# nwicakson/diffpose-nw

Hardware: AMD Instinct MI355X
Metric: poses/sec (B=1024, 17j, K=50 DDIM) at 1/2/4/8 MI355X; MPJPE Δ vs ref (higher is better)
Workload: dtype fp32

## Files before the change

diffpose-nw_amd/csrc/dpk_kernels.hip:

```cpp
#include <hip/hip_runtime.h>

#include <math.h>
#include <stdint.h>
#include <stdio.h>
#include <stdlib.h>
#include <string.h>

#include <algorithm>
#include <atomic>
#include <string>
#include <type_traits>
#include <unordered_map>
#include <vector>

#include "diffpose_kernels.h"

#ifndef DPK_ABLATE
#define DPK_ABLATE 0
#endif
#define DPK_RUN(bit) ((DPK_ABLATE & (bit)) == 0)
#ifndef DPK_TRACE
#define DPK_TRACE 0
#endif
#if DPK_TRACE
namespace dpk {
__shared__ unsigned long long* tr_row[8];
__shared__ int tr_ix[8];
__device__ __forceinline__ void tr_stamp() {
    const int w = threadIdx.x >> 6;
    if (tr_row[w] && (threadIdx.x & 63) == 0 && tr_ix[w] < 256) tr_row[w][tr_ix[w]] = __builtin_amdgcn_s_memtime();
    if ((threadIdx.x & 63) == 0 && tr_row[w]) tr_ix[w] += 1;
}
}
#ifndef DPK_GEMM_HOOK
#define DPK_GEMM_HOOK(tag)                       \
    do {                                         \
        if ((tag) != 0) {                        \
            __builtin_amdgcn_sched_barrier(0);   \
            dpk::tr_stamp();                     \
            __builtin_amdgcn_sched_barrier(0);   \
        }                                        \
    } while (0)
#endif
#endif
#ifndef DPK_GEMM_HOOK
#define DPK_GEMM_HOOK(tag)
#endif


namespace dpk_shared {
struct SampleArgs {
    const float* arena;
    const float* coef;
    const float* tproj;
    const float* x_in;
    float* x_out;
    float* xs;
    float* x0s;
    float* uvxyz;
    int N;
    int K;
    int H;
    int root_mode;
    unsigned mask;
    const unsigned* pmask;
    float eta;
    unsigned long long seed;
    int pose_off;
    int num_layers;
    int split_n;
    int split_k;
    int split_full;
    unsigned* flags;
    unsigned token;
    const float* noise;
    int* split_stats;
    int split_dbg;
#if DPK_TRACE
    unsigned long long* trace;
    int trace_step;
#endif
};
}

#include "dpk_stage.inc"
#include "dpk_scratch.inc"

#define DPK_P 4
namespace dpk {
#include "dpk_sampler.inc"
#include "dpk_genfused.inc"
}
#undef DPK_P
#define DPK_P 2
namespace dpk2 {
#include "dpk_sampler.inc"
#include "dpk_genfused.inc"
}
#undef DPK_P
#define DPK_P 2
#undef DPK_D
#undef DPK_NH
#define DPK_D 128
#define DPK_NH 8
namespace dpkw {
#include "dpk_sampler.inc"
#include "dpk_genfused.inc"
}
#undef DPK_NH
#undef DPK_D
#undef DPK_P
#define DPK_P 2
#define DPK_D 128
#define DPK_NH 4
namespace dpkw4 {
#include "dpk_sampler.inc"
#include "dpk_genfused.inc"
}
#undef DPK_NH
#undef DPK_D
#undef DPK_P
#define DPK_P 4
#define DPK_D 64
#define DPK_NH 2
namespace dpkn {
#include "dpk_sampler.inc"
#include "dpk_genfused.inc"
}
#undef DPK_NH
#define DPK_NH 4
namespace dpkn4 {
#include "dpk_sampler.inc"
#include "dpk_genfused.inc"
}
#undef DPK_NH
#undef DPK_D
#undef DPK_P

namespace dpk {

__global__ void __launch_bounds__(256) ddim_kernel(const float* __restrict__ xt, const float* __restrict__ et,
                                                   float* __restrict__ xn, float* __restrict__ x0o, long long n,
                                                   const float* __restrict__ cf, int step, float eta,
                                                   unsigned long long seed, const float* __restrict__ noise) {
    const long long i = (long long)blockIdx.x * 256 + threadIdx.x;
    if (i >= n) return;
    const float z = noise ? noise[i] : (eta != 0.f ? normal_noise(seed, step, i) : 0.f);
    float x0, x1;
    ddim_elem(cf, xt[i], et[i], z, x0, x1);
    xn[i] = x1;
    if (x0o) x0o[i] = x0;
}

}

using namespace dpk;

struct Sched {
    uint64_t serial = 0;
    float* buf = nullptr;
    float* coef = nullptr;
    float* tps = nullptr;
    int K = 0;
    float eta = 0.f;
    std::vector<float> h_coef;
    uint64_t tps_gen = 0;
    int pins = 0;
    std::vector<std::pair<hipStream_t, hipEvent_t>> uses;
};

struct CapRes {
    unsigned long long id = 0;
    std::atomic<int> refs{1};
    std::atomic<bool> released{false};
    bool tracked = false;
    std::vector<Sched*> scheds;
    std::vector<ScratchBuf> bufs;
    std::vector<std::pair<hipStream_t, int>> slots;
};
static void cap_release_cb(void* p) {
    CapRes* c = static_cast<CapRes*>(p);
    c->released.store(true);
    if (c->refs.fetch_sub(1) == 1) delete c;
}

struct GenModel;
struct dpk_handle {
    int device = 0;
    GenModel* gen = nullptr;
    int n_pts = J;
    int kind = 0;
    int num_layers = NL;
    int n_cu = 256;
    int tail_plan = 2;
    unsigned* flags = nullptr;
    std::vector<int> slot_free;
    std::vector<std::pair<int, hipEvent_t>> slot_busy;
    std::vector<hipEvent_t> slot_ev;
    int split_dbg = 0;
    unsigned token = 0;
    std::vector<CapRes*> caps;
    std::string err;
    float* arena = nullptr;
    float* temb = nullptr;
    float* tproj_zero = nullptr;
    hipStream_t aux = nullptr;
    uint64_t weights_gen = 0;
    Sched* sched = nullptr;
    std::vector<Sched*> retired;
    ScratchPool pool;
    Stage stage;
    Packed pk;
    char* arena16 = nullptr;
    char* arenabf = nullptr;
    int gemm_mode = 0;
    bool have_graph = false, have_weights = false;
    unsigned mask = (1u << J) - 1u;
    const unsigned* pmask = nullptr;
    int pmask_n = 0;
    bool profiling = false;
    std::vector<std::pair<hipEvent_t, hipEvent_t>> ev_used, ev_free;
#if DPK_TRACE
    unsigned long long* trace = nullptr;
    size_t trace_len = 0;
    int trace_step = -1;
#endif
};

static int fail(dpk_handle* h, int code, const std::string& msg) {
    if (h) h->err = msg;
    return code;
}

template <class F>
static int profiled(dpk_handle* h, hipStream_t st, bool cap, const char* who, F launch) {
    if (!h->profiling || cap) return launch();
    if (h->ev_free.empty()) {
        hipEvent_t a, b;
        if (hipEventCreate(&a) != hipSuccess || hipEventCreate(&b) != hipSuccess)
            return fail(h, DPK_E_HIP, std::string(who) + ": event record");
        h->ev_free.push_back({a, b});
    }
    const std::pair<hipEvent_t, hipEvent_t> ev = h->ev_free.back();
    h->ev_free.pop_back();
    if (hipEventRecord(ev.first, st) != hipSuccess) return fail(h, DPK_E_HIP, std::string(who) + ": event record");
    const int rc = launch();
    if (rc) return rc;
    if (hipEventRecord(ev.second, st) != hipSuccess) return fail(h, DPK_E_HIP, std::string(who) + ": event record");
    h->ev_used.push_back(ev);
    return DPK_OK;
}

#define HIPCHK(h, expr)                                                                        \
    do {                                                                                       \
        hipError_t e_ = (expr);                                                                \
        if (e_ != hipSuccess)                                                                  \
            return fail((h), DPK_E_HIP, std::string(#expr) + ": " + hipGetErrorString(e_));    \
    } while (0)

static int capturing(dpk_handle* h, hipStream_t st, bool* cap) {
    hipStreamCaptureStatus cs = hipStreamCaptureStatusNone;
    HIPCHK(h, hipStreamIsCapturing(st, &cs));
    *cap = cs != hipStreamCaptureStatusNone;
    return DPK_OK;
}

static void sched_free(Sched* s) {
    if (s->buf) (void)hipFree(s->buf);
    for (auto& u : s->uses) (void)hipEventDestroy(u.second);
    delete s;
}

static void sched_sweep(dpk_handle* h) {
    std::vector<Sched*> keep;
    for (Sched* s : h->retired) {
        bool done = s->pins == 0;
        for (auto& u : s->uses) done = done && hipEventQuery(u.second) == hipSuccess;
        if (done) sched_free(s);
        else keep.push_back(s);
    }
    h->retired.swap(keep);
}

static int cap_get(dpk_handle* h, hipStream_t st, CapRes** out) {
    hipStreamCaptureStatus cs = hipStreamCaptureStatusNone;
    unsigned long long id = 0;
    hipGraph_t graph = nullptr;
    HIPCHK(h, hipStreamGetCaptureInfo_v2(st, &cs, &id, &graph, nullptr, nullptr));
    for (CapRes* c : h->caps)
        if (c->id == id) {
            *out = c;
            return DPK_OK;
        }
    CapRes* c = new CapRes();
    c->id = id;
    const char* env = getenv("DPK_CAPTURE_RELEASE");
    if (graph && !(env && atoi(env) == 0)) {
        c->refs.fetch_add(1);
        hipUserObject_t obj = nullptr;
        if (hipUserObjectCreate(&obj, c, cap_release_cb, 1, hipUserObjectNoDestructorSync) != hipSuccess) {
            c->refs.fetch_sub(1);
            (void)hipGetLastError();
        } else if (hipGraphRetainUserObject(graph, obj, 1, hipGraphUserObjectMove) != hipSuccess) {
            (void)hipGetLastError();
            (void)hipUserObjectRelease(obj, 1);
        } else {
            c->tracked = true;
        }
    }
    h->caps.push_back(c);
    *out = c;
    return DPK_OK;
}

static void slot_put(dpk_handle* h, int slot) { h->slot_free.push_back(slot); }

static bool drain_relaxed() {
    hipStreamCaptureMode mode = hipStreamCaptureModeRelaxed;
    const bool exch = hipThreadExchangeStreamCaptureMode(&mode) == hipSuccess;
    const hipError_t se = hipDeviceSynchronize();
    if (exch) (void)hipThreadExchangeStreamCaptureMode(&mode);
    if (se != hipSuccess) (void)hipGetLastError();
    return se == hipSuccess;
}

static void cap_sweep(dpk_handle* h) {
    bool any = false;
    for (CapRes* c : h->caps) any = any || (c->tracked && c->released.load());
    if (!any) return;
    std::vector<CapRes*> keep;
    for (CapRes* c : h->caps) {
        if (!(c->tracked && c->released.load())) {
            keep.push_back(c);
            continue;
        }
        for (Sched* s : c->scheds) --s->pins;
        scratch_release(h->pool, c->bufs);
        for (auto& s : c->slots) slot_put(h, s.second);
        if (c->refs.fetch_sub(1) == 1) delete c;
    }
    h->caps.swap(keep);
    sched_sweep(h);
}

static int sched_note_use(dpk_handle* h, Sched* s, hipStream_t st, bool cap) {
    if (cap) {
        CapRes* c = nullptr;
        const int rc = cap_get(h, st, &c);
        if (rc) return rc;
        if (std::find(c->scheds.begin(), c->scheds.end(), s) == c->scheds.end()) {
            c->scheds.push_back(s);
            ++s->pins;
        }
        return DPK_OK;
    }
    hipEvent_t ev = nullptr;
    for (auto& u : s->uses)
        if (u.first == st) ev = u.second;
    if (!ev) {
        HIPCHK(h, hipEventCreateWithFlags(&ev, hipEventDisableTiming));
        s->uses.push_back({st, ev});
    }
    HIPCHK(h, hipEventRecord(ev, st));
    return DPK_OK;
}

static int sched_compute_tps(dpk_handle* h, Sched* s) {
    hipLaunchKernelGGL(temb_kernel, dim3(s->K), dim3(256), 0, h->aux, h->temb, s->coef + 5, 6, s->tps);
    HIPCHK(h, hipGetLastError());
    HIPCHK(h, hipStreamSynchronize(h->aux));
    s->tps_gen = h->weights_gen;
    return DPK_OK;
}

static int upload(dpk_handle* h) {
    HIPCHK(h, hipSetDevice(h->device));
    HIPCHK(h, hipDeviceSynchronize());
    sched_sweep(h);
    if (!h->arena) HIPCHK(h, hipMalloc(&h->arena, (size_t)ARENA_FLOATS * 4));
    if (!h->arena16) HIPCHK(h, hipMalloc(&h->arena16, (size_t)ARENA16_BYTES));
    HIPCHK(h, hipMemcpy(h->arena16, h->pk.a16.data(), (size_t)ARENA16_BYTES, hipMemcpyHostToDevice));
    if (!h->arenabf) HIPCHK(h, hipMalloc(&h->arenabf, (size_t)ARENAB_BYTES));
    HIPCHK(h, hipMemcpy(h->arenabf, h->pk.abf.data(), (size_t)ARENAB_BYTES, hipMemcpyHostToDevice));
    if (!h->temb) HIPCHK(h, hipMalloc(&h->temb, (size_t)TEMB_FLOATS * 4));
    HIPCHK(h, hipMemcpy(h->arena, h->pk.arena.data(), (size_t)ARENA_FLOATS * 4, hipMemcpyHostToDevice));
    HIPCHK(h, hipMemcpy(h->temb, h->pk.temb.data(), (size_t)TEMB_FLOATS * 4, hipMemcpyHostToDevice));
    ++h->weights_gen;
    if (!h->have_weights || h->kind != 0) return DPK_OK;
    if (h->sched) {
        const int rc = sched_compute_tps(h, h->sched);
        if (rc) return rc;
    }
    for (Sched* s : h->retired) {
        const int rc = sched_compute_tps(h, s);
        if (rc) return rc;
    }
    return DPK_OK;
}

constexpr int FLAG_SLOTS = 64;
static int split_slot(dpk_handle* h, hipStream_t st, bool cap) {
    if (!h->flags) return -1;
    if (cap) {
        CapRes* c = nullptr;
        if (cap_get(h, st, &c)) return -1;
        for (auto& s : c->slots)
            if (s.first == st) return s.second;
        if (h->slot_free.empty()) return -1;
        const int slot = h->slot_free.back();
        h->slot_free.pop_back();
        c->slots.push_back({st, slot});
        return slot;
    }
    std::vector<std::pair<int, hipEvent_t>> busy;
    for (auto& b : h->slot_busy) {
        if (hipEventQuery(b.second) == hipSuccess) {
            h->slot_free.push_back(b.first);
            h->slot_ev.push_back(b.second);
        } else {
            busy.push_back(b);
        }
    }
    (void)hipGetLastError();
    h->slot_busy.swap(busy);
    if (h->slot_free.empty()) return -1;
    const int slot = h->slot_free.back();
    h->slot_free.pop_back();
    return slot;
}
static int split_slot_hold(dpk_handle* h, int slot, hipStream_t st) {
    hipEvent_t ev = nullptr;
    if (!h->slot_ev.empty()) {
        ev = h->slot_ev.back();
        h->slot_ev.pop_back();
    } else if (hipEventCreateWithFlags(&ev, hipEventDisableTiming) != hipSuccess) {
        h->slot_free.push_back(slot);
        HIPCHK(h, hipStreamSynchronize(st));
        return DPK_OK;
    }
    h->slot_busy.push_back({slot, ev});
    HIPCHK(h, hipEventRecord(ev, st));
    return DPK_OK;
}

template <int MODE, int PT>
static void launch_tiles(dpk_handle* h, int blocks, size_t shmem, hipStream_t st, const SampleArgs& a) {
    const char* a16 = h->gemm_mode == 2 ? h->arenabf : h->arena16;
    if constexpr (PT == 4) dpk::launch_sample<MODE>(h->pk.sparse, h->gemm_mode, blocks, shmem, st, a, h->arena, a16);
    else dpk2::launch_sample<MODE>(h->pk.sparse, h->gemm_mode, blocks, shmem, st, a, h->arena, a16);
}

template <int MODE>
static int launch_sampler(dpk_handle* h, hipStream_t st, SampleArgs a, bool cap) {
    const int N = a.N;
    const int round4 = P * h->n_cu;
    if constexpr (MODE == M_SAMPLE) {
        const int tiles = (N + P - 1) / P, q = tiles / h->n_cu, r = tiles % h->n_cu;
        if (h->tail_plan == 2 && a.K >= 2 && q >= 1 && r > 0 && 2 * r <= h->n_cu) {
            const int slot = split_slot(h, st, cap);
            if (slot >= 0) {
                a.pose_off = 0;
                a.split_n = r;
                a.split_k = a.K / 2;
                a.split_full = q * h->n_cu;
                a.flags = h->flags + (size_t)slot * h->n_cu;
                a.split_stats = reinterpret_cast<int*>(h->flags + (size_t)FLAG_SLOTS * h->n_cu);
                a.split_dbg = h->split_dbg;
                h->token = (h->token + 1) & 0x3fffffffu;
                if (h->token == 0) h->token = 1;
                a.token = h->token;
                launch_tiles<MODE, P>(h, q * h->n_cu + 2 * r, 0, st, a);
                HIPCHK(h, hipGetLastError());
                return cap ? DPK_OK : split_slot_hold(h, slot, st);
            }
        }
    }
    int n4 = N;
    const int rem = N % round4;
    if (h->tail_plan >= 1 && rem != 0 && rem <= 2 * h->n_cu) n4 = N - rem;
    if (n4 > 0) {
        a.pose_off = 0;
        launch_tiles<MODE, P>(h, (n4 + P - 1) / P, 0, st, a);
    }
    if (n4 < N) {
        constexpr int P2 = dpk2::P;
        constexpr size_t half = 160 * 1024 / 2, lds2 = (size_t)dpk2::SM_FLOATS * 4;
        constexpr size_t pad = lds2 > half ? 0 : half - lds2 + 256;
        a.pose_off = n4;
        launch_tiles<MODE, P2>(h, (N - n4 + P2 - 1) / P2, pad, st, a);
    }
    HIPCHK(h, hipGetLastError());
    return DPK_OK;
}

static int call_scratch(dpk_handle* h, hipStream_t st, bool cap, size_t n, const char* who, ScratchBuf& got,
                        ScratchStatus& why) {
    why = SCRATCH_OK;
    if (!cap) {
        got = ScratchBuf{st, scratch_get(h->pool, st, n), n};
        if (got.p) return DPK_OK;
        return fail(h, DPK_E_HIP, std::string(who) + ": scratch of " + std::to_string(n) + " floats: " +
                                      hipGetErrorString(hipGetLastError()));
    }
    CapRes* c = nullptr;
    const int rc = cap_get(h, st, &c);
    if (rc) return rc;
    why = scratch_get_captured(h->pool, c->bufs, st, n, got);
    return why == SCRATCH_OK ? DPK_OK : DPK_E_STATE;
}

static SampleArgs eps_args(const dpk_handle* h, const float* arena, const float* tproj, const float* x, float* out,
                           int N) {
    SampleArgs a{};
    a.arena = arena;
    a.tproj = tproj;
    a.x_in = x;
    a.x_out = out;
    a.N = N;
    a.K = 1;
    a.mask = h->mask;
    a.pmask = h->pmask;
    a.num_layers = h->num_layers;
    return a;
}
static SampleArgs sample_args(const dpk_handle* h, const float* arena, const float* tproj, const Sched* sc,
                              const float* x, float* out, float* xs, float* x0s, int N, uint64_t seed,
                              const float* noise) {
    SampleArgs a = eps_args(h, arena, tproj, x, out, N);
    a.coef = sc->coef;
    a.K = sc->K;
    a.eta = sc->eta;
    a.xs = xs;
    a.x0s = x0s;
    a.seed = seed;
    a.noise = noise;
    return a;
}
static SampleArgs pose_args(const dpk_handle* h, const float* arena, const float* zeros, const float* x2d, float* xyz,
                            float* uvxyz, int N, int H, int root_mode) {
    SampleArgs a = eps_args(h, arena, zeros, x2d, xyz, N);
    a.uvxyz = uvxyz;
    a.H = H;
    a.root_mode = root_mode;
    return a;
}

#include "dpk_generic.inc"

static int enter_call(dpk_handle* h, int N, const char* who, hipStream_t st, bool* cap) {
    if (h->pmask && N > h->pmask_n)
        return fail(h, DPK_E_INVALID, std::string(who) + ": " + std::to_string(N) + " poses but dpk_set_pose_masks covers " +
                                          std::to_string(h->pmask_n));
    HIPCHK(h, hipSetDevice(h->device));
    const int rc = capturing(h, st, cap);
    if (rc) return rc;
    if (!*cap) cap_sweep(h);
    return DPK_OK;
}

extern "C" {

int dpk_version(void) { return 100; }

int dpk_kernel_geometry(int* ppw, int* tpw, int* lds) {
    if (ppw) *ppw = P;
    if (tpw) *tpw = NT;
    if (lds) *lds = SM_FLOATS * 4;
    return DPK_OK;
}

int dpk_create(const dpk_config* cfg, dpk_handle** out) {
    if (!cfg || !out) return DPK_E_INVALID;
    *out = nullptr;
    const char* fg = getenv("DPK_FORCE_GENERIC");
    const bool pose_io = cfg->coords_in == CIN_POSE && cfg->coords_out == COUT_POSE;
    const bool compiled = cfg->hid_dim == D && cfg->num_layers >= 1 && cfg->num_layers <= NL && cfg->n_head == NH &&
                          cfg->n_pts == J && (pose_io || (cfg->coords_in == CIN && cfg->coords_out == COUT)) &&
                          !(fg && atoi(fg) != 0);
    if (cfg->hid_dim < 2 || cfg->n_head < 1 || cfg->hid_dim % cfg->n_head != 0 || cfg->num_layers < 1 ||
        cfg->n_pts < 2 || cfg->n_pts > dpkg::GJ_MAX || cfg->coords_in < 1 || cfg->coords_out < 1)
        return DPK_E_UNSUPPORTED;
    int kind;
    if (pose_io) kind = 1;
    else if (cfg->coords_in == cfg->coords_out) kind = 0;
    else return DPK_E_UNSUPPORTED;
    int ndev = 0;
    if (hipGetDeviceCount(&ndev) != hipSuccess || cfg->device < 0 || cfg->device >= ndev) return DPK_E_HIP;
    dpk_handle* h = new dpk_handle();
    h->device = cfg->device;
    h->kind = kind;
    h->num_layers = cfg->num_layers;
    h->n_pts = cfg->n_pts;
    h->mask = cfg->n_pts >= 32 ? ~0u : (1u << cfg->n_pts) - 1u;
    if (compiled) stage_init(h->stage, D, NH, J, cfg->num_layers, cfg->coords_in, cfg->coords_out, kind);
    else {
        h->gen = gen_new(cfg->hid_dim, cfg->n_head, cfg->n_pts, cfg->num_layers, cfg->coords_in, cfg->coords_out, kind);
        h->pool.replaced = gen_scratch_replaced;
        h->pool.ctx = h->gen;
    }
    if (hipSetDevice(h->device) != hipSuccess ||
        hipStreamCreateWithFlags(&h->aux, hipStreamNonBlocking) != hipSuccess ||
        hipDeviceGetAttribute(&h->n_cu, hipDeviceAttributeMultiprocessorCount, h->device) != hipSuccess) {
        if (h->aux) (void)hipStreamDestroy(h->aux);
        gen_free(h->gen);
        delete h;
        return DPK_E_HIP;
    }
    h->n_cu = std::max(h->n_cu, 1);
    if (const char* ts = getenv("DPK_TAIL_SPLIT")) h->tail_plan = std::min(std::max(atoi(ts), 0), 2);
    if (DPK_TRACE) h->tail_plan = 0;
    const size_t flag_bytes = ((size_t)FLAG_SLOTS * h->n_cu + 4) * 4;
    for (int s = FLAG_SLOTS - 1; s >= 0; --s) h->slot_free.push_back(s);
    if (hipMalloc(&h->flags, flag_bytes) != hipSuccess || hipMemset(h->flags, 0, flag_bytes) != hipSuccess) {
        if (h->flags) (void)hipFree(h->flags);
        (void)hipStreamDestroy(h->aux);
        gen_free(h->gen);
        delete h;
        return DPK_E_HIP;
    }
    *out = h;
    return DPK_OK;
}

void dpk_destroy(dpk_handle* h) {
    if (!h) return;
    (void)hipSetDevice(h->device);
    if (h->arena) (void)hipFree(h->arena);
    if (h->arena16) (void)hipFree(h->arena16);
    if (h->arenabf) (void)hipFree(h->arenabf);
    if (h->temb) (void)hipFree(h->temb);
    if (h->tproj_zero) (void)hipFree(h->tproj_zero);
    if (h->flags) (void)hipFree(h->flags);
    gen_free(h->gen);
    if (h->sched) sched_free(h->sched);
    for (Sched* s : h->retired) sched_free(s);
    scratch_free_all(h->pool);
    for (CapRes* c : h->caps) {
        scratch_free(c->bufs);
        if (c->refs.fetch_sub(1) == 1) delete c;
    }
    for (auto& b : h->slot_busy) (void)hipEventDestroy(b.second);
    for (hipEvent_t e : h->slot_ev) (void)hipEventDestroy(e);
    if (h->aux) (void)hipStreamDestroy(h->aux);
    for (auto* v : {&h->ev_used, &h->ev_free})
        for (auto& e : *v) {
            (void)hipEventDestroy(e.first);
            (void)hipEventDestroy(e.second);
        }
    delete h;
}

const char* dpk_last_error(const dpk_handle* h) { return h ? h->err.c_str() : "null handle"; }

static int pack_upload(dpk_handle* h) {
    if (h->gen) return gen_upload(h, h->gen);
    dpk::pack_model(h->stage, h->pk, true);
    return upload(h);
}

int dpk_set_graph(dpk_handle* h, const float* adj) {
    if (!h || !adj) return fail(h, DPK_E_INVALID, "dpk_set_graph: null argument");
    stage_set_graph(h->gen ? h->gen->s : h->stage, adj);
    h->have_graph = true;
    return h->have_weights ? pack_upload(h) : DPK_OK;
}

int dpk_set_mask(dpk_handle* h, const uint8_t* m) {
    if (!h || !m) return fail(h, DPK_E_INVALID, "dpk_set_mask: null argument");
    unsigned bits = 0;
    for (int j = 0; j < h->n_pts; ++j)
        if (m[j]) bits |= 1u << j;
    h->mask = bits;
    return DPK_OK;
}

int dpk_set_pose_masks(dpk_handle* h, const uint32_t* bits_dev, int n) {
    if (!h) return DPK_E_INVALID;
    if (bits_dev && n <= 0) return fail(h, DPK_E_INVALID, "dpk_set_pose_masks: n must be positive");
    h->pmask = reinterpret_cast<const unsigned*>(bits_dev);
    h->pmask_n = bits_dev ? n : 0;
    return DPK_OK;
}

int dpk_load_weights(dpk_handle* h, const char* const* names, const float* const* ptrs, const int64_t* numels,
                     int n) {
    if (!h || !names || !ptrs || !numels || n <= 0) return fail(h, DPK_E_INVALID, "dpk_load_weights: bad args");
    for (int i = 0; i < n; ++i)
        if (!names[i] || !ptrs[i]) return fail(h, DPK_E_INVALID, "dpk_load_weights: null entry");
    std::string err;
    if (!stage_load(h->gen ? h->gen->s : h->stage, names, ptrs, numels, n, err))
        return fail(h, DPK_E_WEIGHTS, "dpk_load_weights: " + err);
    h->have_weights = true;
    const int rc = pack_upload(h);
    if (rc || h->gen || h->kind == 0) return rc;
    if (!h->tproj_zero) {
        HIPCHK(h, hipMalloc(&h->tproj_zero, (size_t)NL * D * 4));
        HIPCHK(h, hipMemset(h->tproj_zero, 0, (size_t)NL * D * 4));
    }
    return DPK_OK;
}

int dpk_set_schedule(dpk_handle* h, const float* abar, int n_alpha, const int* seq, int K, float eta) {
    if (!h || !abar || !seq || K <= 0 || n_alpha < 2) return fail(h, DPK_E_INVALID, "dpk_set_schedule: bad args");
    if (h->kind != 0) return fail(h, DPK_E_STATE, "GCNpose handle (coords 2->3) has no diffusion schedule");
    std::vector<float> c((size_t)K * 6);
    for (int s = 0; s < K; ++s) {
        const int t = seq[K - 1 - s];
        const int tn = (K - 2 - s) >= 0 ? seq[K - 2 - s] : -1;
        if (t + 1 < 0 || t + 1 >= n_alpha || tn + 1 < 0 || tn + 1 >= n_alpha)
            return fail(h, DPK_E_INVALID, "dpk_set_schedule: timestep outside alpha table (index t+1)");
        const float at = abar[t + 1], an = abar[tn + 1];
        const float one = 1.0f;
        volatile float s1a = sqrtf(one - at);
        volatile float sa = sqrtf(at);
        volatile float san = sqrtf(an);
        volatile float r = at / an;
        volatile float u = one - r;
        volatile float v = one - an;
        volatile float w = u * v;
        volatile float inner = w / (one - at);
        volatile float c1 = eta * sqrtf(inner);
        volatile float c1sq = c1 * c1;
        volatile float c2 = sqrtf((one - an) - c1sq);
        c[s * 6 + 0] = s1a;
        c[s * 6 + 1] = sa;
        c[s * 6 + 2] = san;
        c[s * 6 + 3] = c1;
        c[s * 6 + 4] = c2;
        c[s * 6 + 5] = (float)t;
    }
    HIPCHK(h, hipSetDevice(h->device));
    sched_sweep(h);
    if (h->sched && h->sched->K == K && h->sched->eta == eta && h->sched->h_coef == c) return DPK_OK;
    Sched* s = new Sched();
    static uint64_t sched_serial = 0;
    s->serial = ++sched_serial;
    const size_t tps_off = ((size_t)K * 6 + 3) / 4 * 4;
    hipError_t e = hipMalloc(&s->buf, (tps_off + (size_t)K * NL * D) * 4);
    if (e != hipSuccess) {
        delete s;
        return fail(h, DPK_E_HIP, std::string("dpk_set_schedule: hipMalloc: ") + hipGetErrorString(e) +
                                      " (a schedule cannot be built while a graph is being captured)");
    }
    s->coef = s->buf;
    s->tps = s->buf + tps_off;
    s->K = K;
    s->eta = eta;
    s->h_coef = c;
    e = hipMemcpyAsync(s->coef, c.data(), c.size() * 4, hipMemcpyHostToDevice, h->aux);
    if (e == hipSuccess) e = hipStreamSynchronize(h->aux);
    if (e != hipSuccess) {
        sched_free(s);
        return fail(h, DPK_E_HIP, std::string("dpk_set_schedule: coef upload: ") + hipGetErrorString(e));
    }
    if (h->have_weights && !h->gen) {
        const int rc = sched_compute_tps(h, s);
        if (rc) {
            sched_free(s);
            return rc;
        }
    }
    if (h->sched) h->retired.push_back(h->sched);
    h->sched = s;
    sched_sweep(h);
    return DPK_OK;
}


static int check_ready(dpk_handle* h, int kind = 0) {
    if (h->kind != kind)
        return fail(h, DPK_E_STATE, kind ? "GCNdiff handle: dpk_pose needs a GCNpose handle (coords 2->3)"
                                         : "GCNpose handle (coords 2->3): use dpk_pose");
    if (!h->have_graph) return fail(h, DPK_E_STATE, "graph (adjacency) not set");
    if (!h->have_weights) return fail(h, DPK_E_STATE, "weights not loaded");
    if (h->gen && h->gemm_mode != 0)
        return fail(h, DPK_E_UNSUPPORTED, "generic-shape path (model shape other than hid 96 / 4 heads / 17 joints): "
                                          "fp32 GEMMs only (gemm mode 0)");
    if (h->gemm_mode == 1 && !h->pk.w16_ok)
        return fail(h, DPK_E_UNSUPPORTED, "gemm mode 1 (3x fp16): a GEMM weight has |w| >= 1015, outside the split-fp16 "
                                          "packing range; use gemm mode 0 (fp32)");
    return DPK_OK;
}

int dpk_eps(dpk_handle* h, const float* x, const float* t, float* eps, int N, void* stream) {
    if (!h) return DPK_E_INVALID;
    if (N < 0 || (N > 0 && (!x || !t || !eps))) return fail(h, DPK_E_INVALID, "dpk_eps: bad args");
    int rc = check_ready(h);
    if (rc) return rc;
    if (N == 0) return DPK_OK;
    hipStream_t st = (hipStream_t)stream;
    bool cap = false;
    if ((rc = enter_call(h, N, "dpk_eps", st, &cap))) return rc;
    if (h->gen) return gen_eps(h, x, t, eps, N, st, cap);
    constexpr size_t PP = (size_t)NL * D;
    ScratchBuf buf;
    ScratchStatus why;
    if ((rc = call_scratch(h, st, cap, (size_t)(cap ? N : std::max(N, 64)) * PP, "dpk_eps", buf, why))) {
        if (why == SCRATCH_NO_SPARE)
            return fail(h, rc, "dpk_eps: a captured call needs a projection buffer of " + std::to_string(N) +
                                   " poses, and the spare holds " + std::to_string(buf.cap / PP) +
                                   "; make an uncaptured dpk_eps call of >= N poses before the capture");
        if (why == SCRATCH_SHARED_TOO_SMALL)
            return fail(h, rc, "dpk_eps: the captured calls of one stream share the buffer of the capture's "
                               "first call (" + std::to_string(buf.cap / PP) + " poses); this one has " +
                                   std::to_string(N) + "; warm up with the largest N before capturing");
        return rc;
    }
    hipLaunchKernelGGL(temb_kernel, dim3(N), dim3(256), 0, st, h->temb, t, 1, buf.p);
    HIPCHK(h, hipGetLastError());
    return profiled(h, st, cap, "dpk_eps", [&] {
        return launch_sampler<M_EPS>(h, st, eps_args(h, h->arena, buf.p, x, eps, N), cap);
    });
}

int dpk_sample(dpk_handle* h, const float* x, float* out, float* xs, float* x0s, int N, uint64_t seed,
               void* stream) {
    return dpk_sample_noise(h, x, out, xs, x0s, N, seed, nullptr, stream);
}

int dpk_sample_noise(dpk_handle* h, const float* x, float* out, float* xs, float* x0s, int N, uint64_t seed,
                     const float* noise, void* stream) {
    if (!h) return DPK_E_INVALID;
    if (N < 0 || (N > 0 && (!x || !out))) return fail(h, DPK_E_INVALID, "dpk_sample: bad args");
    int rc = check_ready(h);
    if (rc) return rc;
    Sched* sc = h->sched;
    if (!sc) return fail(h, DPK_E_STATE, "schedule not set");
    if (N == 0) return DPK_OK;
    if (!h->gen && sc->tps_gen != h->weights_gen)
        return fail(h, DPK_E_STATE, "dpk_sample: schedule projections are stale");
    hipStream_t st = (hipStream_t)stream;
    bool cap = false;
    if ((rc = enter_call(h, N, "dpk_sample", st, &cap))) return rc;
    if (!cap) sched_sweep(h);
    if (h->gen) return gen_sample(h, sc, x, out, xs, x0s, N, seed, noise, st, cap);
    if (xs) HIPCHK(h, hipMemcpyAsync(xs, x, (size_t)N * PE * 4, hipMemcpyDeviceToDevice, st));
    SampleArgs a = sample_args(h, h->arena, sc->tps, sc, x, out, xs, x0s, N, seed, noise);
#if DPK_TRACE
    if (h->trace_step >= 0) {
        const size_t len = (size_t)((N + P - 1) / P) * NW * TRACE_SLOTS;
        if (h->trace_len < len) {
            if (h->trace) HIPCHK(h, hipFree(h->trace));
            HIPCHK(h, hipMalloc(&h->trace, len * 8));
            h->trace_len = len;
        }
        HIPCHK(h, hipMemsetAsync(h->trace, 0, len * 8, st));
    }
    a.trace = h->trace_step >= 0 ? h->trace : nullptr;
    a.trace_step = h->trace_step;
#endif
    rc = profiled(h, st, cap, "dpk_sample", [&] { return launch_sampler<M_SAMPLE>(h, st, a, cap); });
    return rc ? rc : sched_note_use(h, sc, st, cap);
}

int dpk_pose(dpk_handle* h, const float* x2d, float* xyz, float* uvxyz, int N, int H, int root_mode,
             void* stream) {
    if (!h) return DPK_E_INVALID;
    if (N < 0 || H < 1 || root_mode < 0 || root_mode > 2 || (N > 0 && (!x2d || (!xyz && !uvxyz))))
        return fail(h, DPK_E_INVALID, "dpk_pose: bad args");
    int rc = check_ready(h, 1);
    if (rc) return rc;
    if (N == 0) return DPK_OK;
    hipStream_t st = (hipStream_t)stream;
    bool cap = false;
    if ((rc = enter_call(h, N, "dpk_pose", st, &cap))) return rc;
    if (h->gen) return gen_pose(h, x2d, xyz, uvxyz, N, H, root_mode, st, cap);
    return profiled(h, st, cap, "dpk_pose", [&] {
        return launch_sampler<M_POSE>(h, st, pose_args(h, h->arena, h->tproj_zero, x2d, xyz, uvxyz, N, H, root_mode), cap);
    });
}

int dpk_set_gemm_mode(dpk_handle* h, int mode) {
    if (!h) return DPK_E_INVALID;
    if (mode < 0 || mode > 2)
        return fail(h, DPK_E_INVALID, "dpk_set_gemm_mode: mode must be 0 (fp32), 1 (3xfp16) or 2 (bf16)");
    h->gemm_mode = mode;
    return DPK_OK;
}

int dpk_set_tail_plan(dpk_handle* h, int plan) {
    if (!h) return DPK_E_INVALID;
    if (plan < 0 || plan > 2) return fail(h, DPK_E_INVALID, "dpk_set_tail_plan: plan must be 0, 1 or 2");
    h->tail_plan = DPK_TRACE ? 0 : plan;
    return DPK_OK;
}

int dpk_profile(dpk_handle* h, int enable) {
    if (!h) return DPK_E_INVALID;
    h->profiling = enable != 0;
    return DPK_OK;
}

int dpk_profile_read(dpk_handle* h, float* ms, int cap, int* count) {
    if (!h || (cap > 0 && !ms)) return fail(h, DPK_E_INVALID, "dpk_profile_read: bad args");
    HIPCHK(h, hipSetDevice(h->device));
    int n = 0;
    for (auto& e : h->ev_used) {
        HIPCHK(h, hipEventSynchronize(e.second));
        float t = 0.f;
        HIPCHK(h, hipEventElapsedTime(&t, e.first, e.second));
        if (n < cap) ms[n] = t;
        ++n;
        h->ev_free.push_back(e);
    }
    h->ev_used.clear();
    if (count) *count = n;
    return DPK_OK;
}

int dpk_ddim_update(dpk_handle* h, const float* xt, const float* et, float* xn, float* x0, int64_t n, int step,
                    uint64_t seed, void* stream) {
    return dpk_ddim_update_noise(h, xt, et, xn, x0, n, step, seed, nullptr, stream);
}

int dpk_ddim_update_noise(dpk_handle* h, const float* xt, const float* et, float* xn, float* x0, int64_t n,
                          int step, uint64_t seed, const float* noise, void* stream) {
    if (!h) return DPK_E_INVALID;
    if (n < 0 || (n > 0 && (!xt || !et || !xn))) return fail(h, DPK_E_INVALID, "dpk_ddim_update: bad args");
    Sched* sc = h->sched;
    if (!sc) return fail(h, DPK_E_STATE, "schedule not set");
    if (step < 0 || step >= sc->K) return fail(h, DPK_E_INVALID, "dpk_ddim_update: step out of range");
    if (n == 0) return DPK_OK;
    HIPCHK(h, hipSetDevice(h->device));
    hipStream_t st = (hipStream_t)stream;
    bool cap = false;
    int rc = capturing(h, st, &cap);
    if (rc) return rc;
    if (!cap) cap_sweep(h);
    const long long nb = (n + 255) / 256;
    hipLaunchKernelGGL(ddim_kernel, dim3((unsigned)nb), dim3(256), 0, st, xt, et, xn, x0, (long long)n,
                       sc->coef + step * 6, step, sc->eta, (unsigned long long)seed, noise);
    HIPCHK(h, hipGetLastError());
    return sched_note_use(h, sc, st, cap);
}

int dpk_debug_split(dpk_handle* h, int mode, int* fallbacks) {
    if (!h) return DPK_E_INVALID;
    if (mode < 0 || mode > 2) return fail(h, DPK_E_INVALID, "dpk_debug_split: mode must be 0, 1 or 2");
    h->split_dbg = mode;
    if (fallbacks) {
        HIPCHK(h, hipSetDevice(h->device));
        HIPCHK(h, hipDeviceSynchronize());
        int* ctr = reinterpret_cast<int*>(h->flags + (size_t)FLAG_SLOTS * h->n_cu);
        HIPCHK(h, hipMemcpy(fallbacks, ctr, 4, hipMemcpyDeviceToHost));
        HIPCHK(h, hipMemset(ctr, 0, 4));
    }
    return DPK_OK;
}

int dpk_debug_resources(dpk_handle* h, int* out, int n) {
    if (!h || (n > 0 && !out)) return DPK_E_INVALID;
    int released = 0, tracked = 0, retired = (int)h->retired.size();
    for (CapRes* c : h->caps) {
        tracked += c->tracked ? 1 : 0;
        released += (c->tracked && c->released.load()) ? 1 : 0;
    }
    const size_t spare = h->pool.spare.cap;
    const int v[8] = {(int)h->caps.size(), tracked, released, (int)h->slot_free.size(), retired,
                      h->gen ? 0 : (int)(spare / ((size_t)NL * D)), gen_graph_count(h->gen),
                      h->gen ? (int)((spare * 4) >> 10) : 0};
    for (int i = 0; i < n && i < 8; ++i) out[i] = v[i];
    return DPK_OK;
}

#if DPK_TRACE
int dpk_debug_trace(dpk_handle* h, int step, unsigned long long* out, long long cap) {
    if (!h) return DPK_E_INVALID;
    h->trace_step = step;
    if (!out || !h->trace) return DPK_OK;
    HIPCHK(h, hipDeviceSynchronize());
    HIPCHK(h, hipMemcpy(out, h->trace, std::min((size_t)cap, h->trace_len) * 8, hipMemcpyDeviceToHost));
    return (int)std::min((size_t)cap, h->trace_len);
}
#endif

}
```

diffpose-nw_amd/csrc/dpk_layout.inc:

```

#ifndef DPK_D
#define DPK_D 96
#endif
#ifndef DPK_NH
#define DPK_NH 4
#endif
constexpr int J = 17;
constexpr int D = DPK_D;
constexpr int D2 = 2 * D;
constexpr int D3 = 3 * D;
constexpr int E = 4 * D;
constexpr int NL = 5;
constexpr int NH = DPK_NH;
constexpr int DK = D / NH;
static_assert(D % 32 == 0 && D <= 128 && (DK == 24 || DK == 16 || DK == 32), "widths: multiples of 32 up to 128, d_k 16, 24 or 32");
constexpr int NCD = D / 16;
constexpr int CIN = 5;
constexpr int COUT = 5;
constexpr int PE = J * CIN;

constexpr bool HALF_MODES = D == 96 && NH == 4;

constexpr int P = DPK_P;
constexpr int R = P * J;
static_assert(P == 4 || P == 2, "4 or 2 poses per workgroup");
constexpr int NW = 4;
constexpr int NT = 64 * NW;
constexpr int stride40(int n) { return n + (104 - n % 64) % 64; }
constexpr int LDX = stride40(D);
constexpr int LD2 = stride40(D3);
static_assert(LDX % 64 == 40 && LD2 % 64 == 40 && LDX >= D && LD2 >= D3, "row strides");

constexpr int SM_XS = 0;
constexpr int SM_B1 = SM_XS + R * LDX;
constexpr int SM_B2 = SM_B1 + R * LDX;
constexpr int SM_XST = SM_B2 + R * LD2;
constexpr int SM_LNP = SM_XST + ((R * CIN + 3) / 4) * 4;
constexpr int SM_TC = SM_LNP + NL * 4 * D;
constexpr int SM_TS = SM_TC + 2 * J * J;
constexpr int SM_FLOATS = SM_TS + J * (5 + 9) * 2;
static_assert(SM_FLOATS * 4 <= 160 * 1024, "LDS budget");

constexpr int BLK = 256;
constexpr int KB_D = D / 16, KB_D2 = D2 / 16, KB_D3 = D3 / 16;
constexpr int OFF_QKV = 0;
constexpr int OFF_O = OFF_QKV + 3 * NCD * KB_D * BLK;
constexpr int OFF_FC1 = OFF_O + NCD * KB_D * BLK;
constexpr int OFF_FC2 = OFF_FC1 + 2 * NCD * KB_D * BLK;
constexpr int OFF_C1 = OFF_FC2 + NCD * KB_D2 * BLK;
constexpr int OFF_C2 = OFF_C1 + NCD * KB_D3 * BLK;
constexpr int OFF_BQKV = OFF_C2 + NCD * KB_D3 * BLK;
constexpr int OFF_BO = OFF_BQKV + D3;
constexpr int OFF_BFC1 = OFF_BO + D;
constexpr int OFF_BFC2 = OFF_BFC1 + D2;
constexpr int OFF_BC1 = OFF_BFC2 + D;
constexpr int OFF_BC2 = OFF_BC1 + D;
constexpr int OFF_LN0A = OFF_BC2 + D;
constexpr int OFF_LN0B = OFF_LN0A + D;
constexpr int OFF_LN1A = OFF_LN0B + D;
constexpr int OFF_LN1B = OFF_LN1A + D;
constexpr int OFF_LG = OFF_LN1B + D;
constexpr int OFF_LGF = ((OFF_LG + J * J + 63) / 64) * 64;
constexpr int OFF_CQKV = OFF_LGF + 2 * 5 * 64;
constexpr int LAYER_FLOATS = ((OFF_CQKV + D3 + 63) / 64) * 64;
constexpr int OFF_WIN = NL * LAYER_FLOATS;
constexpr int OFF_WOUT = OFF_WIN + NCD * 1 * BLK;
constexpr int OFF_BIN = OFF_WOUT + 1 * KB_D3 * BLK;
constexpr int OFF_BOUT = OFF_BIN + D;
constexpr int OFF_CHEB = OFF_BOUT + 16;
constexpr int OFF_CHEBS = OFF_CHEB + 2 * J * J;
constexpr int SPT1 = 5, SPT2 = 9;
constexpr int OFF_CHEBT = OFF_CHEBS + 136;
constexpr int CHEBT_FLOATS = J * (SPT1 + SPT2) * 2;
constexpr int ARENA_FLOATS = ((OFF_CHEBT + CHEBT_FLOATS + 63) / 64) * 64;

constexpr float W16_SCALE = 64.0f;
constexpr int BLK16 = 2048;
constexpr int KB32_D = D / 32, KB32_D2 = D2 / 32, KB32_D3 = D3 / 32;
constexpr int O16_QKV = 0;
constexpr int O16_O = O16_QKV + 3 * NCD * KB32_D * BLK16;
constexpr int O16_FC1 = O16_O + NCD * KB32_D * BLK16;
constexpr int O16_FC2 = O16_FC1 + 2 * NCD * KB32_D * BLK16;
constexpr int O16_C1 = O16_FC2 + NCD * KB32_D2 * BLK16;
constexpr int O16_C2 = O16_C1 + NCD * KB32_D3 * BLK16;
constexpr int LAYER16_BYTES = O16_C2 + NCD * KB32_D3 * BLK16;
constexpr int ARENA16_BYTES = NL * LAYER16_BYTES;

constexpr int TOFF_W0 = 0;
constexpr int TOFF_B0 = TOFF_W0 + D * E;
constexpr int TOFF_W1 = TOFF_B0 + E;
constexpr int TOFF_B1 = TOFF_W1 + E * E;
constexpr int TOFF_WP = TOFF_B1 + E;
constexpr int TOFF_BP = TOFF_WP + NL * E * D;
constexpr int TEMB_FLOATS = TOFF_BP + NL * D;

constexpr float SQRT_DK = DK == 24 ? 4.898979485566356f : DK == 32 ? 5.656854249492381f : 4.0f;
constexpr float LN_EPS = 1e-6f;
constexpr int H36M_EDGES[16][2] = {{0, 1}, {1, 2}, {2, 3}, {0, 4}, {4, 5}, {5, 6}, {0, 7}, {7, 8},
                                   {8, 9}, {9, 10}, {8, 11}, {11, 12}, {12, 13}, {8, 14}, {14, 15}, {15, 16}};
struct SparsePattern {
    int n1[J], c1[J][J], o1[J];
    int n2[J], c2[J][J], o2[J];
    int nnz1, nnz2;
};
constexpr SparsePattern make_pattern() {
    SparsePattern sp{};
    bool a[J][J] = {};
    for (int i = 0; i < J; ++i) a[i][i] = true;
    for (int e = 0; e < 16; ++e) {
        a[H36M_EDGES[e][0]][H36M_EDGES[e][1]] = true;
        a[H36M_EDGES[e][1]][H36M_EDGES[e][0]] = true;
    }
    int t1 = 0, t2 = 0;
    for (int i = 0; i < J; ++i) {
        sp.n1[i] = 0;
        sp.n2[i] = 0;
        sp.o1[i] = t1;
        sp.o2[i] = t2;
        for (int j = 0; j < J; ++j) {
            bool two = false;
            for (int k = 0; k < J; ++k) two = two || (a[i][k] && a[k][j]);
            if (a[i][j]) sp.c1[i][sp.n1[i]++] = j;
            if (two) sp.c2[i][sp.n2[i]++] = j;
        }
        t1 += sp.n1[i];
        t2 += sp.n2[i];
    }
    sp.nnz1 = t1;
    sp.nnz2 = t2;
    return sp;
}
constexpr SparsePattern SPAT = make_pattern();
static_assert(SPAT.nnz1 == 49 && SPAT.nnz2 == 87, "H36M Chebyshev sparsity");
```

diffpose-nw_amd/csrc/dpk_sampler.inc:

```

#include "dpk_layout.inc"

struct NoHook {
    __device__ __forceinline__ void operator()() const {}
};
#ifndef DPK_PRE_MID
#define DPK_PRE_MID 14
#endif
#define DPK_MID(bit) ((DPK_PRE_MID & (bit)) != 0)

typedef float f32x4 __attribute__((ext_vector_type(4)));
typedef float f32x2 __attribute__((ext_vector_type(2)));

__device__ __forceinline__ f32x2 pfma(f32x2 a, f32x2 b, f32x2 c) { return __builtin_elementwise_fma(a, b, c); }
__device__ __forceinline__ f32x2 splat2(float x) { return f32x2{x, x}; }
__device__ __forceinline__ f32x2 vpair(float x) {
    f32x2 p = {x, x};
    asm volatile("" : "+v"(p));
    return p;
}
__device__ __forceinline__ f32x4 padd4(f32x4 x, f32x2 ns) {
    const f32x2 lo = f32x2{x[0], x[1]} + ns, hi = f32x2{x[2], x[3]} + ns;
    return f32x4{lo[0], lo[1], hi[0], hi[1]};
}
__device__ __forceinline__ f32x4 pmul4(f32x4 x, f32x2 r) {
    const f32x2 lo = f32x2{x[0], x[1]} * r, hi = f32x2{x[2], x[3]} * r;
    return f32x4{lo[0], lo[1], hi[0], hi[1]};
}

typedef _Float16 f16x8 __attribute__((ext_vector_type(8)));
typedef _Float16 f16x4 __attribute__((ext_vector_type(4)));
typedef _Float16 f16x2 __attribute__((ext_vector_type(2)));
typedef __bf16 bf16x8 __attribute__((ext_vector_type(8)));
typedef __bf16 bf16x2 __attribute__((ext_vector_type(2)));
typedef short s16x4 __attribute__((ext_vector_type(4)));

enum { M_SAMPLE = 0, M_EPS = 1, M_POSE = 2 };
constexpr int CIN_POSE = 2, COUT_POSE = 3;

using SampleArgs = ::dpk_shared::SampleArgs;
constexpr int TRACE_SLOTS = 256;

__device__ __forceinline__ void philox(uint32_t c[4], uint32_t k0, uint32_t k1) {
#pragma unroll
    for (int r = 0; r < 10; ++r) {
        const uint64_t p0 = (uint64_t)0xD2511F53u * c[0];
        const uint64_t p1 = (uint64_t)0xCD9E8D57u * c[2];
        const uint32_t n0 = (uint32_t)(p1 >> 32) ^ c[1] ^ k0;
        const uint32_t n2 = (uint32_t)(p0 >> 32) ^ c[3] ^ k1;
        c[1] = (uint32_t)p1;
        c[3] = (uint32_t)p0;
        c[0] = n0;
        c[2] = n2;
        k0 += 0x9E3779B9u;
        k1 += 0xBB67AE85u;
    }
}

__device__ __forceinline__ float normal_noise(unsigned long long seed, int step, long long idx) {
    uint32_t c[4] = {(uint32_t)idx, (uint32_t)((unsigned long long)idx >> 32), (uint32_t)step, 0x5EEDu};
    philox(c, (uint32_t)seed, (uint32_t)(seed >> 32));
    const float u1 = ((float)(c[0] >> 8) + 1.0f) * (1.0f / 16777216.0f);
    const float u2 = (float)(c[1] >> 8) * (1.0f / 16777216.0f);
    return sqrtf(-2.0f * logf(u1)) * cosf(6.283185307179586f * u2);
}

__device__ __forceinline__ void ddim_elem(const float* cf, float xt, float et, float z, float& x0, float& xn) {
    x0 = (xt - et * cf[0]) / cf[1];
    xn = (cf[2] * x0 + cf[3] * z) + cf[4] * et;
}

template <int J>
__device__ __forceinline__ float row_ror(float x) {
    return __builtin_bit_cast(float, __builtin_amdgcn_update_dpp(__builtin_bit_cast(int, x), __builtin_bit_cast(int, x),
                                                                 0x120 + J, 0xf, 0xf, false));
}

__device__ __forceinline__ float sum4rows(float v) {
    float a = v, b = v;
    asm("s_nop 1\n\tv_permlane32_swap_b32 %0, %1" : "+v"(a), "+v"(b));
    const float s1 = a + b;
    float c = s1, d = s1;
    asm("s_nop 1\n\tv_permlane16_swap_b32 %0, %1" : "+v"(c), "+v"(d));
    return c + d;
}

__device__ __forceinline__ void sum4rows2(float& x, float& y) {
    asm("s_nop 1\n\tv_permlane32_swap_b32 %0, %1" : "+v"(x), "+v"(y));
    float c = x + y, d = c;
    asm("s_nop 1\n\tv_permlane16_swap_b32 %0, %1" : "+v"(c), "+v"(d));
    x = c + d;
    y = x;
    asm("s_nop 1\n\tv_permlane32_swap_b32 %0, %1" : "+v"(x), "+v"(y));
}
__device__ __forceinline__ void max4rows2(float& x, float& y) {
    asm("s_nop 1\n\tv_permlane32_swap_b32 %0, %1" : "+v"(x), "+v"(y));
    float c = fmaxf(x, y), d = c;
    asm("s_nop 1\n\tv_permlane16_swap_b32 %0, %1" : "+v"(c), "+v"(d));
    x = fmaxf(c, d);
    y = x;
    asm("s_nop 1\n\tv_permlane32_swap_b32 %0, %1" : "+v"(x), "+v"(y));
}

__device__ __forceinline__ float rs4rows(float v0, float v1, float v2, float v3) {
    asm("s_nop 1\n\tv_permlane32_swap_b32 %0, %1" : "+v"(v0), "+v"(v2));
    asm("s_nop 1\n\tv_permlane32_swap_b32 %0, %1" : "+v"(v1), "+v"(v3));
    float a = v0 + v2, b = v1 + v3;
    asm("s_nop 1\n\tv_permlane16_swap_b32 %0, %1" : "+v"(a), "+v"(b));
    return a + b;
}

constexpr int PAD_MFMA4 = 5;
constexpr int PAD_MFMA16 = 11;
template <int N, int K>
__device__ __forceinline__ void mfma_pad(f32x4 (&v)[K]) {
    static_assert(K >= 1 && K <= 8, "mfma_pad: 1..8 accumulators");
    if constexpr (K == 1) asm volatile("s_nop %1" : "+v"(v[0]) : "i"(N));
    else if constexpr (K == 2) asm volatile("s_nop %2" : "+v"(v[0]), "+v"(v[1]) : "i"(N));
    else if constexpr (K == 3) asm volatile("s_nop %3" : "+v"(v[0]), "+v"(v[1]), "+v"(v[2]) : "i"(N));
    else if constexpr (K == 4) asm volatile("s_nop %4" : "+v"(v[0]), "+v"(v[1]), "+v"(v[2]), "+v"(v[3]) : "i"(N));
    else if constexpr (K == 5)
        asm volatile("s_nop %5" : "+v"(v[0]), "+v"(v[1]), "+v"(v[2]), "+v"(v[3]), "+v"(v[4]) : "i"(N));
    else if constexpr (K == 6)
        asm volatile("s_nop %6" : "+v"(v[0]), "+v"(v[1]), "+v"(v[2]), "+v"(v[3]), "+v"(v[4]), "+v"(v[5]) : "i"(N));
    else if constexpr (K == 7)
        asm volatile("s_nop %7"
                     : "+v"(v[0]), "+v"(v[1]), "+v"(v[2]), "+v"(v[3]), "+v"(v[4]), "+v"(v[5]), "+v"(v[6])
                     : "i"(N));
    else
        asm volatile("s_nop %8"
                     : "+v"(v[0]), "+v"(v[1]), "+v"(v[2]), "+v"(v[3]), "+v"(v[4]), "+v"(v[5]), "+v"(v[6]), "+v"(v[7])
                     : "i"(N));
}

__device__ __forceinline__ int opaque(int x) {
    asm volatile("" : "+v"(x));
    return x;
}
__device__ __forceinline__ int opaque_s(int x) {
    asm volatile("" : "+s"(x));
    return x;
}

struct BSrc {
    __amdgpu_buffer_rsrc_t rsrc;
    int voff;
    int sbase;
    __device__ __forceinline__ f32x4 load(int blk) const {
        return __builtin_bit_cast(f32x4, __builtin_amdgcn_raw_buffer_load_b128(rsrc, voff, sbase + blk * 1024, 0));
    }
};

__device__ __forceinline__ f32x4 bload(const BSrc& s, int toff, int kb) {
    return __builtin_bit_cast(f32x4, __builtin_amdgcn_raw_buffer_load_b128(s.rsrc, toff, kb * 1024, 0));
}

template <int NC, int KB>
__device__ __forceinline__ BSrc bsrc(const float* Bp, int ct0, int lane) {
    BSrc s;
    s.rsrc = __builtin_amdgcn_make_buffer_rsrc((void*)Bp, (short)0, 0x7fffffff, 0x00020000);
    s.voff = lane * 16;
    s.sbase = ct0 * KB * 1024;
    return s;
}

enum { TM_NONE = 0, TM_VALU = 1, TM_MFMA4 = 2 };

template <int NR, int NCW, int TM, int TR, int KB, bool TRANS = true>
struct GemmTile {
    static constexpr int TA = TM == TM_VALU ? TR : 1;
    static constexpr int NQ = TM == TM_MFMA4 ? (NCW + 1) / 2 : 1;
    f32x4 acc[NR][NCW];
    float tl[NCW][TA];
    f32x4 tacc[NQ];
    int aoff[NR], toff[TA];

    __device__ __forceinline__ void loadA(f32x4 (&a)[NR], f32x4 (&t)[TA], const float* A, int kb) const {
#pragma unroll
        for (int i = 0; i < NR; ++i) a[i] = *reinterpret_cast<const f32x4*>(A + aoff[i] + kb * 16);
        if constexpr (TM != TM_NONE) {
#pragma unroll
            for (int i = 0; i < TA; ++i) t[i] = *reinterpret_cast<const f32x4*>(A + toff[i] + kb * 16);
        }
    }
    __device__ __forceinline__ static void loadB(f32x4 (&b)[NCW], const BSrc& s, const int (&soff)[NCW], int kb) {
#pragma unroll
        for (int c = 0; c < NCW; ++c) b[c] = bload(s, soff[c], kb);
    }
    template <bool FIRST = false>
    __device__ __forceinline__ void mma(const f32x4 (&a)[NR], const f32x4 (&t)[TA], const f32x4 (&b)[NCW]) {
        const f32x4 z = {0.f, 0.f, 0.f, 0.f};
#pragma unroll
        for (int j = 0; j < 4; ++j) {
#pragma unroll
            for (int i = 0; i < NR; ++i)
#pragma unroll
                for (int c = 0; c < NCW; ++c) {
                    const f32x4 cin = (FIRST && j == 0) ? z : acc[i][c];
                    acc[i][c] = TRANS ? __builtin_amdgcn_mfma_f32_16x16x4f32(b[c][j], a[i][j], cin, 0, 0, 0)
                                      : __builtin_amdgcn_mfma_f32_16x16x4f32(a[i][j], b[c][j], cin, 0, 0, 0);
                }
            if constexpr (TM == TM_VALU) {
#pragma unroll
                for (int c = 0; c < NCW; ++c)
#pragma unroll
                    for (int r = 0; r < TR; ++r) tl[c][r] = fmaf(t[r][j], b[c][j], tl[c][r]);
            } else if constexpr (TM == TM_MFMA4) {
#pragma unroll
                for (int q = 0; q < NQ; ++q)
                    tacc[q] = __builtin_amdgcn_mfma_f32_4x4x1f32(b[q][j], t[0][j], (FIRST && j == 0) ? z : tacc[q], 0, 0, 0);
            }
        }
    }
    __device__ __forceinline__ static void schedule_half() { __builtin_amdgcn_sched_barrier(0); }
};

template <int NCW>
struct BPre {
    f32x4 b0[NCW], b1[NCW];
};

__device__ __forceinline__ int gemm_ch(int wave) { return R == 68 ? (wave & 1) : (wave >> 1); }
__device__ __forceinline__ int gemm_pr(int wave) { return R == 68 ? (wave >> 1) : (wave & 1); }

template <int NCW>
__device__ __forceinline__ int col_rot(int wave) { return gemm_pr(wave) ? (NCW + 1) / 2 : 0; }

template <int NCW, int KB>
__device__ __forceinline__ void tile_offsets(int (&soff)[NCW], const BSrc& s, int rot) {
#pragma unroll
    for (int c = 0; c < NCW; ++c) {
        const int cc = c + rot;
        soff[c] = s.voff + s.sbase + (cc >= NCW ? cc - NCW : cc) * KB * 1024;
    }
}

template <int NC, int KB, int NPRE = 2>
__device__ __forceinline__ BPre<NC / 2> gemm_prefetch(const float* Bp, int wave, int lane) {
    constexpr int NCW = NC / 2;
    const BSrc s = bsrc<NC, KB>(Bp, gemm_ch(wave) * NCW, lane);
    int soff[NCW];
    tile_offsets<NCW, KB>(soff, s, col_rot<NCW>(wave));
    BPre<NCW> pre;
#pragma unroll
    for (int c = 0; c < NCW; ++c) {
        pre.b0[c] = bload(s, soff[c], 0);
        pre.b1[c] = (KB > 1 && NPRE > 1) ? bload(s, soff[c], 1) : f32x4{0.f, 0.f, 0.f, 0.f};
    }
    return pre;
}

#ifndef DPK_PRE_LATE
#define DPK_PRE_LATE 5
#endif
#define DPK_LATE(bit) ((DPK_PRE_LATE & (bit)) != 0)
#ifndef DPK_FC1_NPRE
#define DPK_FC1_NPRE 2
#endif
#ifndef DPK_QKV_NPRE
#define DPK_QKV_NPRE 1
#endif
enum { E_STORE = 0, E_STORE_RELU, E_RESID, E_RESID_RELU, E_CHEB1, E_STORE_NB };

struct EpiArgs {
    float* dst;
    int ldd;
    const float* bias;
    const float* tproj;
    int tproj_pose_stride;
    int pose0;
    int pose_max;
};

__device__ __forceinline__ float rcp_nr(float d) {
    const float r = __builtin_amdgcn_rcpf(d);
    return fmaf(r, fmaf(-d, r, 1.0f), r);
}

template <int MODE>
__device__ __forceinline__ float epi_value(float acc, float bias, float tp, float old) {
    const float v = acc + bias;
    if constexpr (MODE == E_STORE_NB) return acc;
    else if constexpr (MODE == E_STORE) return v;
    else if constexpr (MODE == E_STORE_RELU) return fmaxf(v, 0.f);
    else if constexpr (MODE == E_RESID) return old + v;
    else if constexpr (MODE == E_RESID_RELU) return old + fmaxf(v, 0.f);
    else return fmaxf(v, 0.f) + tp;
}

template <int MODE, bool NB = false>
__device__ __forceinline__ f32x4 epi_value4(f32x4 acc, f32x4 bias, f32x4 tp, f32x4 old) {
    if constexpr (MODE == E_STORE_NB) return acc;
    f32x4 v = acc;
    if constexpr (!NB) v = acc + bias;
    const f32x4 z = {0.f, 0.f, 0.f, 0.f};
    if constexpr (MODE == E_STORE) return v;
    else if constexpr (MODE == E_STORE_RELU) return __builtin_elementwise_max(v, z);
    else if constexpr (MODE == E_RESID) return old + v;
    else if constexpr (MODE == E_RESID_RELU) return old + __builtin_elementwise_max(v, z);
    else return __builtin_elementwise_max(v, z) + tp;
}

__device__ __forceinline__ float tproj_at(const EpiArgs& e, int row, int col, float tcol) {
    if (e.tproj_pose_stride == 0) return tcol;
    const int pose = min(e.pose0 + row / J, e.pose_max);
    return e.tproj[(size_t)pose * e.tproj_pose_stride + col];
}


template <int NR, int NCW, int TM, int TR, int NC, int KB, int MODE, bool XS2 = false, int NPRE = 2>
__device__ __forceinline__ void gemm_wave(const float* A, int lda, const float* Bp, int rt0, int ct0, int rot,
                                          int trow0, bool tail_dup, int lane, const EpiArgs& e,
                                          const BPre<NCW>& pre, const float* AX = nullptr, int ldx = 0) {
    using T = GemmTile<NR, NCW, TM, TR, KB>;
    constexpr int TA = T::TA, NQ = T::NQ;
    static_assert(KB == 1 || KB % 2 == 0, "k-blocks in pairs");
    lane = opaque(lane);
    T g;
#pragma unroll
    for (int c = 0; c < NCW; ++c)
#pragma unroll
        for (int r = 0; r < TA; ++r) g.tl[c][r] = 0.f;
    const int rl = lane & 15, kq = (lane >> 4) * 4;
#pragma unroll
    for (int i = 0; i < NR; ++i) g.aoff[i] = ((rt0 + i) * 16 + rl) * lda + kq;
    if constexpr (TM == TM_MFMA4) {
        g.toff[0] = (trow0 + (lane & 3)) * lda + kq;
    } else {
#pragma unroll
        for (int i = 0; i < TA; ++i) g.toff[i] = (trow0 + i) * lda + kq;
    }
    int xoff[NR], xtoff = 0;
    if constexpr (XS2) {
        static_assert(TM == TM_MFMA4, "XS2: 4x4x1 tail rows");
#pragma unroll
        for (int i = 0; i < NR; ++i) xoff[i] = ((rt0 + i) * 16 + rl) * ldx + kq;
        xtoff = (trow0 + (lane & 3)) * ldx + kq;
    }
    int gcol[NCW];
#pragma unroll
    for (int c = 0; c < NCW; ++c) {
        const int cc = c + rot;
        gcol[c] = ct0 + (cc >= NCW ? cc - NCW : cc);
    }
    const BSrc src = bsrc<NC, KB>(Bp, ct0, lane);
    int soff[NCW];
    tile_offsets<NCW, KB>(soff, src, rot);
    const int tcol = 4 * ((lane >> 2) & 3) + (lane >> 4);
    f32x4 bias4[NCW], tp4[NCW];
    float tbias[NQ], ttp[NQ];
    auto load_epi_consts = [&]() {
        const unsigned kqu = (unsigned)kq, tcu = (unsigned)tcol;
        const int boff = (int)(e.bias - Bp) * 4;
#pragma unroll
        for (int c = 0; c < NCW; ++c) {
            const float* pt = e.tproj + gcol[c] * 16;
            if constexpr (MODE == E_STORE_NB) bias4[c] = f32x4{0.f, 0.f, 0.f, 0.f};
            else bias4[c] = __builtin_bit_cast(f32x4, __builtin_amdgcn_raw_buffer_load_b128(src.rsrc, kq * 4, boff + gcol[c] * 64, 0));
            tp4[c] = (MODE == E_CHEB1 && e.tproj_pose_stride == 0) ? *reinterpret_cast<const f32x4*>(pt + kqu)
                                                                   : f32x4{0.f, 0.f, 0.f, 0.f};
        }
#pragma unroll
        for (int q = 0; q < NQ; ++q) {
            tbias[q] = 0.f;
            ttp[q] = 0.f;
            if constexpr (TM == TM_MFMA4) {
                if constexpr (MODE != E_STORE_NB)
                    tbias[q] = __builtin_bit_cast(float, __builtin_amdgcn_raw_buffer_load_b32(src.rsrc, tcol * 4, boff + gcol[q] * 64, 0));
                if (MODE == E_CHEB1 && e.tproj_pose_stride == 0) ttp[q] = (e.tproj + gcol[q] * 16)[tcu];
            }
        }
    };
    constexpr int KBX = D / 16;
    constexpr int S = (KB == 1) ? 1
                      : (XS2 && (KBX == 8 || KBX == 4)) ? 4
                      : (NCW <= 6 && KB % 3 == 0) ? 3 : 2;
    static_assert(KB == 1 || KB % S == 0, "ring slots divide the k-blocks");
    static_assert(!XS2 || (KB > 2 * S && (KBX == S || KBX == 2 * S)), "XS2: the x block is one or two ring passes");
    f32x4 as[S][NR], ts[S][TA], bs[S][NCW];
    auto loadA = [&](int st, int kb) {
        if (XS2 && kb < KBX) {
#pragma unroll
            for (int i = 0; i < NR; ++i) as[st][i] = *reinterpret_cast<const f32x4*>(AX + xoff[i] + kb * 16);
            ts[st][0] = *reinterpret_cast<const f32x4*>(AX + xtoff + kb * 16);
        } else {
            g.loadA(as[st], ts[st], A, kb);
        }
    };
    constexpr bool RES = MODE == E_RESID || MODE == E_RESID_RELU;
    const int trow = trow0 + (lane & 3);
    constexpr int R0 = (NCW + 1) / 2;
    auto tile_ptr = [&](int i, int c) -> float* {
        const int row = (rt0 + i) * 16 + rl;
        float* rb = e.dst + row * e.ldd + kq + ct0 * 16;
        return (c < NCW - R0 ? rb + rot * 16 : rb - (rot ? (NCW - R0) * 16 : 0)) + c * 16;
    };
    f32x4 old[NR][NCW];
    float oldt[NQ];
    auto load_old = [&]() {
        if constexpr (RES) {
#pragma unroll
            for (int i = 0; i < NR; ++i)
#pragma unroll
                for (int c = 0; c < NCW; ++c)
                    old[i][c] = *reinterpret_cast<const f32x4*>(tile_ptr(i, c));
            if constexpr (TM == TM_MFMA4) {
#pragma unroll
                for (int q = 0; q < NQ; ++q) oldt[q] = e.dst[min(trow, R - 1) * e.ldd + gcol[q] * 16 + tcol];
            }
        }
    };
    constexpr int NP = S > 1 ? NPRE : 1;
#pragma unroll
    for (int c = 0; c < NCW; ++c) {
        bs[0][c] = pre.b0[c];
        if constexpr (NP > 1) bs[1][c] = pre.b1[c];
    }
    DPK_GEMM_HOOK(0);
#pragma unroll
    for (int st = NP; st < S; ++st) T::loadB(bs[st], src, soff, st);
#pragma unroll
    for (int st = 0; st < S; ++st) loadA(st, st);
    if constexpr (KB > S) {
#pragma unroll
        for (int st = 0; st < S; ++st) {
            if (st == 0) g.template mma<true>(as[0], ts[0], bs[0]);
            else g.mma(as[st], ts[st], bs[st]);
            T::loadB(bs[st], src, soff, st + S);
            loadA(st, st + S);
            T::schedule_half();
        }
#pragma unroll 1
        for (int kb = S; kb < KB - S; kb += S) {
#pragma unroll
            for (int st = 0; st < S; ++st) {
                g.mma(as[st], ts[st], bs[st]);
                T::loadB(bs[st], src, soff, kb + st + S);
                g.loadA(as[st], ts[st], A, kb + st + S);
                T::schedule_half();
            }
        }
        load_old();
        load_epi_consts();
#pragma unroll
        for (int st = 0; st < S; ++st) g.mma(as[st], ts[st], bs[st]);
    } else {
        __builtin_amdgcn_sched_barrier(0);
        load_epi_consts();
        load_old();
#pragma unroll
        for (int st = 0; st < S; ++st) {
            if (st == 0) g.template mma<true>(as[st], ts[st], bs[st]);
            else g.mma(as[st], ts[st], bs[st]);
        }
    }
    DPK_GEMM_HOOK(1);
    __builtin_amdgcn_sched_barrier(0);
    auto tproj4 = [&](int row, int col4, const f32x4& uniform4) -> f32x4 {
        if constexpr (MODE != E_CHEB1) return f32x4{0.f, 0.f, 0.f, 0.f};
        if (e.tproj_pose_stride == 0) return uniform4;
        const int pose = min(e.pose0 + row / J, e.pose_max);
        return *reinterpret_cast<const f32x4*>(e.tproj + (size_t)pose * e.tproj_pose_stride + col4);
    };
#pragma unroll
    for (int i = 0; i < NR; ++i) {
        const int row = (rt0 + i) * 16 + rl;
#pragma unroll
        for (int c = 0; c < NCW; ++c) {
            const int col4 = gcol[c] * 16 + kq;
            const f32x4 tp = tproj4(row, col4, tp4[c]);
            *reinterpret_cast<f32x4*>(tile_ptr(i, c)) =
                epi_value4<MODE>(g.acc[i][c], bias4[c], tp, RES ? old[i][c] : f32x4{0.f, 0.f, 0.f, 0.f});
        }
    }
    if constexpr (TM == TM_VALU) {
        static_assert(TM != TM_VALU, "gemm_wave computes transposed tiles; VALU tails are gemm_out's");
    } else if constexpr (TM == TM_MFMA4) {
        const int row = trow;
        mfma_pad<PAD_MFMA4>(g.tacc);
#pragma unroll
        for (int q = 0; q < NQ; ++q) {
            const float v = rs4rows(g.tacc[q][0], g.tacc[q][1], g.tacc[q][2], g.tacc[q][3]);
            const bool skip = (q == NQ - 1 && tail_dup) || row >= R;
            const int col = gcol[q] * 16 + tcol;
            const float tp = MODE == E_CHEB1 ? tproj_at(e, min(row, R - 1), col, ttp[q]) : 0.f;
            float val = epi_value<MODE>(v, tbias[q], tp, RES ? oldt[q] : 0.f);
            asm volatile("" : "+v"(val));
            if (!skip) e.dst[row * e.ldd + col] = val;
        }
    }
    DPK_GEMM_HOOK(2);
}

template <int NC, int KB, int MODE, bool XS2 = false, int NPRE = 2>
__device__ __forceinline__ void gemm_wg(const float* A, int lda, const float* Bp, int wave, int lane,
                                        const EpiArgs& e, const BPre<NC / 2>& pre,
                                        const float* AX = nullptr, int ldx = 0) {
    static_assert(NC % 2 == 0 && (R == 68 || R == 34), "row tiles x 2 column halves + tail rows");
    constexpr int NCW = NC / 2;
    constexpr int NRW = R == 68 ? 2 : 1;
    const int pr = gemm_pr(wave);
    const bool dup = (NCW & 1) && pr == 1;
    gemm_wave<NRW, NCW, TM_MFMA4, 0, NC, KB, MODE, XS2, NPRE>(A, lda, Bp, NRW * pr, gemm_ch(wave) * NCW,
                                                             col_rot<NCW>(wave), R - R % 16, dup, lane, e, pre, AX, ldx);
}

template <int PW>
__device__ __forceinline__ int pass_col(int ctp, int c, int rot) {
    const int cc = c + rot;
    return ctp + (cc >= PW ? cc - PW : cc);
}

#ifndef DPK_HS_BF
#define DPK_HS_BF 3
#endif
#ifndef DPK_PWQ16
#define DPK_PWQ16 3
#endif
#ifndef DPK_PWF16
#define DPK_PWF16 3
#endif
constexpr int BLKB = 1024;
template <int G>
constexpr int blkh() { return G == 1 ? BLK16 : BLKB; }
template <int G>
constexpr int offh(int l, int o16) { return G == 1 ? l * LAYER16_BYTES + o16 : (l * LAYER16_BYTES + o16) / 2; }
constexpr int ARENAB_BYTES = ARENA16_BYTES / 2;

template <int G>
struct AFr {
    f16x8 h, l;
};

__device__ __forceinline__ f16x8 cat2x4(f16x2 a, f16x2 b, f16x2 c, f16x2 d) {
    const f16x4 ab = __builtin_shufflevector(a, b, 0, 1, 2, 3), cd = __builtin_shufflevector(c, d, 0, 1, 2, 3);
    return __builtin_shufflevector(ab, cd, 0, 1, 2, 3, 4, 5, 6, 7);
}
template <int G>
__device__ __forceinline__ void acvt(const f32x4& lo4, const f32x4& hi4, AFr<G>& o) {
    const f32x2 v[4] = {f32x2{lo4[0], lo4[1]}, f32x2{lo4[2], lo4[3]}, f32x2{hi4[0], hi4[1]}, f32x2{hi4[2], hi4[3]}};
    f16x2 h[4], l[4];
#pragma unroll
    for (int p = 0; p < 4; ++p) {
        if constexpr (G == 2) {
            h[p] = __builtin_bit_cast(f16x2, __builtin_convertvector(v[p], bf16x2));
        } else {
            h[p] = __builtin_convertvector(v[p], f16x2);
            l[p] = __builtin_convertvector(v[p] - __builtin_convertvector(h[p], f32x2), f16x2);
        }
    }
    o.h = cat2x4(h[0], h[1], h[2], h[3]);
    if constexpr (G == 1) o.l = cat2x4(l[0], l[1], l[2], l[3]);
}

struct BSrcH {
    __amdgpu_buffer_rsrc_t rsrc;
    __device__ __forceinline__ f16x8 load(int voff, int soff) const {
        return __builtin_bit_cast(f16x8, __builtin_amdgcn_raw_buffer_load_b128(rsrc, voff, soff, 0));
    }
};
template <int G, int NC, int KB32>
__device__ __forceinline__ BSrcH bsrch(const char* Bp) {
    BSrcH s;
    s.rsrc = __builtin_amdgcn_make_buffer_rsrc((void*)Bp, (short)0, NC * KB32 * blkh<G>(), 0x00020000);
    return s;
}

template <int G, int PW>
struct BPreH {
    f16x8 h[2][PW], l[2][G == 1 ? PW : 1];
};
template <int PW>
__device__ __forceinline__ int passh_rot(int wave) { return gemm_pr(wave) ? (PW + 1) / 2 : 0; }
template <int G, int NC, int KB32, int PW>
__device__ __forceinline__ BPreH<G, PW> gemmh_prefetch(const char* Bp, int wave, int lane, int ps = 0) {
    constexpr int BK = blkh<G>();
    const BSrcH s = bsrch<G, NC, KB32>(Bp);
    const int ctp = gemm_ch(wave) * (NC / 2) + ps * PW, rot = passh_rot<PW>(wave);
    BPreH<G, PW> pre;
#pragma unroll
    for (int c = 0; c < PW; ++c) {
        const int voff = lane * 16 + pass_col<PW>(ctp, c, rot) * KB32 * BK;
#pragma unroll
        for (int k = 0; k < 2; ++k) {
            pre.h[k][c] = s.load(voff, k * BK);
            if constexpr (G == 1) pre.l[k][c] = s.load(voff, k * BK + 1024);
        }
    }
    return pre;
}

template <int G, int NR, int PW, int NC, int KB32, int MODE, bool XS2, int S, int AR>
__device__ __forceinline__ void gemmh_pass(const float* A, int lda, const float* AX, int ldx, const BSrcH& src,
                                           int rt0, int ctp, int rot, int trow0, bool tail_dup, int lane,
                                           const EpiArgs& e, const BPreH<G, PW>& pre, AFr<G> (*ar)[NR + 1]) {
    constexpr int BK = blkh<G>();
    constexpr int NQ = (PW + 1) / 2;
    constexpr int NA = NR + 1;
    static_assert(S >= 2 && S <= KB32, "ring slots");
    lane = opaque(lane);
    const int rl = lane & 15, g = lane >> 4, kq = g * 4;
    int gcol[PW], voff[PW];
#pragma unroll
    for (int c = 0; c < PW; ++c) {
        gcol[c] = pass_col<PW>(ctp, c, rot);
        voff[c] = lane * 16 + gcol[c] * KB32 * BK;
    }
    int aoff[NA], xoff[NA];
#pragma unroll
    for (int i = 0; i < NR; ++i) {
        aoff[i] = (int)__umul24((unsigned)((rt0 + i) * 16 + rl), (unsigned)lda) + kq;
        xoff[i] = (int)__umul24((unsigned)((rt0 + i) * 16 + rl), (unsigned)ldx) + kq;
    }
    const int trow_a = min(trow0 + rl, R - 1);
    aoff[NR] = (int)__umul24((unsigned)trow_a, (unsigned)lda) + kq;
    xoff[NR] = (int)__umul24((unsigned)trow_a, (unsigned)ldx) + kq;
    f32x4 raw[NA][2];
    auto loadA = [&](int kb) {
        if constexpr (AR != 2) {
#pragma unroll
            for (int i = 0; i < NA; ++i) {
                const float* p = (XS2 && kb * 32 < D) ? AX + xoff[i] + kb * 32 : A + aoff[i] + kb * 32;
                raw[i][0] = *reinterpret_cast<const f32x4*>(p);
                raw[i][1] = *reinterpret_cast<const f32x4*>(p + 16);
            }
        }
    };
    f16x8 bh[S][PW], bl[S][G == 1 ? PW : 1];
    auto loadB = [&](int st, int kb) {
#pragma unroll
        for (int c = 0; c < PW; ++c) {
            bh[st][c] = src.load(voff[c], kb * BK);
            if constexpr (G == 1) bl[st][c] = src.load(voff[c], kb * BK + 1024);
        }
    };
    f32x4 bias4[PW], tp4[PW];
    auto load_epi = [&]() {
        const __amdgpu_buffer_rsrc_t br = __builtin_amdgcn_make_buffer_rsrc((void*)e.bias, (short)0, 0x7fffffff, 0x00020000);
#pragma unroll
        for (int c = 0; c < PW; ++c) {
            bias4[c] = MODE == E_STORE_NB ? f32x4{0.f, 0.f, 0.f, 0.f}
                                          : __builtin_bit_cast(f32x4, __builtin_amdgcn_raw_buffer_load_b128(br, kq * 4, gcol[c] * 64, 0));
            tp4[c] = (MODE == E_CHEB1 && e.tproj_pose_stride == 0)
                         ? *reinterpret_cast<const f32x4*>(e.tproj + gcol[c] * 16 + kq)
                         : f32x4{0.f, 0.f, 0.f, 0.f};
        }
    };
#pragma unroll
    for (int c = 0; c < PW; ++c) {
        bh[0][c] = pre.h[0][c];
        bh[1][c] = pre.h[1][c];
        if constexpr (G == 1) {
            bl[0][c] = pre.l[0][c];
            bl[1][c] = pre.l[1][c];
        }
    }
#pragma unroll
    for (int st = 2; st < S; ++st) loadB(st, st);
    loadA(0);
    DPK_GEMM_HOOK(0);
    f32x4 acc[NR][PW], tacc[NQ];
    const f32x4 z = {0.f, 0.f, 0.f, 0.f};
    AFr<G> af[NA];
    auto cvt = [&](int kb) {
#pragma unroll
        for (int i = 0; i < NA; ++i) {
            if constexpr (AR == 2) af[i] = ar[kb][i];
            else acvt<G>(raw[i][0], raw[i][1], af[i]);
            if constexpr (AR == 1) ar[kb][i] = af[i];
        }
    };
    constexpr bool RES = MODE == E_RESID || MODE == E_RESID_RELU;
    f32x4 oldv[NR][PW], oldt[NQ];
    auto load_old = [&]() {
#pragma unroll
        for (int i = 0; i < NR; ++i) {
            const float* rp = e.dst + __umul24((unsigned)((rt0 + i) * 16 + rl), (unsigned)e.ldd) + kq;
#pragma unroll
            for (int c = 0; c < PW; ++c) oldv[i][c] = *reinterpret_cast<const f32x4*>(rp + gcol[c] * 16);
        }
#pragma unroll
        for (int q = 0; q < NQ; ++q)
            oldt[q] = *reinterpret_cast<const f32x4*>(e.dst + __umul24((unsigned)trow_a, (unsigned)e.ldd) + gcol[q] * 16 + kq);
    };
    constexpr int LAG = 2;
    constexpr int KEPI = KB32 - 2;
    constexpr float INV = 1.0f / W16_SCALE;
    const f32x2 inv2 = {INV, INV};
    auto epi_tile = [&](int i, int c) {
        const int row = (rt0 + i) * 16 + rl;
        float* p = e.dst + __umul24((unsigned)row, (unsigned)e.ldd) + kq + gcol[c] * 16;
        const f32x4 old = RES ? oldv[i][c] : z;
        f32x4 tp = tp4[c];
        if (MODE == E_CHEB1 && e.tproj_pose_stride != 0) {
            const int pose = min(e.pose0 + row / J, e.pose_max);
            tp = *reinterpret_cast<const f32x4*>(e.tproj + (size_t)pose * e.tproj_pose_stride + gcol[c] * 16 + kq);
        }
        const f32x4 a = acc[i][c];
        const f32x2 lo = __builtin_elementwise_fma(f32x2{a[0], a[1]}, inv2, f32x2{bias4[c][0], bias4[c][1]});
        const f32x2 hi = __builtin_elementwise_fma(f32x2{a[2], a[3]}, inv2, f32x2{bias4[c][2], bias4[c][3]});
        const f32x4 v = f32x4{lo[0], lo[1], hi[0], hi[1]};
        *reinterpret_cast<f32x4*>(p) = epi_value4<MODE, true>(v, z, tp, old);
    };
    auto tail_mfmas = [&](int st, int kb) {
#pragma unroll
        for (int q = 0; q < NQ; ++q) {
            f32x4 t = kb == 0 ? z : tacc[q];
            const f16x8 th = af[NR].h;
            if constexpr (G == 2) {
                t = __builtin_amdgcn_mfma_f32_16x16x32_bf16(__builtin_bit_cast(bf16x8, bh[st][q]), __builtin_bit_cast(bf16x8, th), t, 0, 0, 0);
            } else {
                t = __builtin_amdgcn_mfma_f32_16x16x32_f16(bl[st][q], th, t, 0, 0, 0);
                t = __builtin_amdgcn_mfma_f32_16x16x32_f16(bh[st][q], af[NR].l, t, 0, 0, 0);
                t = __builtin_amdgcn_mfma_f32_16x16x32_f16(bh[st][q], th, t, 0, 0, 0);
            }
            tacc[q] = t;
        }
    };
    auto epi_tail = [&](int q) {
        const int row = trow0 + rl;
        f32x4 tp = tp4[q];
        if (MODE == E_CHEB1 && e.tproj_pose_stride != 0) {
            const int pose = min(e.pose0 + min(row, R - 1) / J, e.pose_max);
            tp = *reinterpret_cast<const f32x4*>(e.tproj + (size_t)pose * e.tproj_pose_stride + gcol[q] * 16 + kq);
        }
        const f32x4 a = tacc[q];
        const f32x2 lo = __builtin_elementwise_fma(f32x2{a[0], a[1]}, inv2, f32x2{bias4[q][0], bias4[q][1]});
        const f32x2 hi = __builtin_elementwise_fma(f32x2{a[2], a[3]}, inv2, f32x2{bias4[q][2], bias4[q][3]});
        f32x4 o = epi_value4<MODE, true>(f32x4{lo[0], lo[1], hi[0], hi[1]}, z, tp, RES ? oldt[q] : z);
        asm volatile("" : "+v"(o));
        const bool skip = (q == NQ - 1 && tail_dup) || row >= R;
        if (!skip) *reinterpret_cast<f32x4*>(e.dst + __umul24((unsigned)row, (unsigned)e.ldd) + gcol[q] * 16 + kq) = o;
    };
#pragma unroll
    for (int kb = 0; kb < KB32; ++kb) {
        const int st = kb % S;
        cvt(kb);
        if (kb + 1 < KB32) loadA(kb + 1);
        if (kb == KEPI) {
            load_epi();
            if constexpr (RES) load_old();
        }
        const bool weave_kb = kb + 1 == KB32;
#pragma unroll
        for (int tt = 0; tt < NR * PW; ++tt) {
            const int i = tt / PW, c = tt % PW;
            const f32x4 cin = kb == 0 ? z : acc[i][c];
            if constexpr (G == 2) {
                acc[i][c] = __builtin_amdgcn_mfma_f32_16x16x32_bf16(__builtin_bit_cast(bf16x8, bh[st][c]),
                                                                    __builtin_bit_cast(bf16x8, af[i].h), cin, 0, 0, 0);
            } else {
                f32x4 t = __builtin_amdgcn_mfma_f32_16x16x32_f16(bl[st][c], af[i].h, cin, 0, 0, 0);
                t = __builtin_amdgcn_mfma_f32_16x16x32_f16(bh[st][c], af[i].l, t, 0, 0, 0);
                acc[i][c] = __builtin_amdgcn_mfma_f32_16x16x32_f16(bh[st][c], af[i].h, t, 0, 0, 0);
            }
            if (weave_kb && tt >= LAG) {
                epi_tile((tt - LAG) / PW, (tt - LAG) % PW);
                __builtin_amdgcn_sched_barrier(0);
            }
        }
        tail_mfmas(st, kb);
        if (kb + S < KB32) loadB(st, kb + S);
        __builtin_amdgcn_sched_barrier(0);
    }
    DPK_GEMM_HOOK(1);
#pragma unroll
    for (int tt = NR * PW > LAG ? NR * PW - LAG : 0; tt < NR * PW; ++tt) epi_tile(tt / PW, tt % PW);
#pragma unroll
    for (int q = 0; q < NQ; ++q) epi_tail(q);
    DPK_GEMM_HOOK(2);
}

template <int G, int NC, int KB32, int PW, int MODE, bool XS2 = false>
__device__ __forceinline__ void gemmh_wg(const float* A, int lda, const char* Bp, int wave, int lane, const EpiArgs& e,
                                         const BPreH<G, PW>& pre, const float* AX = nullptr, int ldx = 0) {
    static_assert(NC % 2 == 0 && (NC / 2) % PW == 0 && (R == 68 || R == 34), "passes of PW column tiles");
    constexpr int NCW = NC / 2, NRW = R == 68 ? 2 : 1, NPASS = NCW / PW;
    constexpr int S = PW >= 6 ? ((G == 2 && KB32 == 3) ? 3 : 2)
                              : (KB32 <= 3 ? KB32 : (G == 2 ? (DPK_HS_BF < KB32 ? DPK_HS_BF : KB32) : 3));
    const int pr = gemm_pr(wave);
    const int rot = passh_rot<PW>(wave);
    const bool dup = (PW & 1) && pr == 1;
    const BSrcH src = bsrch<G, NC, KB32>(Bp);
    const int ct0 = gemm_ch(wave) * NCW;
    if constexpr (NPASS == 1) {
        gemmh_pass<G, NRW, PW, NC, KB32, MODE, XS2, S, 0>(A, lda, AX, ldx, src, NRW * pr, ct0, rot, R - R % 16, dup,
                                                          lane, e, pre, nullptr);
    } else {
        AFr<G> ar[KB32][NRW + 1];
        gemmh_pass<G, NRW, PW, NC, KB32, MODE, XS2, S, 1>(A, lda, AX, ldx, src, NRW * pr, ct0, rot, R - R % 16, dup,
                                                          lane, e, pre, ar);
#pragma unroll
        for (int ps = 1; ps < NPASS; ++ps) {
            const BPreH<G, PW> p2 = gemmh_prefetch<G, NC, KB32, PW>(Bp, wave, lane, ps);
            gemmh_pass<G, NRW, PW, NC, KB32, MODE, XS2, S, 2>(A, lda, AX, ldx, src, NRW * pr, ct0 + ps * PW, rot,
                                                              R - R % 16, dup, lane, e, p2, ar);
        }
    }
}

template <int G, int NC, int KB32, int PW>
struct HGemm {
    using Pre = BPreH<G, PW>;
    __device__ __forceinline__ static Pre prefetch(const char* Bp, int wave, int lane) {
        return gemmh_prefetch<G, NC, KB32, PW>(Bp, wave, lane);
    }
    template <int MODE, bool XS2 = false>
    __device__ __forceinline__ static void run(const float* A, int lda, const char* Bp, int wave, int lane,
                                               const EpiArgs& e, const Pre& pre, const float* AX = nullptr, int ldx = 0) {
        gemmh_wg<G, NC, KB32, PW, MODE, XS2>(A, lda, Bp, wave, lane, e, pre, AX, ldx);
    }
};

template <int KB>
__device__ __forceinline__ BPre<1> out_prefetch(const float* Bp, int lane) {
    const BSrc s = bsrc<1, KB>(Bp, 0, lane);
    BPre<1> pre;
    pre.b0[0] = s.load(0);
    pre.b1[0] = s.load(1);
    return pre;
}

template <int KB, int NCOL, class Epi>
__device__ __forceinline__ void gemm_out(const float* A, int lda, const float* Bp, int wave, int lane, Epi epi,
                                         const BPre<1>& pre) {
    using T = GemmTile<1, 1, TM_VALU, 1, KB, false>;
    static_assert(KB % 2 == 0, "k-blocks in pairs");
    lane = opaque(lane);
    T g;
    g.acc[0][0] = f32x4{0.f, 0.f, 0.f, 0.f};
    g.tl[0][0] = 0.f;
    const int rl = lane & 15, kq = (lane >> 4) * 4;
    g.aoff[0] = (wave * 16 + rl) * lda + kq;
    g.toff[0] = (R - R % 16 + wave) * lda + kq;
    const BSrc src = bsrc<1, KB>(Bp, 0, lane);
    const int soff[1] = {src.voff};
    f32x4 a0[1], t0[1], b0[1] = {pre.b0[0]}, a1[1], t1[1], b1[1] = {pre.b1[0]};
    g.loadA(a0, t0, A, 0);
    g.loadA(a1, t1, A, 1);
#pragma unroll 1
    for (int kb = 0; kb < KB - 2; kb += 2) {
        g.mma(a0, t0, b0);
        T::loadB(b0, src, soff, kb + 2);
        g.loadA(a0, t0, A, kb + 2);
        g.mma(a1, t1, b1);
        T::loadB(b1, src, soff, kb + 3);
        g.loadA(a1, t1, A, kb + 3);
    }
    g.mma(a0, t0, b0);
    g.mma(a1, t1, b1);
    const float tv = sum4rows(g.tl[0][0]);
    if (rl < NCOL) {
#pragma unroll
        for (int r = 0; r < 4; ++r) epi(wave * 16 + kq + r, rl, g.acc[0][0][r]);
        if (kq == 0) epi(R - R % 16 + wave, rl, tv);
    }
}
__device__ __forceinline__ float row_sum(float v) {
    v += row_ror<8>(v);
    v += row_ror<4>(v);
    v += row_ror<2>(v);
    return v + row_ror<1>(v);
}

__device__ __forceinline__ float quad_sum(float v) {
    v += __builtin_bit_cast(float, __builtin_amdgcn_update_dpp(__builtin_bit_cast(int, v), __builtin_bit_cast(int, v),
                                                               0xB1, 0xf, 0xf, false));
    return v + __builtin_bit_cast(float, __builtin_amdgcn_update_dpp(__builtin_bit_cast(int, v), __builtin_bit_cast(int, v),
                                                                     0x4E, 0xf, 0xf, false));
}
template <bool POSEMAP = false, bool AFFINE = true>
__device__ __forceinline__ void layer_norm(const float* src, float* dst, const float* gain, const float* shift,
                                           int tid) {
    tid = opaque(tid);
    const int w = tid >> 6, lane = tid & 63;
    constexpr int LNC = D / 16, LNT = D / 32;
    static_assert(!POSEMAP || R == 68, "pose-mapped LayerNorm: 4-pose tiles");
    constexpr float RD = 1.0f / (float)D, RD1 = 1.0f / (float)(D - 1);
    constexpr int RM = R - R % 16, RT = R % 16;
    static_assert((RM == 64 && RT == 4) || (RM == 32 && RT == 2), "row tiles + one tail row per wave");
    if constexpr (RM != 64)
        if (w >= RT) return;
    const int row = (POSEMAP ? w * J : w * 16) + (lane >> 2), part = lane & 3;
    const int trow = POSEMAP ? w * J + 16 : RM + w;
    const float* s = src + row * LDX;
    const int tl = lane & 15;
    const float* st = src + trow * LDX;
    f32x4 v[LNC], gv[LNC], sv[LNC];
    f32x2 u[LNT], tg[LNT], tsh[LNT];
#pragma unroll
    for (int e = 0; e < LNC; ++e) v[e] = *reinterpret_cast<const f32x4*>(s + 4 * (part + 4 * e));
#pragma unroll
    for (int e = 0; e < LNT; ++e) u[e] = *reinterpret_cast<const f32x2*>(st + 2 * tl + 32 * e);
    const float c0 = s[0], tc0 = st[0];
    if constexpr (AFFINE) {
#pragma unroll
        for (int e = 0; e < LNC; ++e) {
            gv[e] = *reinterpret_cast<const f32x4*>(gain + 4 * (part + 4 * e));
            sv[e] = *reinterpret_cast<const f32x4*>(shift + 4 * (part + 4 * e));
        }
#pragma unroll
        for (int e = 0; e < LNT; ++e) {
            tg[e] = *reinterpret_cast<const f32x2*>(gain + 2 * tl + 32 * e);
            tsh[e] = *reinterpret_cast<const f32x2*>(shift + 2 * tl + 32 * e);
        }
    }
    f32x4 d1 = {0.f, 0.f, 0.f, 0.f}, d2 = {0.f, 0.f, 0.f, 0.f};
    const f32x2 nc0 = vpair(-c0);
#pragma unroll
    for (int e = 0; e < LNC; ++e) {
        const f32x4 d = padd4(v[e], nc0);
        d1 += d;
        d2 = __builtin_elementwise_fma(d, d, d2);
    }
    f32x2 e1 = {0.f, 0.f}, e2 = {0.f, 0.f};
    const f32x2 ntc0 = vpair(-tc0);
#pragma unroll
    for (int e = 0; e < LNT; ++e) {
        const f32x2 d = u[e] + ntc0;
        e1 += d;
        e2 = __builtin_elementwise_fma(d, d, e2);
    }
    const float s1 = quad_sum((d1[0] + d1[1]) + (d1[2] + d1[3]));
    const float s2 = quad_sum((d2[0] + d2[1]) + (d2[2] + d2[3]));
    const float t1 = row_sum(e1[0] + e1[1]);
    const float t2 = row_sum(e2[0] + e2[1]);
    const float mean = fmaf(s1, RD, c0), tmean = fmaf(t1, RD, tc0);
    const float var = fmaxf(fmaf(-s1 * RD, s1, s2), 0.f) * RD1;
    const float tvar = fmaxf(fmaf(-t1 * RD, t1, t2), 0.f) * RD1;
    const float den = __builtin_amdgcn_sqrtf(var) + LN_EPS, tden = __builtin_amdgcn_sqrtf(tvar) + LN_EPS;
    const float rcp = rcp_nr(den), trcp = rcp_nr(tden);
    const f32x2 nmean = vpair(-mean), rcpp = vpair(rcp);
    const f32x2 ntmean = vpair(-tmean), trcpp = vpair(trcp);
    float* d = dst + row * LDX;
#pragma unroll
    for (int e = 0; e < LNC; ++e) {
        const int c = 4 * (part + 4 * e);
        f32x4 t;
        if constexpr (!AFFINE) t = pmul4(padd4(v[e], nmean), rcpp);
        else t = __builtin_elementwise_fma(padd4(v[e], nmean), pmul4(gv[e], rcpp), sv[e]);
        *reinterpret_cast<f32x4*>(d + c) = t;
    }
    float* dt = dst + trow * LDX;
#pragma unroll
    for (int e = 0; e < LNT; ++e) {
        const int c = 2 * tl + 32 * e;
        f32x2 t;
        if constexpr (!AFFINE) t = (u[e] + ntmean) * trcpp;
        else t = __builtin_elementwise_fma(u[e] + ntmean, tg[e] * trcpp, tsh[e]);
        if (lane < 16) *reinterpret_cast<f32x2*>(dt + c) = t;
    }
}

__device__ __forceinline__ s16x4 bf4(float a, float b, float c, float d) {
    typedef unsigned u32x2 __attribute__((ext_vector_type(2)));
    const unsigned lo = __builtin_bit_cast(unsigned, __builtin_convertvector(f32x2{a, b}, bf16x2));
    const unsigned hi = __builtin_bit_cast(unsigned, __builtin_convertvector(f32x2{c, d}, bf16x2));
    return __builtin_bit_cast(s16x4, u32x2{lo, hi});
}

template <int GA = 0, class Hook = NoHook>
__device__ __forceinline__ void attention_mma(const float* qkv, float* out, unsigned mask, int wave, int lane,
                                              const Hook& hook = Hook{}) {
    static_assert(GA == 0 || DK == 24, "bf16 attention: d_k 24");
    constexpr bool A16 = GA == 2;
    lane = opaque(lane);
    constexpr int WPP = NW / P, HW = NH / WPP;
    static_assert(WPP * P == NW && HW * WPP == NH, "waves per pose");
    wave = opaque_s(wave);
    const int pose = WPP == 1 ? wave : wave / WPP;
    const int hoff = WPP == 1 ? 0 : (wave % WPP) * HW * DK;
    if (pose >= P) return;
    const int g = lane >> 4, c = lane & 15;
    constexpr float LOG2E = 1.4426950408889634f;
    const float sl = (1.0f / SQRT_DK) * LOG2E;
    const float* prow = qkv + pose * J * LD2 + hoff;
    float* orow = out + pose * J * LDX + hoff;
    const bool kok16 = ((mask >> 16) & 1u) != 0u;
    bool kokr[4];
#pragma unroll
    for (int r = 0; r < 4; ++r) kokr[r] = ((mask >> (4 * g + r)) & 1u) != 0u;
    auto scale = [&](float dot, bool ok) { return fmaf(dot, ok ? sl : 0.f, ok ? 0.f : -1e9f); };
    auto ex = [&](float x) { return __builtin_amdgcn_exp2f(x); };
    f32x4 q4[HW], k4[HW], Q4[HW], K4[HW], V4a[HW], V4b[HW];
    f32x2 q2[HW], k2[HW], Q2[HW], K2[HW];
    f32x4 qh[HW], kh[HW], Qh[HW], Kh[HW];
    float va[HW][4], vb[HW][4];
#pragma unroll
    for (int h = 0; h < HW; ++h) {
        const float* rc = prow + h * DK + c * LD2;
        const float* r16 = prow + h * DK + 16 * LD2;
        q4[h] = *reinterpret_cast<const f32x4*>(rc + 4 * g);
        k4[h] = *reinterpret_cast<const f32x4*>(rc + D + 4 * g);
        Q4[h] = *reinterpret_cast<const f32x4*>(r16 + 4 * g);
        K4[h] = *reinterpret_cast<const f32x4*>(r16 + D + 4 * g);
        if constexpr (GA == 2 || DK == 32) {
            const int o2 = 16 + 4 * (DK == 32 ? g : (g & 1));
            qh[h] = *reinterpret_cast<const f32x4*>(rc + o2);
            kh[h] = *reinterpret_cast<const f32x4*>(rc + D + o2);
            Qh[h] = *reinterpret_cast<const f32x4*>(r16 + o2);
            Kh[h] = *reinterpret_cast<const f32x4*>(r16 + D + o2);
            if constexpr (DK == 24) Kh[h] = g < 2 ? Kh[h] : f32x4{0.f, 0.f, 0.f, 0.f};
        } else if constexpr (DK == 24) {
            q2[h] = *reinterpret_cast<const f32x2*>(rc + 16 + 2 * g);
            k2[h] = *reinterpret_cast<const f32x2*>(rc + D + 16 + 2 * g);
            Q2[h] = *reinterpret_cast<const f32x2*>(r16 + 16 + 2 * g);
            K2[h] = *reinterpret_cast<const f32x2*>(r16 + D + 16 + 2 * g);
        }
    }
    f32x4 st[HW], st16[HW];
    f32x4 sk16[HW], skk[HW];
#pragma unroll
    for (int h = 0; h < HW; ++h) {
        st[h] = f32x4{0.f, 0.f, 0.f, 0.f};
        st16[h] = f32x4{0.f, 0.f, 0.f, 0.f};
    }
    auto load_v = [&]() {
#pragma unroll
        for (int h = 0; h < HW; ++h) {
            const float* vbase = prow + h * DK + 2 * D;
#pragma unroll
            for (int r = 0; r < 4; ++r) {
                va[h][r] = vbase[(4 * g + r) * LD2 + c];
                if constexpr (DK == 32) {
                    vb[h][r] = vbase[(4 * g + r) * LD2 + 16 + c];
                } else if constexpr (DK == 24) {
                    const float v1 = vbase[(4 * g + r) * LD2 + 16 + (c & 7)];
                    vb[h][r] = c < 8 ? v1 : 1.0f;
                } else {
                    vb[h][r] = 1.0f;
                }
            }
            V4a[h] = *reinterpret_cast<const f32x4*>(vbase + 16 * LD2 + 4 * g);
            if constexpr (DK == 24) V4b[h] = *reinterpret_cast<const f32x4*>(vbase + 16 * LD2 + 16 + 4 * (g & 1));
            if constexpr (DK == 32) V4b[h] = *reinterpret_cast<const f32x4*>(vbase + 16 * LD2 + 16 + 4 * g);
        }
    };
    if constexpr (GA == 2) {
#pragma unroll
        for (int h = 0; h < HW; ++h) {
            AFr<2> fk, fq, fQ;
            acvt<2>(k4[h], kh[h], fk);
            acvt<2>(q4[h], qh[h], fq);
            acvt<2>(Q4[h], Qh[h], fQ);
            if constexpr (DK == 24) {
                typedef unsigned u32x4 __attribute__((ext_vector_type(4)));
                u32x4 kw = __builtin_bit_cast(u32x4, fk.h);
                kw[2] = g < 2 ? kw[2] : 0u;
                kw[3] = g < 2 ? kw[3] : 0u;
                fk.h = __builtin_bit_cast(f16x8, kw);
            }
            const bf16x8 kb = __builtin_bit_cast(bf16x8, fk.h);
            st[h] = __builtin_amdgcn_mfma_f32_16x16x32_bf16(kb, __builtin_bit_cast(bf16x8, fq.h), st[h], 0, 0, 0);
            st16[h] = __builtin_amdgcn_mfma_f32_16x16x32_bf16(kb, __builtin_bit_cast(bf16x8, fQ.h), st16[h], 0, 0, 0);
            if constexpr (A16) {
                AFr<2> fK;
                acvt<2>(K4[h], Kh[h], fK);
                const bf16x8 k16 = __builtin_bit_cast(bf16x8, fK.h);
                const f32x4 z4 = {0.f, 0.f, 0.f, 0.f};
                sk16[h] = __builtin_amdgcn_mfma_f32_16x16x32_bf16(k16, __builtin_bit_cast(bf16x8, fq.h), z4, 0, 0, 0);
                skk[h] = __builtin_amdgcn_mfma_f32_16x16x32_bf16(k16, __builtin_bit_cast(bf16x8, fQ.h), z4, 0, 0, 0);
            }
        }
    } else {
#pragma unroll
    for (int m = 0; m < DK / 4; ++m)
#pragma unroll
        for (int h = 0; h < HW; ++h) {
            const float kk = m < 4 ? k4[h][m & 3] : DK == 32 ? kh[h][m & 3] : k2[h][m & 1];
            const float qq = m < 4 ? q4[h][m & 3] : DK == 32 ? qh[h][m & 3] : q2[h][m & 1];
            const float QQ = m < 4 ? Q4[h][m & 3] : DK == 32 ? Qh[h][m & 3] : Q2[h][m & 1];
            st[h] = __builtin_amdgcn_mfma_f32_16x16x4f32(kk, qq, st[h], 0, 0, 0);
            st16[h] = __builtin_amdgcn_mfma_f32_16x16x4f32(kk, QQ, st16[h], 0, 0, 0);
        }
    }
    if constexpr (!__is_same(Hook, NoHook)) {
        __builtin_amdgcn_sched_barrier(0);
        hook();
        __builtin_amdgcn_sched_barrier(0);
    }
    load_v();
    float s_c16[HW], s_1616[HW];
    if constexpr (A16) {
#pragma unroll
        for (int h = 0; h < HW; ++h) {
            s_c16[h] = scale(sk16[h][0], kok16);
            s_1616[h] = scale(skk[h][0], kok16);
        }
    } else {
#pragma unroll
    for (int h = 0; h < HW; ++h) {
        float pa = 0.f, pc = 0.f;
#pragma unroll
        for (int m = 0; m < 4; ++m) {
            pa = fmaf(q4[h][m], K4[h][m], pa);
            pc = fmaf(Q4[h][m], K4[h][m], pc);
        }
        if constexpr (GA == 2 || DK == 32) {
#pragma unroll
            for (int m = 0; m < 4; ++m) {
                pa = fmaf(qh[h][m], Kh[h][m], pa);
                pc = fmaf(Qh[h][m], Kh[h][m], pc);
            }
        } else if constexpr (DK == 24) {
#pragma unroll
            for (int m = 0; m < 2; ++m) {
                pa = fmaf(q2[h][m], K2[h][m], pa);
                pc = fmaf(Q2[h][m], K2[h][m], pc);
            }
        }
        s_c16[h] = pa;
        s_1616[h] = pc;
    }
#pragma unroll
    for (int h = 0; h < HW; ++h) {
        sum4rows2(s_c16[h], s_1616[h]);
        s_c16[h] = scale(s_c16[h], kok16);
        s_1616[h] = scale(s_1616[h], kok16);
    }
    }
    float p[HW][4], p16[HW], u[HW][4], u16[HW], mx[HW], my[HW];
#pragma unroll
    for (int h = 0; h < HW; ++h) {
#pragma unroll
        for (int r = 0; r < 4; ++r) {
            p[h][r] = scale(st[h][r], kokr[r]);
            u[h][r] = scale(st16[h][r], kokr[r]);
        }
    }
    float big = 0.f, big2 = 0.f;
#pragma unroll
    for (int h = 0; h < HW; ++h) {
#pragma unroll
        for (int r = 0; r < 4; ++r) big = fmaxf(big, fmaxf(fabsf(st[h][r]), fabsf(st16[h][r])));
        big2 = fmaxf(big2, fmaxf(fabsf(s_c16[h]), fabsf(s_1616[h])));
    }
    big = fmaxf(big * sl, big2);
    const bool shift = (mask & ((1u << J) - 1u)) == 0u || __builtin_amdgcn_ballot_w64(!(big <= 64.f)) != 0;
    if (!shift) {
#pragma unroll
        for (int h = 0; h < HW; ++h) {
#pragma unroll
            for (int r = 0; r < 4; ++r) {
                p[h][r] = ex(p[h][r]);
                u[h][r] = ex(u[h][r]);
            }
            p16[h] = ex(s_c16[h]);
            u16[h] = ex(s_1616[h]);
        }
    } else {
#pragma unroll
    for (int h = 0; h < HW; ++h) {
        mx[h] = fmaxf(fmaxf(p[h][0], p[h][1]), fmaxf(p[h][2], p[h][3]));
        my[h] = fmaxf(fmaxf(u[h][0], u[h][1]), fmaxf(u[h][2], u[h][3]));
    }
#pragma unroll
    for (int h = 0; h < HW; ++h) {
        max4rows2(mx[h], my[h]);
        mx[h] = fmaxf(mx[h], s_c16[h]);
        my[h] = fmaxf(my[h], s_1616[h]);
    }
#pragma unroll
    for (int h = 0; h < HW; ++h) {
#pragma unroll
        for (int r = 0; r < 4; ++r) {
            p[h][r] = ex(p[h][r] - mx[h]);
            u[h][r] = ex(u[h][r] - my[h]);
        }
        p16[h] = ex(s_c16[h] - mx[h]);
        u16[h] = ex(s_1616[h] - my[h]);
    }
    }
    f32x4 oa[HW], ob[HW];
    f32x4 oa16[HW], ob16[HW];
    float ya[HW], yb[HW];
#pragma unroll
    for (int h = 0; h < HW; ++h) {
        oa[h] = f32x4{0.f, 0.f, 0.f, 0.f};
        ob[h] = f32x4{0.f, 0.f, 0.f, 0.f};
        ya[h] = 0.f;
        yb[h] = 0.f;
    }
    if constexpr (GA == 2) {
#pragma unroll
        for (int h = 0; h < HW; ++h) {
            const s16x4 pb = bf4(p[h][0], p[h][1], p[h][2], p[h][3]);
            const s16x4 vab = bf4(va[h][0], va[h][1], va[h][2], va[h][3]), vbb = bf4(vb[h][0], vb[h][1], vb[h][2], vb[h][3]);
            oa[h] = __builtin_amdgcn_mfma_f32_16x16x16bf16_1k(vab, pb, oa[h], 0, 0, 0);
            ob[h] = __builtin_amdgcn_mfma_f32_16x16x16bf16_1k(vbb, pb, ob[h], 0, 0, 0);
            if constexpr (A16) {
                const s16x4 ub = bf4(u[h][0], u[h][1], u[h][2], u[h][3]);
                const f32x4 z4 = {0.f, 0.f, 0.f, 0.f};
                oa16[h] = __builtin_amdgcn_mfma_f32_16x16x16bf16_1k(vab, ub, z4, 0, 0, 0);
                ob16[h] = __builtin_amdgcn_mfma_f32_16x16x16bf16_1k(vbb, ub, z4, 0, 0, 0);
            }
        }
    } else {
#pragma unroll
    for (int r = 0; r < 4; ++r)
#pragma unroll
        for (int h = 0; h < HW; ++h) {
            oa[h] = __builtin_amdgcn_mfma_f32_16x16x4f32(va[h][r], p[h][r], oa[h], 0, 0, 0);
            ob[h] = __builtin_amdgcn_mfma_f32_16x16x4f32(vb[h][r], p[h][r], ob[h], 0, 0, 0);
        }
    }
    if constexpr (!A16) {
        __builtin_amdgcn_sched_barrier(0);
#pragma unroll
        for (int r = 0; r < 4; ++r)
#pragma unroll
            for (int h = 0; h < HW; ++h) {
                ya[h] = fmaf(u[h][r], va[h][r], ya[h]);
                yb[h] = fmaf(u[h][r], vb[h][r], yb[h]);
            }
#pragma unroll
        for (int h = 0; h < HW; ++h) sum4rows2(ya[h], yb[h]);
    }
    float rs[HW], rs16[HW];
    if constexpr (DK == 24) mfma_pad<PAD_MFMA16>(ob);
    if constexpr (A16) mfma_pad<PAD_MFMA16>(ob16);
#pragma unroll
    for (int h = 0; h < HW; ++h) {
        float den, den16;
        if constexpr (DK == 32) {
            float sp = (p[h][0] + p[h][1]) + (p[h][2] + p[h][3]), su = (u[h][0] + u[h][1]) + (u[h][2] + u[h][3]);
            sum4rows2(sp, su);
            den = sp + p16[h];
            den16 = su + u16[h];
        } else if constexpr (DK == 24) {
            float sa = ob[h][0], sb = ob[h][0];
            asm("s_nop 1\n\tv_permlane32_swap_b32 %0, %1" : "+v"(sa), "+v"(sb));
            den = (g < 2 ? sb : ob[h][0]) + p16[h];
            if constexpr (A16) {
                float ta = ob16[h][0], tb = ob16[h][0];
                asm("s_nop 1\n\tv_permlane32_swap_b32 %0, %1" : "+v"(ta), "+v"(tb));
                den16 = (g < 2 ? tb : ob16[h][0]) + u16[h];
            } else {
                const float yr = row_ror<8>(yb[h]);
                den16 = (c < 8 ? yr : yb[h]) + u16[h];
            }
        } else {
            den = ob[h][0] + p16[h];
            den16 = yb[h] + u16[h];
        }
        rs[h] = __builtin_amdgcn_rcpf(den);
        rs16[h] = __builtin_amdgcn_rcpf(den16);
    }
#pragma unroll
    for (int h = 0; h < HW; ++h) {
        const f32x4 p4 = {p16[h], p16[h], p16[h], p16[h]};
        oa[h] = __builtin_elementwise_fma(p4, V4a[h], oa[h]) * rs[h];
        const float* v16 = prow + h * DK + 16 * LD2 + 2 * D;
        const int col = h * DK;
        *reinterpret_cast<f32x4*>(orow + c * LDX + col + 4 * g) = oa[h];
        if constexpr (A16) {
            const f32x4 u4 = {u16[h], u16[h], u16[h], u16[h]};
            const f32x4 o16a = __builtin_elementwise_fma(u4, V4a[h], oa16[h]) * rs16[h];
            const f32x4 o16b = __builtin_elementwise_fma(u4, V4b[h], ob16[h]) * rs16[h];
            if (c == 0) *reinterpret_cast<f32x4*>(orow + 16 * LDX + col + 4 * g) = o16a;
            if (c == 0 && g < 2) *reinterpret_cast<f32x4*>(orow + 16 * LDX + col + 16 + 4 * g) = o16b;
        } else if (g == 0) {
            orow[16 * LDX + col + c] = fmaf(u16[h], v16[c], ya[h]) * rs16[h];
        }
        if constexpr (DK == 24) {
            ob[h] = __builtin_elementwise_fma(p4, V4b[h], ob[h]) * rs[h];
            if (g < 2) *reinterpret_cast<f32x4*>(orow + c * LDX + col + 16 + 4 * g) = ob[h];
            if (!A16 && g == 1 && c < 8) orow[16 * LDX + col + 16 + c] = fmaf(u16[h], v16[16 + c], yb[h]) * rs16[h];
        } else if constexpr (DK == 32) {
            ob[h] = __builtin_elementwise_fma(p4, V4b[h], ob[h]) * rs[h];
            *reinterpret_cast<f32x4*>(orow + c * LDX + col + 16 + 4 * g) = ob[h];
            if (g == 1) orow[16 * LDX + col + 16 + c] = fmaf(u16[h], v16[16 + c], yb[h]) * rs16[h];
        }
    }
}


template <bool SPARSE, bool XSKIP = false>
__device__ __forceinline__ void cheb_prep(const float* __restrict__ cw, const float* src, float* b2, int wave,
                                          int lane) {
    lane = opaque(lane);
    constexpr int WPP = NW / P, G = 2, ng = D / G / WPP;
    static_assert(ng <= 64 && P <= NW, "one pose per wave, one column pair per lane");
    wave = opaque_s(wave);
    const int p = WPP == 1 ? wave : wave / WPP;
    if (p >= P || lane >= ng) return;
    const int c = lane * G + (WPP == 1 ? 0 : (wave % WPP) * (D / WPP));
    const float* sp = src + opaque(p * J * LDX + c);
    float* dp = b2 + opaque(p * J * LD2 + c);
    f32x2 v[J];
#pragma unroll
    for (int i = 0; i < J; ++i) v[i] = *reinterpret_cast<const f32x2*>(sp + i * LDX);
    auto lx = [&](int j, const f32x2 (&u)[J]) {
        f32x2 acc = {0.f, 0.f};
        if constexpr (SPARSE) {
#pragma unroll
            for (int k = 0; k < SPAT.n1[j]; ++k) acc = pfma(splat2(cw[SPAT.o1[j] + k]), u[SPAT.c1[j][k]], acc);
        } else {
#pragma unroll
            for (int i = 0; i < J; ++i) acc = pfma(splat2(cw[j * J + i]), u[i], acc);
        }
        return acc;
    };
    f32x2 t1[J];
#pragma unroll
    for (int j = 0; j < J; ++j) t1[j] = lx(j, v);
#pragma unroll
    for (int j = 0; j < J; ++j) {
        const f32x2 t2 = pfma(splat2(2.0f), lx(j, t1), -v[j]);
        if constexpr (XSKIP) {
            *reinterpret_cast<f32x2*>(dp + j * LD2 + D) = t1[j];
            *reinterpret_cast<f32x2*>(dp + j * LD2 + 2 * D) = t2;
        } else {
            *reinterpret_cast<f32x2*>(dp + j * LD2) = t1[j];
            *reinterpret_cast<f32x2*>(dp + j * LD2 + D) = t2;
            *reinterpret_cast<f32x2*>(dp + j * LD2 + 2 * D) = v[j];
        }
    }
}

struct GFrag {
    float lb[5], l16[5];
    f32x4 b4[NCD];
    float b1[2];
    bf16x8 lh;
    bf16x8 ll;
    float m16[5];
};
__device__ __forceinline__ GFrag gfrag_load(const float* __restrict__ LF, int lane) {
    GFrag f;
#pragma unroll
    for (int s = 0; s < 5; ++s) {
        f.lb[s] = LF[s * 64 + lane];
        f.l16[s] = LF[(5 + s) * 64 + lane];
    }
    return f;
}
__device__ __forceinline__ GFrag gfrag_load_h(const float* __restrict__ LG, int lane) {
    GFrag f;
    const int g = lane >> 4, cl = lane & 15;
    const float* Lr = LG + cl * J + 4 * g;
    const float* L16 = LG + 16 * J + 4 * g;
    f32x4 lo, hi = {0.f, 0.f, 0.f, 0.f};
#pragma unroll
    for (int e = 0; e < 4; ++e) {
        lo[e] = Lr[e];
        f.m16[e] = L16[e];
    }
    const float l_c16 = LG[cl * J + 16], l_1616 = LG[16 * J + 16];
    hi[0] = g == 0 ? l_c16 : 0.f;
    f.m16[4] = g == 0 ? l_1616 : 0.f;
    AFr<2> fr;
    acvt<2>(lo, hi, fr);
    f.lh = __builtin_bit_cast(bf16x8, fr.h);
    const bf16x8 h = f.lh;
    f32x4 rlo, rhi;
#pragma unroll
    for (int e = 0; e < 4; ++e) {
        rlo[e] = lo[e] - (float)h[e];
        rhi[e] = hi[e] - (float)h[4 + e];
    }
    AFr<2> fl;
    acvt<2>(rlo, rhi, fl);
    f.ll = __builtin_bit_cast(bf16x8, fl.h);
    return f;
}
__device__ __forceinline__ void gbias_load(GFrag& f, const float* __restrict__ bias, int lane, int wave) {
    constexpr int TW = NCD / (NW / P);
    if constexpr (TW < NCD) bias += 16 * TW * (wave & 1);
    const int g = lane >> 4, cl = lane & 15;
#pragma unroll
    for (int t = 0; t < NCD; ++t)
        f.b4[t] = t < TW ? *reinterpret_cast<const f32x4*>(bias + 16 * t + 4 * g) : f32x4{0.f, 0.f, 0.f, 0.f};
    f.b1[0] = TW == 6 ? bias[16 * g + cl] : 0.f;
    f.b1[1] = TW == 6 ? bias[16 * (4 + (g & 1)) + cl] : 0.f;
}

template <bool RESID, int GA = 0, class Hook = NoHook>
__device__ __forceinline__ void graph_mma(const GFrag& f, const float* src, float* dst,
                                          const float* __restrict__ bias, int wave, int lane, const Hook& hook = Hook{}) {
    lane = opaque(lane);
    constexpr int WPP = NW / P, TW = NCD / WPP;
    static_assert(TW == 6 || TW == 4 || TW == 3, "graph_mma: 3, 4 or 6 column tiles per wave");
    static_assert(GA == 0 || GA == 2, "fp32 or bf16 graph product");
    wave = opaque_s(wave);
    const int pose = WPP == 1 ? wave : wave / WPP;
    const int t0 = WPP == 1 ? 0 : (wave % WPP) * TW;
    if (pose >= P) return;
    const int g = lane >> 4, cl = lane & 15;
    const float(&lb)[5] = f.lb;
    const float(&l16)[5] = f.l16;
    const float* xp = src + pose * J * LDX + cl + 16 * t0;
    const int row_j = pose * J + cl, row16 = pose * J + 16;
    const int c16a = 16 * (t0 + (TW == 3 ? min(g, 2) : g)) + cl, c16b = 16 * (4 + (g & 1)) + cl;
    f32x4 old[TW];
    float old16a = 0.f, old16b = 0.f, b16a = 0.f;
    if constexpr (RESID) {
#pragma unroll
        for (int t = 0; t < TW; ++t) old[t] = *reinterpret_cast<const f32x4*>(dst + row_j * LDX + 16 * (t0 + t) + 4 * g);
        old16a = dst[row16 * LDX + c16a];
        if constexpr (TW == 6) old16b = dst[row16 * LDX + c16b];
        else b16a = bias[c16a];
    }
    f32x4 acc[TW];
    float p16[TW];
    const f32x4 z = {0.f, 0.f, 0.f, 0.f};
    if constexpr (GA != 0) {
        f32x4 xa[TW];
        float x16[TW];
#pragma unroll
        for (int t = 0; t < TW; ++t) {
#pragma unroll
            for (int e = 0; e < 4; ++e) xa[t][e] = xp[(4 * g + e) * LDX + 16 * t];
            x16[t] = xp[16 * LDX + 16 * t];
        }
#pragma unroll
        for (int t = 0; t < TW; ++t) {
            AFr<2> fx;
            acvt<2>(xa[t], f32x4{g == 0 ? x16[t] : 0.f, 0.f, 0.f, 0.f}, fx);
            acc[t] = __builtin_amdgcn_mfma_f32_16x16x32_bf16(__builtin_bit_cast(bf16x8, fx.h), f.lh, z, 0, 0, 0);
            acc[t] = __builtin_amdgcn_mfma_f32_16x16x32_bf16(__builtin_bit_cast(bf16x8, fx.h), f.ll, acc[t], 0, 0, 0);
        }
        __builtin_amdgcn_sched_barrier(0);
        hook();
        __builtin_amdgcn_sched_barrier(0);
#pragma unroll
        for (int t = 0; t < TW; ++t) {
            float v = f.m16[4] * x16[t];
#pragma unroll
            for (int e = 0; e < 4; ++e) v = fmaf(f.m16[e], xa[t][e], v);
            p16[t] = v;
        }
    } else {
        float a[TW][5];
#pragma unroll
        for (int s = 0; s < 5; ++s) {
            const int row = min(4 * s + g, J - 1);
#pragma unroll
            for (int t = 0; t < TW; ++t) a[t][s] = xp[row * LDX + 16 * t];
        }
#pragma unroll
        for (int s = 0; s < 5; ++s)
#pragma unroll
            for (int t = 0; t < TW; ++t) acc[t] = __builtin_amdgcn_mfma_f32_16x16x4f32(a[t][s], lb[s], s == 0 ? z : acc[t], 0, 0, 0);
        __builtin_amdgcn_sched_barrier(0);
        hook();
        __builtin_amdgcn_sched_barrier(0);
#pragma unroll
        for (int s = 0; s < 5; ++s)
#pragma unroll
            for (int t = 0; t < TW; ++t) p16[t] = s == 0 ? l16[0] * a[t][0] : fmaf(l16[s], a[t][s], p16[t]);
    }
#pragma unroll
    for (int t = 0; t < TW; ++t) {
        const int c0 = 16 * (t0 + t) + 4 * g;
        if constexpr (RESID) {
            *reinterpret_cast<f32x4*>(dst + row_j * LDX + c0) = old[t] + (acc[t] + f.b4[t]);
        } else {
            *reinterpret_cast<f32x4*>(dst + row_j * LDX + c0) = acc[t];
        }
    }
    if constexpr (TW == 6) {
        const float va = rs4rows(p16[0], p16[1], p16[2], p16[3]);
        const float vb = rs4rows(p16[4], p16[5], p16[4], p16[5]);
        if constexpr (RESID) {
            dst[row16 * LDX + c16a] = old16a + (va + f.b1[0]);
            if (g < 2) dst[row16 * LDX + c16b] = old16b + (vb + f.b1[1]);
        } else {
            dst[row16 * LDX + c16a] = va;
            if (g < 2) dst[row16 * LDX + c16b] = vb;
        }
    } else if constexpr (TW == 4) {
        const float va = rs4rows(p16[0], p16[1], p16[2], p16[3]);
        if constexpr (RESID) dst[row16 * LDX + c16a] = old16a + (va + b16a);
        else dst[row16 * LDX + c16a] = va;
    } else {
        const float va = rs4rows(p16[0], p16[1], p16[2], p16[2]);
        if (g < 3) {
            if constexpr (RESID) dst[row16 * LDX + c16a] = old16a + (va + b16a);
            else dst[row16 * LDX + c16a] = va;
        }
    }
}

template <bool SPARSE>
__device__ __forceinline__ void input_prep(const float* __restrict__ cw, const float* xst, float* b1, int tid) {
    tid = opaque(tid);
    if (tid >= P * CIN) return;
    const int p = tid / CIN, c = tid - p * CIN;
    float v[J];
#pragma unroll
    for (int i = 0; i < J; ++i) v[i] = xst[(p * J + i) * CIN + c];
#pragma unroll
    for (int j = 0; j < J; ++j) {
        float a1 = 0.f, a2 = 0.f;
        if constexpr (SPARSE) {
#pragma unroll
            for (int k = 0; k < SPAT.n1[j]; ++k) a1 = fmaf(cw[SPAT.o1[j] + k], v[SPAT.c1[j][k]], a1);
#pragma unroll
            for (int k = 0; k < SPAT.n2[j]; ++k) a2 = fmaf(cw[SPAT.nnz1 + SPAT.o2[j] + k], v[SPAT.c2[j][k]], a2);
        } else {
#pragma unroll
            for (int i = 0; i < J; ++i) {
                a1 = fmaf(cw[j * J + i], v[i], a1);
                a2 = fmaf(cw[J * J + j * J + i], v[i], a2);
            }
        }
        float* rowp = b1 + (p * J + j) * LDX;
        rowp[c] = v[j];
        rowp[CIN + c] = a1;
        rowp[2 * CIN + c] = a2;
        if (c == 0) rowp[3 * CIN] = 0.f;
    }
}

__device__ __forceinline__ float swishf(float x) { return x * (1.0f / (1.0f + expf(-x))); }

__global__ void __launch_bounds__(256) temb_kernel(const float* __restrict__ tw, const float* __restrict__ tvals,
                                                   int tstride, float* __restrict__ tproj) {
    __shared__ float emb[D];
    __shared__ float h0[E];
    __shared__ float h1[E];
    const int tid = threadIdx.x;
    const float t = tvals[(size_t)blockIdx.x * tstride];
    const float neg_scale = -(float)(9.210340371976184 / (double)(D / 2 - 1));
    if (tid < D) {
        const int k = tid < D / 2 ? tid : tid - D / 2;
        const float f = expf((float)k * neg_scale);
        const float arg = t * f;
        emb[tid] = tid < D / 2 ? sinf(arg) : cosf(arg);
    }
    __syncthreads();
    for (int o = tid; o < E; o += 256) {
        float acc = 0.f;
        for (int k = 0; k < D; ++k) acc = fmaf(emb[k], tw[TOFF_W0 + k * E + o], acc);
        h0[o] = swishf(acc + tw[TOFF_B0 + o]);
    }
    __syncthreads();
    for (int o = tid; o < E; o += 256) {
        float acc = 0.f;
        for (int k = 0; k < E; ++k) acc = fmaf(h0[k], tw[TOFF_W1 + k * E + o], acc);
        h1[o] = swishf(acc + tw[TOFF_B1 + o]);
    }
    __syncthreads();
    for (int o = tid; o < NL * D; o += 256) {
        const int l = o / D, c = o - l * D;
        const float* wp = tw + TOFF_WP + (size_t)l * E * D;
        float acc = 0.f;
        for (int k = 0; k < E; ++k) acc = fmaf(h1[k], wp[k * D + c], acc);
        tproj[(size_t)blockIdx.x * NL * D + o] = acc + tw[TOFF_BP + o];
    }
}

constexpr unsigned SPL_RUN = 1u, SPL_PUB = 2u, SPL_ABANDON = 3u;
constexpr int SPL_IDLE_POLLS = 4096;

__device__ __forceinline__ bool split_claim(const SampleArgs& a, int j, int tid) {
    __shared__ int ok;
    if (tid == 0) {
        if (a.split_dbg == 1)
            for (int it = 0; it < 30000; ++it) __builtin_amdgcn_s_sleep(127);
        const unsigned run = (a.token << 2) | SPL_RUN, ab = (a.token << 2) | SPL_ABANDON;
        int res = -1;
        while (res < 0) {
            unsigned v = __hip_atomic_load(a.flags + j, __ATOMIC_RELAXED, __HIP_MEMORY_SCOPE_AGENT);
            if (v == ab) {
                __hip_atomic_store(a.flags + j, 0u, __ATOMIC_RELAXED, __HIP_MEMORY_SCOPE_AGENT);
                res = 0;
            } else if (__hip_atomic_compare_exchange_strong(a.flags + j, &v, run, __ATOMIC_RELAXED, __ATOMIC_RELAXED,
                                                            __HIP_MEMORY_SCOPE_AGENT)) {
                res = 1;
            }
        }
        ok = res;
    }
    __syncthreads();
    return ok != 0;
}
__device__ __forceinline__ void split_publish(const SampleArgs& a, int j, int tid) {
    __builtin_amdgcn_fence(__ATOMIC_RELEASE, "agent");
    __syncthreads();
    if (tid == 0)
        __hip_atomic_store(a.flags + j, (a.token << 2) | SPL_PUB, __ATOMIC_RELEASE, __HIP_MEMORY_SCOPE_AGENT);
}
__device__ __forceinline__ bool split_wait(const SampleArgs& a, int j, int tid) {
    __shared__ int ok;
    if (tid == 0) {
        const unsigned run = (a.token << 2) | SPL_RUN, pub = (a.token << 2) | SPL_PUB;
        const unsigned ab = (a.token << 2) | SPL_ABANDON;
        int idle = a.split_dbg ? 0 : SPL_IDLE_POLLS;
        int res = -1;
        while (res < 0) {
            unsigned v = __hip_atomic_load(a.flags + j, __ATOMIC_ACQUIRE, __HIP_MEMORY_SCOPE_AGENT);
            if (v == pub) {
                __hip_atomic_store(a.flags + j, 0u, __ATOMIC_RELAXED, __HIP_MEMORY_SCOPE_AGENT);
                res = 1;
            } else if (v == run || idle > 0) {
                if (v != run) --idle;
                __builtin_amdgcn_s_sleep(64);
            } else if (__hip_atomic_compare_exchange_strong(a.flags + j, &v, ab, __ATOMIC_ACQUIRE, __ATOMIC_RELAXED,
                                                            __HIP_MEMORY_SCOPE_AGENT)) {
                if (a.split_stats) __hip_atomic_fetch_add(a.split_stats, 1, __ATOMIC_RELAXED, __HIP_MEMORY_SCOPE_AGENT);
                res = 0;
            }
        }
        ok = res;
    }
    __syncthreads();
    __builtin_amdgcn_fence(__ATOMIC_ACQUIRE, "agent");
    return ok != 0;
}

template <int MODE, bool SPARSE, int G16, int ZM = 0>
__global__ void __launch_bounds__(NT, 1) sample_kernel(SampleArgs a, const float* __restrict__ arena,
                                                               const char* __restrict__ arena16) {
    constexpr bool EPS_MODE = MODE == M_EPS;
    constexpr bool POSE = MODE == M_POSE;
    __shared__ __attribute__((aligned(16))) float sm[SM_FLOATS];
    float* XS = sm + SM_XS;
    float* B1 = sm + SM_B1;
    float* B2 = sm + SM_B2;
    float* XST = sm + SM_XST;
    float* LNP = sm + SM_LNP;

    const int tid = threadIdx.x, lane = tid & 63;
    const int wave = __builtin_amdgcn_readfirstlane(tid >> 6);
    int tile = blockIdx.x, s_beg = 0, s_end = MODE == M_SAMPLE ? a.K : 1, half = 0;
    if constexpr (MODE == M_SAMPLE) {
        if (a.split_n) {
            const int b = blockIdx.x, n = a.split_n;
            if (b < n) {
                tile = a.split_full + b;
                s_end = a.split_k;
                half = 1;
            } else if (b < n + a.split_full) {
                tile = b - n;
            } else {
                tile = a.split_full + (b - n - a.split_full);
                s_beg = a.split_k;
                half = 2;
            }
        }
    }
    const int pose0 = a.pose_off + tile * P;
    const int npose = min(P, a.N - pose0);
    const int nvalid = npose * PE;
    const float* W = arena;
    const float* CW = SPARSE ? W + OFF_CHEBS : sm + SM_TC;
    unsigned kmask = a.mask;
    if (a.pmask) kmask = a.pmask[min(pose0 + wave / (NW / P), a.N - 1)];

    if constexpr (POSE) {
        for (int i = tid; i < R * CIN; i += NT) {
            const int row = i / CIN, c = i - row * CIN;
            XST[i] = (c < CIN_POSE && row < npose * J) ? a.x_in[((size_t)pose0 * J + row) * CIN_POSE + c] : 0.f;
        }
    } else {
        const float* src = a.x_in;
        if constexpr (MODE == M_SAMPLE) {
            if (half == 1 && !split_claim(a, tile - a.split_full, tid)) return;
            if (half == 2) {
                if (split_wait(a, tile - a.split_full, tid)) src = a.x_out;
                else s_beg = 0;
            }
        }
        for (int i = tid; i < R * CIN; i += NT) XST[i] = i < nvalid ? src[(size_t)pose0 * PE + i] : 0.f;
    }
    static_assert(OFF_LN0B == OFF_LN0A + D && OFF_LN1A == OFF_LN0A + 2 * D && OFF_LN1B == OFF_LN0A + 3 * D, "LN block");
    for (int i = tid; i < NL * 4 * D; i += NT) LNP[i] = W[(i / (4 * D)) * LAYER_FLOATS + OFF_LN0A + i % (4 * D)];
    for (int i = tid; i < 2 * J * J; i += NT) sm[SM_TC + i] = W[OFF_CHEB + i];
    if constexpr (SPARSE)
        for (int i = tid; i < CHEBT_FLOATS; i += NT)
            reinterpret_cast<int*>(sm)[SM_TS + i] = reinterpret_cast<const int*>(W)[OFF_CHEBT + i];
    __syncthreads();

#if DPK_TRACE
    if ((tid & 63) == 0) {
        ::dpk::tr_row[wave] = nullptr;
        ::dpk::tr_ix[wave] = 0;
    }
#define DPK_STAMP()                                                                                       \
    do {                                                                                                  \
        if ((tid & 63) == 0)                                                                              \
            ::dpk::tr_row[wave] = (a.trace && s == a.trace_step)                                                 \
                               ? a.trace + ((size_t)blockIdx.x * NW + wave) * TRACE_SLOTS                 \
                               : nullptr;                                                                 \
        ::dpk::tr_stamp();                                                                                       \
    } while (0)
#define BAR()          \
    do {               \
        DPK_STAMP();   \
        __syncthreads(); \
        DPK_STAMP();   \
    } while (0)
#else
#define BAR() __syncthreads()
#endif
#pragma unroll 1
    for (int s = s_beg; s < s_end; ++s) {
        {
            const BPre<NCD / 2> pre = gemm_prefetch<NCD, 1>(W + OFF_WIN, wave, lane);
            input_prep<SPARSE>(CW, XST, B1, tid);
            BAR();
            const EpiArgs e{XS, LDX, W + OFF_BIN, nullptr, 0, pose0, a.N - 1};
            gemm_wg<NCD, 1, E_STORE>(B1, LDX, W + OFF_WIN, wave, lane, e, pre);
        }
        BAR();

#pragma unroll 1
        for (int l = 0; l < a.num_layers; ++l) {
            const float* LW = W + l * LAYER_FLOATS;
            constexpr int GH = G16 ? G16 : 1;
            const char* LH = arena16 + offh<GH>(l, 0);
            constexpr int PWQ = G16 == 2 ? 9 : DPK_PWQ16;
            constexpr int PWF = G16 == 2 ? 6 : DPK_PWF16;
            constexpr int GG = G16 == 2 ? 2 : 0;
            {
                const EpiArgs e{B2, LD2, LW + OFF_CQKV, nullptr, 0, pose0, a.N - 1};
                using HQ = HGemm<GH, 3 * NCD, KB32_D, PWQ>;
                BPre<3 * NCD / 2> pre;
                typename HQ::Pre preh;
                if constexpr (G16 == 0 && !DPK_LATE(1)) pre = gemm_prefetch<3 * NCD, KB_D, DPK_QKV_NPRE>(LW + OFF_QKV, wave, lane);
                if (DPK_RUN(8)) layer_norm<false, false>(XS, B1, LNP + l * 4 * D, LNP + l * 4 * D + D, tid);
                if constexpr (G16) {
                    __builtin_amdgcn_sched_barrier(0);
                    preh = HQ::prefetch(LH + O16_QKV / GH, wave, lane);
                } else if constexpr (DPK_LATE(1)) {
                    __builtin_amdgcn_sched_barrier(0);
                    pre = gemm_prefetch<3 * NCD, KB_D, DPK_QKV_NPRE>(LW + OFF_QKV, wave, lane);
                }
                BAR();
                if (DPK_RUN(16 | 32)) {
                    if constexpr (G16) HQ::template run<E_STORE>(B1, LDX, LH + O16_QKV / GH, wave, lane, e, preh);
                    else gemm_wg<3 * NCD, KB_D, E_STORE, false, DPK_QKV_NPRE>(B1, LDX, LW + OFF_QKV, wave, lane, e, pre);
                }
            }
            BAR();
            {
                const EpiArgs e{XS, LDX, LW + OFF_BO, nullptr, 0, pose0, a.N - 1};
                using HO = HGemm<GH, NCD, KB32_D, 3>;
                BPre<NCD / 2> pre;
                typename HO::Pre preh;
                auto o_pre = [&]() {
                    if constexpr (G16) preh = HO::prefetch(LH + O16_O / GH, wave, lane);
                    else pre = gemm_prefetch<NCD, KB_D>(LW + OFF_O, wave, lane);
                };
                if constexpr (!DPK_LATE(2) && !DPK_MID(2)) o_pre();
                if (DPK_RUN(1)) {
                    if constexpr (DPK_MID(2)) attention_mma<GG>(B2, B1, kmask, wave, lane, o_pre);
                    else attention_mma<GG>(B2, B1, kmask, wave, lane);
                }
                if constexpr (DPK_LATE(2)) {
                    __builtin_amdgcn_sched_barrier(0);
                    o_pre();
                }
                BAR();
                if (DPK_RUN(16 | 64)) {
                    if constexpr (G16) HO::template run<E_RESID>(B1, LDX, LH + O16_O / GH, wave, lane, e, preh);
                    else gemm_wg<NCD, KB_D, E_RESID>(B1, LDX, LW + OFF_O, wave, lane, e, pre);
                }
            }
            BAR();
            GFrag gb;
            gbias_load(gb, LW + OFF_BFC2, lane, wave);
            {
                using HF = HGemm<GH, 2 * NCD, KB32_D, PWF>;
                BPre<NCD> pre;
                typename HF::Pre preh;
                auto f_pre = [&]() {
                    if constexpr (G16) preh = HF::prefetch(LH + O16_FC1 / GH, wave, lane);
                    else pre = gemm_prefetch<2 * NCD, KB_D, DPK_FC1_NPRE>(LW + OFF_FC1, wave, lane);
                };
                constexpr bool FC1_MID = DPK_MID(4) && R == 68;
                if constexpr (!DPK_LATE(4) && !FC1_MID) f_pre();
                const GFrag gf = GG != 0 ? gfrag_load_h(LW + OFF_LG, lane) : gfrag_load(LW + OFF_LGF, lane);
                if constexpr (R == 68) {
                    if (DPK_RUN(8)) layer_norm<true>(XS, B1, LNP + l * 4 * D + 2 * D, LNP + l * 4 * D + 3 * D, tid);
                    asm volatile("" ::: "memory");
                    if constexpr (FC1_MID) {
                        if (DPK_RUN(2)) graph_mma<false, GG>(gf, B1, B1, nullptr, wave, lane, f_pre);
                    } else if (DPK_RUN(2)) graph_mma<false, GG>(gf, B1, B1, nullptr, wave, lane);
                } else {
                    if (DPK_RUN(8)) layer_norm(XS, B1, LNP + l * 4 * D + 2 * D, LNP + l * 4 * D + 3 * D, tid);
                    BAR();
                    if (DPK_RUN(2)) graph_mma<false, GG>(gf, B1, B1, nullptr, wave, lane);
                }
                if constexpr (DPK_LATE(4) && !FC1_MID) {
                    __builtin_amdgcn_sched_barrier(0);
                    f_pre();
                }
                BAR();
                if (DPK_RUN(16 | 128)) {
                    const EpiArgs e{B2, LD2, LW + OFF_BFC1, nullptr, 0, pose0, a.N - 1};
                    if constexpr (G16) HF::template run<E_STORE_RELU>(B1, LDX, LH + O16_FC1 / GH, wave, lane, e, preh);
                    else gemm_wg<2 * NCD, KB_D, E_STORE_RELU, false, DPK_FC1_NPRE>(B1, LDX, LW + OFF_FC1, wave, lane, e, pre);
                }
            }
            GFrag gf2 = GG != 0 ? gfrag_load_h(LW + OFF_LG, lane) : gfrag_load(LW + OFF_LGF, lane);
#pragma unroll
            for (int t = 0; t < NCD; ++t) gf2.b4[t] = gb.b4[t];
            gf2.b1[0] = gb.b1[0];
            gf2.b1[1] = gb.b1[1];
            {
                const EpiArgs e{B1, LDX, nullptr, nullptr, 0, pose0, a.N - 1};
                if constexpr (G16) {
                    using H2 = HGemm<GH, NCD, KB32_D2, 3>;
                    const typename H2::Pre pre = H2::prefetch(LH + O16_FC2 / GH, wave, lane);
                    BAR();
                    if (DPK_RUN(16 | 256)) H2::template run<E_STORE_NB>(B2, LD2, LH + O16_FC2 / GH, wave, lane, e, pre);
                } else {
                    const BPre<NCD / 2> pre = gemm_prefetch<NCD, KB_D2>(LW + OFF_FC2, wave, lane);
                    BAR();
                    if (DPK_RUN(16 | 256)) gemm_wg<NCD, KB_D2, E_STORE_NB>(B2, LD2, LW + OFF_FC2, wave, lane, e, pre);
                }
            }
            {
                const float* tp = a.tproj + (MODE == M_SAMPLE ? (size_t)s * NL * D : 0) + l * D;
                const EpiArgs e{B1, LDX, LW + OFF_BC1, tp, EPS_MODE ? NL * D : 0, pose0, a.N - 1};
                using HC = HGemm<GH, NCD, KB32_D3, 3>;
                BPre<NCD / 2> pre;
                typename HC::Pre preh;
                auto c1_pre = [&]() {
                    if constexpr (G16) preh = HC::prefetch(LH + O16_C1 / GH, wave, lane);
                    else pre = gemm_prefetch<NCD, KB_D3>(LW + OFF_C1, wave, lane);
                };
                if constexpr (!DPK_LATE(8) && !DPK_MID(8)) c1_pre();
                BAR();
                if constexpr (DPK_MID(8)) {
                    if (DPK_RUN(2)) graph_mma<true, GG>(gf2, B1, XS, LW + OFF_BFC2, wave, lane, c1_pre);
                } else if (DPK_RUN(2)) graph_mma<true, GG>(gf2, B1, XS, LW + OFF_BFC2, wave, lane);
                if (DPK_RUN(4)) cheb_prep<SPARSE, true>(CW, XS, B2, wave, lane);
                if constexpr (DPK_LATE(8)) {
                    __builtin_amdgcn_sched_barrier(0);
                    c1_pre();
                }
                BAR();
                if (DPK_RUN(16 | 512)) {
                    if constexpr (G16) HC::template run<E_CHEB1, true>(B2, LD2, LH + O16_C1 / GH, wave, lane, e, preh, XS, LDX);
                    else gemm_wg<NCD, KB_D3, E_CHEB1, true>(B2, LD2, LW + OFF_C1, wave, lane, e, pre, XS, LDX);
                }
            }
            {
                const EpiArgs e{XS, LDX, LW + OFF_BC2, nullptr, 0, pose0, a.N - 1};
                using HC = HGemm<GH, NCD, KB32_D3, 3>;
                BPre<NCD / 2> pre;
                typename HC::Pre preh;
                auto c2_pre = [&]() {
                    if constexpr (G16) preh = HC::prefetch(LH + O16_C2 / GH, wave, lane);
                    else pre = gemm_prefetch<NCD, KB_D3>(LW + OFF_C2, wave, lane);
                };
                if constexpr (!DPK_LATE(16)) c2_pre();
                BAR();
                if (DPK_RUN(4)) cheb_prep<SPARSE, true>(CW, B1, B2, wave, lane);
                if constexpr (DPK_LATE(16)) {
                    __builtin_amdgcn_sched_barrier(0);
                    c2_pre();
                }
                BAR();
                if (DPK_RUN(16 | 1024)) {
                    if constexpr (G16) HC::template run<E_RESID_RELU, true>(B2, LD2, LH + O16_C2 / GH, wave, lane, e, preh, B1, LDX);
                    else gemm_wg<NCD, KB_D3, E_RESID_RELU, true>(B2, LD2, LW + OFF_C2, wave, lane, e, pre, B1, LDX);
                }
            }
            BAR();
        }
        constexpr int COUTK = POSE ? COUT_POSE : COUT;
        constexpr int NOUT = P * J * COUTK, NIT = (NOUT + NT - 1) / NT;
        const BPre<1> preo = out_prefetch<KB_D>(W + OFF_WOUT, lane);
        float bo[NIT];
#pragma unroll
        for (int k = 0; k < NIT; ++k) bo[k] = W[OFF_BOUT + (tid + k * NT) % COUTK];
        if (wave < R / 16)
            gemm_out<KB_D, 3 * COUTK>(XS, LDX, W + OFF_WOUT, wave, lane,
                                      [&](int r, int c, float v) { B2[r * LD2 + c] = v; }, preo);
        BAR();
        {
            float cf[5] = {0.f, 0.f, 0.f, 0.f, 0.f};
            if constexpr (MODE == M_SAMPLE) {
                const float* cfp = a.coef + s * 6;
#pragma unroll
                for (int i = 0; i < 5; ++i) cf[i] = cfp[i];
            }
            const float* T1d = sm + SM_TC;
            const float* T2d = T1d + J * J;
            const int tid_o = opaque(tid);
#pragma unroll
            for (int k = 0; k < NIT; ++k) {
                const int idx = tid_o + k * NT;
                if (idx >= NOUT) break;
                const int p = idx / (J * COUTK), rem = idx - p * (J * COUTK);
                const int j = rem / COUTK, c = rem - j * COUTK;
                const float* yp = B2 + p * J * LD2;
                float a1 = 0.f, a2 = 0.f;
                if constexpr (SPARSE) {
                    typedef int i32x2 __attribute__((ext_vector_type(2)));
                    const i32x2* ts = reinterpret_cast<const i32x2*>(sm + SM_TS) + j * (SPT1 + SPT2);
#pragma unroll
                    for (int q = 0; q < SPT1; ++q) {
                        const i32x2 e = ts[q];
                        a1 = fmaf(__builtin_bit_cast(float, e[0]), yp[e[1] + COUTK + c], a1);
                    }
#pragma unroll
                    for (int q = 0; q < SPT2; ++q) {
                        const i32x2 e = ts[SPT1 + q];
                        a2 = fmaf(__builtin_bit_cast(float, e[0]), yp[e[1] + 2 * COUTK + c], a2);
                    }
                } else {
#pragma unroll
                    for (int i = 0; i < J; ++i) {
                        a1 = fmaf(T1d[j * J + i], yp[i * LD2 + COUTK + c], a1);
                        a2 = fmaf(T2d[j * J + i], yp[i * LD2 + 2 * COUTK + c], a2);
                    }
                }
                const float et = ((yp[j * LD2 + c] + a1) + a2) + bo[k];
                const int r = p * J + j;
                const int oidx = r * CIN + c;
                const bool valid = oidx < nvalid;
                const size_t gidx = (size_t)pose0 * PE + oidx;
                if (POSE) {
                    B1[r * LDX + c] = et;
                } else if (EPS_MODE) {
                    if (valid) a.x_out[gidx] = et;
                } else {
                    float z = 0.f;
                    if constexpr (ZM == 1) z = valid ? a.noise[(size_t)s * a.N * PE + gidx] : 0.f;
                    else z = a.eta != 0.f ? normal_noise(a.seed, s, (long long)gidx) : 0.f;
                    float x0, xn;
                    ddim_elem(cf, XST[oidx], et, z, x0, xn);
                    XST[oidx] = xn;
                    if (valid) {
                        if (a.x0s) a.x0s[(size_t)s * a.N * PE + gidx] = x0;
                        if (a.xs) a.xs[(size_t)(s + 1) * a.N * PE + gidx] = xn;
                    }
                }
            }
        }
        BAR();
    }
    if constexpr (MODE == M_SAMPLE) {
        for (int i = tid; i < nvalid; i += NT) a.x_out[(size_t)pose0 * PE + i] = XST[i];
        if (half == 1) split_publish(a, tile - a.split_full, tid);
    } else if constexpr (POSE) {
        if (a.x_out)
            for (int i = tid; i < npose * J * COUT_POSE; i += NT) {
                const int row = i / COUT_POSE, c = i - row * COUT_POSE;
                a.x_out[(size_t)pose0 * J * COUT_POSE + i] = B1[row * LDX + c];
            }
        if (a.uvxyz)
            for (int i = tid; i < npose * PE; i += NT) {
                const int row = i / CIN, c = i - row * CIN;
                float v;
                if (c < CIN_POSE) {
                    v = XST[i];
                } else {
                    const float raw = B1[row * LDX + (c - CIN_POSE)];
                    const int j = row % J;
                    if (a.root_mode == 0) v = j == 0 ? 0.f : raw;
                    else if (a.root_mode == 1) v = raw - B1[(row - j) * LDX + (c - CIN_POSE)];
                    else v = raw;
                }
                for (int hh = 0; hh < a.H; ++hh) a.uvxyz[((size_t)hh * a.N + pose0) * PE + i] = v;
            }
    }
}

#undef BAR
#undef DPK_STAMP
```

diffpose-nw_amd/diffpose_amd/_lib.py:

```python
from __future__ import annotations

import ctypes
import os

_HERE = os.path.dirname(os.path.abspath(__file__))
LIB_PATH = os.environ.get("DPK_LIB", os.path.join(_HERE, "libdpk.so"))

DPK_OK = 0
ERRORS = {-1: "DPK_E_INVALID", -2: "DPK_E_UNSUPPORTED", -3: "DPK_E_HIP", -4: "DPK_E_STATE", -5: "DPK_E_WEIGHTS"}

EXPORTS = ("dpk_version", "dpk_create", "dpk_set_graph", "dpk_load_weights", "dpk_set_mask", "dpk_set_pose_masks",
           "dpk_set_schedule", "dpk_eps", "dpk_sample", "dpk_sample_noise", "dpk_ddim_update", "dpk_ddim_update_noise",
           "dpk_pose", "dpk_pose_metrics", "dpk_gmm_sample", "dpk_gmm_sample_f64", "dpk_set_gemm_mode",
           "dpk_set_tail_plan", "dpk_debug_split", "dpk_debug_resources", "dpk_profile", "dpk_profile_read",
           "dpk_kernel_geometry", "dpk_last_error", "dpk_destroy")


class DpkConfig(ctypes.Structure):
    _fields_ = [("hid_dim", ctypes.c_int), ("num_layers", ctypes.c_int), ("n_head", ctypes.c_int),
                ("n_pts", ctypes.c_int), ("coords_in", ctypes.c_int), ("coords_out", ctypes.c_int),
                ("device", ctypes.c_int)]


class DpkError(RuntimeError):
    def __init__(self, fn: str, code: int, msg: str = ""):
        super().__init__(f"{fn} failed: {ERRORS.get(code, code)} {msg}".strip())
        self.code = code


_LIB = None


def lib() -> ctypes.CDLL:
    global _LIB
    if _LIB is not None:
        return _LIB
    if not os.path.exists(LIB_PATH):
        raise ImportError(f"libdpk.so not found at {LIB_PATH}: build it with `python __graft_entry__.py` "
                          "(build()) or `make -C diffpose-nw_amd`; there is no CPU fallback")
    import torch

    L = ctypes.CDLL(LIB_PATH)
    if "DPK_LIB" in os.environ:
        class _Partial:
            def __init__(self, lib):
                self._lib = lib

            def __getattr__(self, name):
                try:
                    return getattr(self._lib, name)
                except AttributeError:
                    return lambda *a: -2
        L = _Partial(L)
    vp, i32, i64, u64, fp = ctypes.c_void_p, ctypes.c_int, ctypes.c_int64, ctypes.c_uint64, ctypes.POINTER(ctypes.c_float)
    L.dpk_version.restype = i32
    L.dpk_create.argtypes = [ctypes.POINTER(DpkConfig), ctypes.POINTER(vp)]
    L.dpk_set_graph.argtypes = [vp, fp]
    L.dpk_load_weights.argtypes = [vp, ctypes.POINTER(ctypes.c_char_p), ctypes.POINTER(fp), ctypes.POINTER(i64), i32]
    L.dpk_set_mask.argtypes = [vp, ctypes.POINTER(ctypes.c_uint8)]
    L.dpk_set_pose_masks.argtypes = [vp, vp, i32]
    L.dpk_set_schedule.argtypes = [vp, fp, i32, ctypes.POINTER(i32), i32, ctypes.c_float]
    L.dpk_eps.argtypes = [vp, vp, vp, vp, i32, vp]
    L.dpk_sample.argtypes = [vp, vp, vp, vp, vp, i32, u64, vp]
    L.dpk_sample_noise.argtypes = [vp, vp, vp, vp, vp, i32, u64, vp, vp]
    L.dpk_ddim_update.argtypes = [vp, vp, vp, vp, vp, i64, i32, u64, vp]
    L.dpk_ddim_update_noise.argtypes = [vp, vp, vp, vp, vp, i64, i32, u64, vp, vp]
    L.dpk_debug_split.argtypes = [vp, i32, ctypes.POINTER(i32)]
    L.dpk_debug_resources.argtypes = [vp, ctypes.POINTER(i32), i32]
    L.dpk_pose.argtypes = [vp, vp, vp, vp, i32, i32, i32, vp]
    L.dpk_pose_metrics.argtypes = [vp, vp, i32, i32, i32, vp, vp, vp, vp]
    L.dpk_gmm_sample.argtypes = [vp, vp, i32, i32, vp, i32, vp, u64, ctypes.c_double, vp, vp, vp, vp]
    L.dpk_gmm_sample_f64.argtypes = [vp, vp, i32, i32, vp, i32, vp, u64, ctypes.c_double, vp, vp, vp, vp]
    L.dpk_set_gemm_mode.argtypes = [vp, i32]
    L.dpk_set_tail_plan.argtypes = [vp, i32]
    L.dpk_profile.argtypes = [vp, i32]
    L.dpk_profile_read.argtypes = [vp, fp, i32, ctypes.POINTER(i32)]
    L.dpk_kernel_geometry.argtypes = [ctypes.POINTER(i32)] * 3
    L.dpk_last_error.argtypes = [vp]
    L.dpk_last_error.restype = ctypes.c_char_p
    L.dpk_destroy.argtypes = [vp]
    L.dpk_destroy.restype = None
    for name in EXPORTS:
        if name in ("dpk_last_error", "dpk_destroy"):
            continue
        getattr(L, name).restype = i32
    _LIB = L
    return L


def check(handle, fn: str, rc: int) -> None:
    if rc != DPK_OK:
        msg = ""
        if handle:
            raw = lib().dpk_last_error(handle)
            msg = raw.decode() if raw else ""
        raise DpkError(fn, rc, msg)


def kernel_geometry():
    L = lib()
    a, b, c = ctypes.c_int(), ctypes.c_int(), ctypes.c_int()
    L.dpk_kernel_geometry(ctypes.byref(a), ctypes.byref(b), ctypes.byref(c))
    return {"poses_per_workgroup": a.value, "threads_per_workgroup": b.value, "lds_bytes": c.value}
```

diffpose-nw_amd/diffpose_amd/gcndiff.py:

```python
from __future__ import annotations

import ctypes

import numpy as np
import torch

from . import _lib
from .schedule import alpha_bar_table
from .weights import HID, N_HEAD, N_LAYERS, N_PTS, COORDS, normalize_state_dict

H36M_EDGES = ((0, 1), (1, 2), (2, 3), (0, 4), (4, 5), (5, 6), (0, 7), (7, 8), (8, 9), (9, 10),
              (8, 11), (11, 12), (12, 13), (8, 14), (14, 15), (15, 16))


def adj_mx_from_edges(num_pts: int = N_PTS, edges=H36M_EDGES) -> np.ndarray:
    a = np.zeros((num_pts, num_pts), dtype=np.float32)
    for i, j in np.asarray(edges, dtype=np.int64).reshape(-1, 2):
        a[i, j] = 1.0
        a[j, i] = 1.0
    a += np.eye(num_pts, dtype=np.float32)
    inv = np.power(a.sum(1, dtype=np.float32), -1).astype(np.float32)
    inv[np.isinf(inv)] = 0.0
    return (inv[:, None] * a).astype(np.float32)


def _f32p(a: np.ndarray):
    return a.ctypes.data_as(ctypes.POINTER(ctypes.c_float))


def _dev_index(device) -> int:
    if device is None:
        return torch.cuda.current_device()
    d = torch.device(device)
    if d.type != "cuda":
        raise ValueError(f"HipGCNdiff runs on a HIP device, got {d}")
    return torch.cuda.current_device() if d.index is None else d.index


def _model_dims(config, default_coords=COORDS):
    if config is None:
        return HID, N_LAYERS, N_HEAD, N_PTS, tuple(default_coords)
    m = getattr(config, "model", config)
    return (int(m.hid_dim), int(m.num_layer), int(m.n_head), int(m.n_pts), tuple(int(c) for c in m.coords_dim))


class _HipModel:

    KIND = "diff"
    DEFAULT_COORDS = COORDS

    def __init__(self, adj, config=None, device=None):
        hid, nl, nh, npts, coords = _model_dims(config, self.DEFAULT_COORDS)
        self.device = torch.device("cuda", _dev_index(device))
        L = _lib.lib()
        cfg = _lib.DpkConfig(hid, nl, nh, npts, coords[0], coords[1], self.device.index)
        h = ctypes.c_void_p()
        rc = L.dpk_create(ctypes.byref(cfg), ctypes.byref(h))
        _lib.check(None, "dpk_create", rc)
        self._h = h
        self.n_pts = npts
        self.num_layer = nl
        self.hid_dim = hid
        self.n_head = nh
        self.coords_dim = tuple(coords)
        adj = adj.detach().cpu().numpy() if torch.is_tensor(adj) else np.asarray(adj)
        self.adj = np.ascontiguousarray(adj, dtype=np.float32)
        if self.adj.shape != (npts, npts):
            raise ValueError(f"adj must be ({npts},{npts}), got {self.adj.shape}")
        _lib.check(h, "dpk_set_graph", L.dpk_set_graph(h, _f32p(self.adj)))
        self._mask_key = None
        self._mask_ref = None
        self._pose_bits = None
        self._mask_hold = []
        self._sched_key = None
        self.training = False

    def load_state_dict(self, state_dict, strict: bool = True):
        sd = normalize_state_dict(state_dict, kind=self.KIND, n_layers=self.num_layer, hid=self.hid_dim,
                                  n_pts=self.n_pts, coords=self.coords_dim)
        names = list(sd.keys())
        arrs = [np.ascontiguousarray(sd[k], dtype=np.float32) for k in names]
        c_names = (ctypes.c_char_p * len(names))(*[k.encode() for k in names])
        c_ptrs = (ctypes.POINTER(ctypes.c_float) * len(arrs))(*[_f32p(a) for a in arrs])
        c_num = (ctypes.c_int64 * len(arrs))(*[a.size for a in arrs])
        L = _lib.lib()
        _lib.check(self._h, "dpk_load_weights", L.dpk_load_weights(self._h, c_names, c_ptrs, c_num, len(arrs)))
        self._state = sd
        return self

    def eval(self):
        self.training = False
        return self

    def train(self, mode: bool = True):
        if mode:
            raise NotImplementedError(f"{type(self).__name__} is inference-only (training is out of scope, "
                                      "SURVEY §8f f4)")
        return self.eval()

    def to(self, *a, **k):
        return self

    def cuda(self, *a, **k):
        return self

    def parameters(self):
        return iter(())

    def set_mask(self, mask) -> None:
        L = _lib.lib()
        if torch.is_tensor(mask) or isinstance(mask, np.ndarray):
            shape = tuple(mask.shape)
            if len(shape) == 3 and shape[0] != 1:
                if shape[1:] != (1, self.n_pts):
                    raise ValueError(f"a per-pose mask must be (N, 1, {self.n_pts}), got {shape}")
                mt = torch.as_tensor(mask).to(self.device)
                words = (mt.reshape(shape[0], self.n_pts) != 0).to(torch.int32)
                shifts = torch.arange(self.n_pts, device=self.device, dtype=torch.int32)
                bits = (words << shifts).sum(dim=1, dtype=torch.int32).contiguous()
                _lib.check(self._h, "dpk_set_pose_masks", L.dpk_set_pose_masks(self._h, bits.data_ptr(), shape[0]))
                self._pose_bits = bits
                return
        if mask is None:
            m = np.ones(self.n_pts, dtype=np.uint8)
        else:
            mt = mask.detach().cpu() if torch.is_tensor(mask) else torch.as_tensor(np.asarray(mask))
            m = mt.reshape(-1).numpy().astype(np.uint8)
            if m.size != self.n_pts:
                raise ValueError(f"mask must have {self.n_pts} key entries, got {m.size}")
        m = np.ascontiguousarray(m)
        _lib.check(self._h, "dpk_set_mask", L.dpk_set_mask(self._h, m.ctypes.data_as(ctypes.POINTER(ctypes.c_uint8))))
        if self._pose_bits is not None:
            _lib.check(self._h, "dpk_set_pose_masks", L.dpk_set_pose_masks(self._h, None, 0))
            self._pose_bits = None

    def _check_mask_batch(self, n: int) -> None:
        if self._pose_bits is not None and self._pose_bits.numel() != n:
            raise ValueError(f"per-pose mask has {self._pose_bits.numel()} poses, the batch {n}")

    def _note_mask_use(self) -> None:
        bits = self._pose_bits
        if bits is None:
            return
        if torch.cuda.is_current_stream_capturing():
            if not any(b is bits for b in self._mask_hold):
                self._mask_hold.append(bits)
        else:
            bits.record_stream(torch.cuda.current_stream(self.device))

    def _sync_mask(self, mask) -> None:
        key = None if mask is None else (id(mask), getattr(mask, "_version", 0))
        if key is None or key != self._mask_key or mask is not self._mask_ref:
            self.set_mask(mask)
            self._mask_key = key
            self._mask_ref = mask

    def _check_x(self, x, channels: int | None = None):
        channels = self.coords_dim[0] if channels is None else channels
        if not (torch.is_tensor(x) and x.is_cuda and x.dtype == torch.float32):
            raise TypeError("x must be a float32 CUDA(HIP) tensor")
        if x.dim() != 3 or x.shape[1] != self.n_pts or x.shape[2] != channels:
            raise ValueError(f"x must be (N, {self.n_pts}, {channels}), got {tuple(x.shape)}")
        if x.device != self.device:
            raise ValueError(f"x on {x.device}, model on {self.device}")
        return x.contiguous()

    GEMM_MODES = {"fp32": 0, "f16x3": 1, "bf16": 2}

    def set_gemm_mode(self, mode: str = "fp32") -> None:
        if mode not in self.GEMM_MODES:
            raise ValueError(f"gemm mode must be one of {sorted(self.GEMM_MODES)}, got {mode!r}")
        _lib.check(self._h, "dpk_set_gemm_mode", _lib.lib().dpk_set_gemm_mode(self._h, self.GEMM_MODES[mode]))
        self.gemm_mode = mode

    TAIL_PLANS = {"four": 0, "two_pose": 1, "step_split": 2}

    def set_tail_plan(self, plan: str = "step_split") -> None:
        if plan not in self.TAIL_PLANS:
            raise ValueError(f"tail plan must be one of {sorted(self.TAIL_PLANS)}, got {plan!r}")
        _lib.check(self._h, "dpk_set_tail_plan", _lib.lib().dpk_set_tail_plan(self._h, self.TAIL_PLANS[plan]))

    def debug_split(self, mode: int = 0, read: bool = False):
        n = ctypes.c_int(0)
        _lib.check(self._h, "dpk_debug_split",
                   _lib.lib().dpk_debug_split(self._h, int(mode), ctypes.byref(n) if read else None))
        return n.value if read else None

    def debug_resources(self) -> dict:
        buf = (ctypes.c_int * 8)()
        _lib.check(self._h, "dpk_debug_resources", _lib.lib().dpk_debug_resources(self._h, buf, 8))
        keys = ("captures", "tracked", "released", "free_slots", "retired_schedules", "eps_spare_poses",
                "generic_loop_graphs", "generic_spare_kib")
        return dict(zip(keys, list(buf)))

    def profile(self, enable: bool = True) -> None:
        _lib.check(self._h, "dpk_profile", _lib.lib().dpk_profile(self._h, 1 if enable else 0))

    def kernel_times_ms(self):
        L = _lib.lib()
        cap = 4096
        buf = (ctypes.c_float * cap)()
        n = ctypes.c_int()
        _lib.check(self._h, "dpk_profile_read", L.dpk_profile_read(self._h, buf, cap, ctypes.byref(n)))
        return [buf[i] for i in range(min(n.value, cap))]

    def close(self):
        h, self._h = getattr(self, "_h", None), None
        if h:
            _lib.lib().dpk_destroy(h)
        self._mask_hold = []

    def __del__(self):
        try:
            self.close()
        except Exception:
            pass


class HipGCNdiff(_HipModel):

    def set_schedule(self, seq, betas, eta: float = 0.0) -> None:
        b = betas.detach().cpu().numpy() if torch.is_tensor(betas) else np.asarray(betas)
        b = np.ascontiguousarray(b, dtype=np.float32)
        seq = [int(s) for s in seq]
        key = (tuple(seq), b.tobytes(), float(eta))
        if key == self._sched_key:
            return
        abar = np.ascontiguousarray(alpha_bar_table(b))
        cseq = (ctypes.c_int * len(seq))(*seq)
        L = _lib.lib()
        _lib.check(self._h, "dpk_set_schedule",
                   L.dpk_set_schedule(self._h, _f32p(abar), abar.size, cseq, len(seq), ctypes.c_float(eta)))
        self._sched_key = key
        self.K = len(seq)

    def forward(self, x, mask, t, cemd=0):
        x = self._check_x(x)
        n = x.shape[0]
        t = torch.as_tensor(t, device=self.device).to(torch.float32).reshape(-1).contiguous()
        if t.numel() == 1 and n != 1:
            t = t.expand(n).contiguous()
        if t.numel() != n:
            raise ValueError(f"t must have {n} entries, got {t.numel()}")
        self._sync_mask(mask)
        self._check_mask_batch(n)
        self._note_mask_use()
        eps = torch.empty_like(x)
        stream = torch.cuda.current_stream(self.device).cuda_stream
        L = _lib.lib()
        _lib.check(self._h, "dpk_eps", L.dpk_eps(self._h, x.data_ptr(), t.data_ptr(), eps.data_ptr(), n, stream))
        return eps

    __call__ = forward

    def sample(self, x, seq, betas, eta: float = 0.0, mask=None, seed: int = 0, trajectory: bool = False,
               out=None, noise=None):
        x = self._check_x(x)
        self.set_schedule(seq, betas, eta)
        if noise is not None:
            shape = (self.K,) + tuple(x.shape)
            if not (torch.is_tensor(noise) and noise.is_cuda and noise.dtype == torch.float32
                    and tuple(noise.shape) == shape and noise.device == x.device):
                raise ValueError(f"noise must be a float32 tensor of shape {shape} on {x.device}")
            noise = noise.contiguous()
        self._sync_mask(mask)
        n = x.shape[0]
        self._check_mask_batch(n)
        self._note_mask_use()
        out = torch.empty_like(x) if out is None else out
        xs = x0s = None
        if trajectory:
            xs = torch.empty((self.K + 1,) + tuple(x.shape), dtype=x.dtype, device=x.device)
            x0s = torch.empty((self.K,) + tuple(x.shape), dtype=x.dtype, device=x.device)
        stream = torch.cuda.current_stream(self.device).cuda_stream
        L = _lib.lib()
        xs_p = xs.data_ptr() if xs is not None else None
        x0s_p = x0s.data_ptr() if x0s is not None else None
        seed_c = ctypes.c_uint64(seed & (2**64 - 1))
        if noise is None:
            rc = L.dpk_sample(self._h, x.data_ptr(), out.data_ptr(), xs_p, x0s_p, n, seed_c, stream)
        else:
            rc = L.dpk_sample_noise(self._h, x.data_ptr(), out.data_ptr(), xs_p, x0s_p, n, seed_c,
                                    noise.data_ptr(), stream)
        _lib.check(self._h, "dpk_sample", rc)
        if trajectory:
            return xs, x0s
        return out

    def ddim_update(self, xt, et, step: int, seed: int = 0, want_x0: bool = True, noise=None):
        xt, et = xt.contiguous(), et.contiguous()
        if noise is not None:
            if not (torch.is_tensor(noise) and noise.dtype == torch.float32 and noise.shape == xt.shape
                    and noise.device == xt.device):
                raise ValueError(f"noise must be a float32 tensor shaped like xt {tuple(xt.shape)} on {xt.device}")
            noise = noise.contiguous()
        xn = torch.empty_like(xt)
        x0 = torch.empty_like(xt) if want_x0 else None
        stream = torch.cuda.current_stream(xt.device).cuda_stream
        L = _lib.lib()
        rc = L.dpk_ddim_update_noise(self._h, xt.data_ptr(), et.data_ptr(), xn.data_ptr(),
                                     x0.data_ptr() if x0 is not None else None, xt.numel(), step,
                                     ctypes.c_uint64(seed & (2**64 - 1)),
                                     noise.data_ptr() if noise is not None else None, stream)
        _lib.check(self._h, "dpk_ddim_update", rc)
        return xn, x0



def GCNdiff(adj, config, device=None) -> HipGCNdiff:
    return HipGCNdiff(adj, config, device=device)
```

include/diffpose_kernels.h:

```cpp
#ifndef DIFFPOSE_KERNELS_H
#define DIFFPOSE_KERNELS_H

#include <stdint.h>

#ifdef __cplusplus
extern "C" {
#endif

#define DPK_OK              0
#define DPK_E_INVALID      -1
#define DPK_E_UNSUPPORTED  -2
#define DPK_E_HIP          -3
#define DPK_E_STATE        -4
#define DPK_E_WEIGHTS      -5

typedef struct dpk_handle dpk_handle;

typedef struct {
    int hid_dim;
    int num_layers;
    int n_head;
    int n_pts;
    int coords_in;
    int coords_out;
    int device;
} dpk_config;

int dpk_version(void);

int dpk_create(const dpk_config* cfg, dpk_handle** out);

int dpk_set_graph(dpk_handle* h, const float* adj_host);

int dpk_load_weights(dpk_handle* h, const char* const* names, const float* const* host_ptrs,
                     const int64_t* numels, int n);

int dpk_set_mask(dpk_handle* h, const uint8_t* mask_host);

int dpk_set_pose_masks(dpk_handle* h, const uint32_t* bits_dev, int n);

int dpk_set_schedule(dpk_handle* h, const float* alpha_bar, int n_alpha, const int* seq, int K, float eta);

int dpk_eps(dpk_handle* h, const float* x_dev, const float* t_dev, float* eps_dev, int N, void* stream);

int dpk_sample(dpk_handle* h, const float* x_dev, float* out_dev, float* xs_dev, float* x0s_dev,
               int N, uint64_t seed, void* stream);

int dpk_sample_noise(dpk_handle* h, const float* x_dev, float* out_dev, float* xs_dev, float* x0s_dev,
                     int N, uint64_t seed, const float* noise_dev, void* stream);

int dpk_ddim_update(dpk_handle* h, const float* xt_dev, const float* eps_dev, float* xnext_dev,
                    float* x0_dev, int64_t n_elems, int step, uint64_t seed, void* stream);

int dpk_ddim_update_noise(dpk_handle* h, const float* xt_dev, const float* eps_dev, float* xnext_dev,
                          float* x0_dev, int64_t n_elems, int step, uint64_t seed, const float* noise_dev,
                          void* stream);

int dpk_pose(dpk_handle* h, const float* x2d_dev, float* xyz_dev, float* uvxyz_dev, int N, int H,
             int root_mode, void* stream);

int dpk_pose_metrics(const float* out_uvxyz_dev, const float* targets_dev, int F, int H, int root_mode,
                     double* p1_dev, double* p2_dev, float* xyz_dev, void* stream);

int dpk_gmm_sample(const float* gmm_dev, const float* poses3d_dev, int n_src, int kernel_n,
                   const int64_t* index_dev, int F, const double* u_dev, uint64_t seed, double atol,
                   float* uvxyz_dev, float* noise_scale_dev, int* status_dev, void* stream);

int dpk_gmm_sample_f64(const double* gmm_dev, const double* poses3d_dev, int n_src, int kernel_n,
                       const int64_t* index_dev, int F, const double* u_dev, uint64_t seed, double atol,
                       float* uvxyz_dev, float* noise_scale_dev, int* status_dev, void* stream);

int dpk_set_gemm_mode(dpk_handle* h, int mode);

int dpk_set_tail_plan(dpk_handle* h, int plan);

int dpk_profile(dpk_handle* h, int enable);
int dpk_profile_read(dpk_handle* h, float* ms_out, int cap, int* count);

int dpk_debug_split(dpk_handle* h, int mode, int* fallbacks);
int dpk_debug_resources(dpk_handle* h, int* out, int n);

int dpk_kernel_geometry(int* poses_per_workgroup, int* threads_per_workgroup, int* lds_bytes);

const char* dpk_last_error(const dpk_handle* h);
void dpk_destroy(dpk_handle* h);

#ifdef __cplusplus
}
#endif
#endif
```

Measured before the change: 92920.

## Add 8-wave 4-pose sampler tile splitting GEMM column tiles across wave pairs

Compiles a new dpk8 variant of the fused sampler with 8 wavefronts per 4-pose workgroup. Each GEMM's column tiles are split between waves 0-3 and 4-7, with sub-range prefetches and tuned prefetch masks. The second half of the waves gets raised scheduling priority, and layer norm stays on four waves. The aim is more latency hiding and MFMA issue per CU. It costs more registers and barrier participants per workgroup, and this variant is the default for sparse fp32 and bf16 GEMM modes.

Result: faster. 93890 (median of 6 runs) (+1.0%).

```diff
diff --git a/diffpose-nw_amd/csrc/dpk_kernels.hip b/diffpose-nw_amd/csrc/dpk_kernels.hip
--- a/diffpose-nw_amd/csrc/dpk_kernels.hip
+++ b/diffpose-nw_amd/csrc/dpk_kernels.hip
@@ -91,6 +91,12 @@
 #include "dpk_sampler.inc"
 #include "dpk_genfused.inc"
 }
+#define DPK_NW 8
+namespace dpk8 {
+#include "dpk_sampler.inc"
+#include "dpk_genfused.inc"
+}
+#undef DPK_NW
 #undef DPK_P
 #define DPK_P 2
 namespace dpk2 {
@@ -214,6 +220,7 @@
     char* arena16 = nullptr;
     char* arenabf = nullptr;
     int gemm_mode = 0;
+    int tile_waves = 0;
     bool have_graph = false, have_weights = false;
     unsigned mask = (1u << J) - 1u;
     const unsigned* pmask = nullptr;
@@ -443,11 +450,26 @@
     return DPK_OK;
 }
 
+constexpr int TILE_WAVES_DEFAULT[3] = {8, 4, 8};
+static int tile_waves(const dpk_handle* h) {
+    if (h->tile_waves) return h->tile_waves;
+    return h->pk.sparse ? TILE_WAVES_DEFAULT[h->gemm_mode] : 4;
+}
+
 template <int MODE, int PT>
 static void launch_tiles(dpk_handle* h, int blocks, size_t shmem, hipStream_t st, const SampleArgs& a) {
     const char* a16 = h->gemm_mode == 2 ? h->arenabf : h->arena16;
-    if constexpr (PT == 4) dpk::launch_sample<MODE>(h->pk.sparse, h->gemm_mode, blocks, shmem, st, a, h->arena, a16);
-    else dpk2::launch_sample<MODE>(h->pk.sparse, h->gemm_mode, blocks, shmem, st, a, h->arena, a16);
+    if constexpr (PT == 4) {
+        if constexpr (MODE == M_SAMPLE) {
+            if (tile_waves(h) == 8) {
+                dpk8::launch_sample<MODE>(h->pk.sparse, h->gemm_mode, blocks, shmem, st, a, h->arena, a16);
+                return;
+            }
+        }
+        dpk::launch_sample<MODE>(h->pk.sparse, h->gemm_mode, blocks, shmem, st, a, h->arena, a16);
+    } else {
+        dpk2::launch_sample<MODE>(h->pk.sparse, h->gemm_mode, blocks, shmem, st, a, h->arena, a16);
+    }
 }
 
 template <int MODE>
@@ -607,6 +629,10 @@
         return DPK_E_HIP;
     }
     h->n_cu = std::max(h->n_cu, 1);
+    if (const char* tw = getenv("DPK_TILE_WAVES")) {
+        const int v = atoi(tw);
+        if (v == 0 || v == 4 || v == 8) h->tile_waves = v;
+    }
     if (const char* ts = getenv("DPK_TAIL_SPLIT")) h->tail_plan = std::min(std::max(atoi(ts), 0), 2);
     if (DPK_TRACE) h->tail_plan = 0;
     const size_t flag_bytes = ((size_t)FLAG_SLOTS * h->n_cu + 4) * 4;
@@ -838,7 +864,7 @@
     SampleArgs a = sample_args(h, h->arena, sc->tps, sc, x, out, xs, x0s, N, seed, noise);
 #if DPK_TRACE
     if (h->trace_step >= 0) {
-        const size_t len = (size_t)((N + P - 1) / P) * NW * TRACE_SLOTS;
+        const size_t len = (size_t)((N + P - 1) / P) * tile_waves(h) * TRACE_SLOTS;
         if (h->trace_len < len) {
             if (h->trace) HIPCHK(h, hipFree(h->trace));
             HIPCHK(h, hipMalloc(&h->trace, len * 8));
@@ -875,6 +901,16 @@
     if (mode < 0 || mode > 2)
         return fail(h, DPK_E_INVALID, "dpk_set_gemm_mode: mode must be 0 (fp32), 1 (3xfp16) or 2 (bf16)");
     h->gemm_mode = mode;
+    return DPK_OK;
+}
+
+int dpk_set_tile_waves(dpk_handle* h, int waves) {
+    if (!h) return DPK_E_INVALID;
+    if (waves != 0 && waves != 4 && waves != 8)
+        return fail(h, DPK_E_INVALID, "dpk_set_tile_waves: waves must be 0 (the GEMM mode's default), 4 or 8");
+    if (waves == 8 && h->gen)
+        return fail(h, DPK_E_UNSUPPORTED, "dpk_set_tile_waves: the 8-wave tile is compiled for hid 96 / 4 heads / 17 joints");
+    h->tile_waves = waves;
     return DPK_OK;
 }
 
diff --git a/diffpose-nw_amd/csrc/dpk_layout.inc b/diffpose-nw_amd/csrc/dpk_layout.inc
--- a/diffpose-nw_amd/csrc/dpk_layout.inc
+++ b/diffpose-nw_amd/csrc/dpk_layout.inc
@@ -24,7 +24,13 @@
 constexpr int P = DPK_P;
 constexpr int R = P * J;
 static_assert(P == 4 || P == 2, "4 or 2 poses per workgroup");
+#ifdef DPK_NW
+constexpr int NW = DPK_NW;
+#else
 constexpr int NW = 4;
+#endif
+static_assert(NW == 4 || (NW == 8 && P == 4), "4 waves, or 8 on a 4-pose tile");
+constexpr int NSUB = NW / 4;
 constexpr int NT = 64 * NW;
 constexpr int stride40(int n) { return n + (104 - n % 64) % 64; }
 constexpr int LDX = stride40(D);
diff --git a/diffpose-nw_amd/csrc/dpk_sampler.inc b/diffpose-nw_amd/csrc/dpk_sampler.inc
--- a/diffpose-nw_amd/csrc/dpk_sampler.inc
+++ b/diffpose-nw_amd/csrc/dpk_sampler.inc
@@ -7,7 +7,18 @@
 #ifndef DPK_PRE_MID
 #define DPK_PRE_MID 14
 #endif
-#define DPK_MID(bit) ((DPK_PRE_MID & (bit)) != 0)
+#ifndef DPK_PRE_MID_W8
+#define DPK_PRE_MID_W8 DPK_PRE_MID
+#endif
+#ifndef DPK_PRE_MID_W8F
+#define DPK_PRE_MID_W8F 4
+#endif
+#ifndef DPK_PRE_MID_W8B
+#define DPK_PRE_MID_W8B 4
+#endif
+#define DPK_W8SEL(a, f, b) (G16 == 0 ? (a) : G16 == 1 ? (f) : (b))
+#define DPK_MID(bit) \
+    (((NSUB == 2 ? DPK_W8SEL(DPK_PRE_MID_W8, DPK_PRE_MID_W8F, DPK_PRE_MID_W8B) : DPK_PRE_MID) & (bit)) != 0)
 
 typedef float f32x4 __attribute__((ext_vector_type(4)));
 typedef float f32x2 __attribute__((ext_vector_type(2)));
@@ -166,10 +177,10 @@
 
 enum { TM_NONE = 0, TM_VALU = 1, TM_MFMA4 = 2 };
 
-template <int NR, int NCW, int TM, int TR, int KB, bool TRANS = true>
+template <int NR, int NCW, int TM, int TR, int KB, bool TRANS = true, int NQO = (NCW + 1) / 2>
 struct GemmTile {
     static constexpr int TA = TM == TM_VALU ? TR : 1;
-    static constexpr int NQ = TM == TM_MFMA4 ? (NCW + 1) / 2 : 1;
+    static constexpr int NQ = TM == TM_MFMA4 ? NQO : 1;
     f32x4 acc[NR][NCW];
     float tl[NCW][TA];
     f32x4 tacc[NQ];
@@ -221,7 +232,8 @@
 };
 
 __device__ __forceinline__ int gemm_ch(int wave) { return R == 68 ? (wave & 1) : (wave >> 1); }
-__device__ __forceinline__ int gemm_pr(int wave) { return R == 68 ? (wave >> 1) : (wave & 1); }
+__device__ __forceinline__ int gemm_pr(int wave) { return R == 68 ? (NSUB == 1 ? wave >> 1 : (wave & 3) >> 1) : (wave & 1); }
+constexpr int sub_max(int n) { return NSUB == 1 ? n : n - n / 2; }
 
 template <int NCW>
 __device__ __forceinline__ int col_rot(int wave) { return gemm_pr(wave) ? (NCW + 1) / 2 : 0; }
@@ -236,16 +248,34 @@
 }
 
 template <int NC, int KB, int NPRE = 2>
-__device__ __forceinline__ BPre<NC / 2> gemm_prefetch(const float* Bp, int wave, int lane) {
-    constexpr int NCW = NC / 2;
+__device__ __forceinline__ BPre<sub_max(NC / 2)> gemm_prefetch(const float* Bp, int wave, int lane) {
+    constexpr int NCW = NC / 2, NP = sub_max(NCW);
     const BSrc s = bsrc<NC, KB>(Bp, gemm_ch(wave) * NCW, lane);
-    int soff[NCW];
-    tile_offsets<NCW, KB>(soff, s, col_rot<NCW>(wave));
-    BPre<NCW> pre;
-#pragma unroll
-    for (int c = 0; c < NCW; ++c) {
-        pre.b0[c] = bload(s, soff[c], 0);
-        pre.b1[c] = (KB > 1 && NPRE > 1) ? bload(s, soff[c], 1) : f32x4{0.f, 0.f, 0.f, 0.f};
+    if constexpr (NSUB == 1) {
+        int soff[NCW];
+        tile_offsets<NCW, KB>(soff, s, col_rot<NCW>(wave));
+        BPre<NCW> pre;
+#pragma unroll
+        for (int c = 0; c < NCW; ++c) {
+            pre.b0[c] = bload(s, soff[c], 0);
+            pre.b1[c] = (KB > 1 && NPRE > 1) ? bload(s, soff[c], 1) : f32x4{0.f, 0.f, 0.f, 0.f};
+        }
+        return pre;
+    }
+    const int c0 = NSUB == 1 ? 0 : (wave >> 2) * (NCW / 2), nown = NSUB == 1 ? NCW : (wave >> 2 ? NCW - NCW / 2 : NCW / 2);
+    const int rot = col_rot<NCW>(wave);
+    BPre<NP> pre;
+#pragma unroll
+    for (int c = 0; c < NP; ++c) {
+        const int cc = c0 + c + rot;
+        const int toff = s.voff + s.sbase + (cc >= NCW ? cc - NCW : cc) * KB * 1024;
+        const f32x4 z = {0.f, 0.f, 0.f, 0.f};
+        pre.b0[c] = z;
+        pre.b1[c] = z;
+        if (NSUB == 1 || c < nown) {
+            pre.b0[c] = bload(s, toff, 0);
+            if constexpr (KB > 1 && NPRE > 1) pre.b1[c] = bload(s, toff, 1);
+        }
     }
     return pre;
 }
@@ -253,7 +283,17 @@
 #ifndef DPK_PRE_LATE
 #define DPK_PRE_LATE 5
 #endif
-#define DPK_LATE(bit) ((DPK_PRE_LATE & (bit)) != 0)
+#ifndef DPK_PRE_LATE_W8
+#define DPK_PRE_LATE_W8 DPK_PRE_LATE
+#endif
+#ifndef DPK_PRE_LATE_W8F
+#define DPK_PRE_LATE_W8F 15
+#endif
+#ifndef DPK_PRE_LATE_W8B
+#define DPK_PRE_LATE_W8B 15
+#endif
+#define DPK_LATE(bit) \
+    (((NSUB == 2 ? DPK_W8SEL(DPK_PRE_LATE_W8, DPK_PRE_LATE_W8F, DPK_PRE_LATE_W8B) : DPK_PRE_LATE) & (bit)) != 0)
 #ifndef DPK_FC1_NPRE
 #define DPK_FC1_NPRE 2
 #endif
@@ -308,11 +348,17 @@
 }
 
 
-template <int NR, int NCW, int TM, int TR, int NC, int KB, int MODE, bool XS2 = false, int NPRE = 2>
+template <int NR, int NCW0, int TM0, int TR, int NC, int KB, int MODE, bool XS2 = false, int NPRE = 2, int C0 = 0,
+          int NCS = NCW0, int NPW = NCW0>
 __device__ __forceinline__ void gemm_wave(const float* A, int lda, const float* Bp, int rt0, int ct0, int rot,
                                           int trow0, bool tail_dup, int lane, const EpiArgs& e,
-                                          const BPre<NCW>& pre, const float* AX = nullptr, int ldx = 0) {
-    using T = GemmTile<NR, NCW, TM, TR, KB>;
+                                          const BPre<NPW>& pre, const float* AX = nullptr, int ldx = 0) {
+    constexpr int NCW = NCS;
+    constexpr int NQF = (NCW0 + 1) / 2;
+    constexpr int TQ = NQF - C0 < 0 ? 0 : (NQF - C0 > NCS ? NCS : NQF - C0);
+    constexpr int TM = (TM0 == TM_MFMA4 && TQ == 0) ? TM_NONE : TM0;
+    static_assert(C0 >= 0 && NCS >= 1 && C0 + NCS <= NCW0 && NPW >= NCS, "sub-wave tile range");
+    using T = GemmTile<NR, NCW, TM, TR, KB, true, TQ>;
     constexpr int TA = T::TA, NQ = T::NQ;
     static_assert(KB == 1 || KB % 2 == 0, "k-blocks in pairs");
     lane = opaque(lane);
@@ -332,7 +378,7 @@
     }
     int xoff[NR], xtoff = 0;
     if constexpr (XS2) {
-        static_assert(TM == TM_MFMA4, "XS2: 4x4x1 tail rows");
+        static_assert(TM0 == TM_MFMA4, "XS2: 4x4x1 tail rows");
 #pragma unroll
         for (int i = 0; i < NR; ++i) xoff[i] = ((rt0 + i) * 16 + rl) * ldx + kq;
         xtoff = (trow0 + (lane & 3)) * ldx + kq;
@@ -340,12 +386,17 @@
     int gcol[NCW];
 #pragma unroll
     for (int c = 0; c < NCW; ++c) {
-        const int cc = c + rot;
-        gcol[c] = ct0 + (cc >= NCW ? cc - NCW : cc);
+        const int cc = C0 + c + rot;
+        gcol[c] = ct0 + (cc >= NCW0 ? cc - NCW0 : cc);
     }
     const BSrc src = bsrc<NC, KB>(Bp, ct0, lane);
     int soff[NCW];
-    tile_offsets<NCW, KB>(soff, src, rot);
+    if constexpr (NCS == NCW0) {
+        tile_offsets<NCW, KB>(soff, src, rot);
+    } else {
+#pragma unroll
+        for (int c = 0; c < NCW; ++c) soff[c] = src.voff + src.sbase + (gcol[c] - ct0) * KB * 1024;
+    }
     const int tcol = 4 * ((lane >> 2) & 3) + (lane >> 4);
     f32x4 bias4[NCW], tp4[NCW];
     float tbias[NQ], ttp[NQ];
@@ -382,18 +433,18 @@
         if (XS2 && kb < KBX) {
 #pragma unroll
             for (int i = 0; i < NR; ++i) as[st][i] = *reinterpret_cast<const f32x4*>(AX + xoff[i] + kb * 16);
-            ts[st][0] = *reinterpret_cast<const f32x4*>(AX + xtoff + kb * 16);
+            if constexpr (TM != TM_NONE) ts[st][0] = *reinterpret_cast<const f32x4*>(AX + xtoff + kb * 16);
         } else {
             g.loadA(as[st], ts[st], A, kb);
         }
     };
     constexpr bool RES = MODE == E_RESID || MODE == E_RESID_RELU;
     const int trow = trow0 + (lane & 3);
-    constexpr int R0 = (NCW + 1) / 2;
+    constexpr int R0 = (NCW0 + 1) / 2;
     auto tile_ptr = [&](int i, int c) -> float* {
         const int row = (rt0 + i) * 16 + rl;
         float* rb = e.dst + row * e.ldd + kq + ct0 * 16;
-        return (c < NCW - R0 ? rb + rot * 16 : rb - (rot ? (NCW - R0) * 16 : 0)) + c * 16;
+        return (C0 + c < NCW0 - R0 ? rb + rot * 16 : rb - (rot ? (NCW0 - R0) * 16 : 0)) + (C0 + c) * 16;
     };
     f32x4 old[NR][NCW];
     float oldt[NQ];
@@ -481,7 +532,7 @@
 #pragma unroll
         for (int q = 0; q < NQ; ++q) {
             const float v = rs4rows(g.tacc[q][0], g.tacc[q][1], g.tacc[q][2], g.tacc[q][3]);
-            const bool skip = (q == NQ - 1 && tail_dup) || row >= R;
+            const bool skip = (C0 + q == NQF - 1 && tail_dup) || row >= R;
             const int col = gcol[q] * 16 + tcol;
             const float tp = MODE == E_CHEB1 ? tproj_at(e, min(row, R - 1), col, ttp[q]) : 0.f;
             float val = epi_value<MODE>(v, tbias[q], tp, RES ? oldt[q] : 0.f);
@@ -494,15 +545,25 @@
 
 template <int NC, int KB, int MODE, bool XS2 = false, int NPRE = 2>
 __device__ __forceinline__ void gemm_wg(const float* A, int lda, const float* Bp, int wave, int lane,
-                                        const EpiArgs& e, const BPre<NC / 2>& pre,
+                                        const EpiArgs& e, const BPre<sub_max(NC / 2)>& pre,
                                         const float* AX = nullptr, int ldx = 0) {
     static_assert(NC % 2 == 0 && (R == 68 || R == 34), "row tiles x 2 column halves + tail rows");
     constexpr int NCW = NC / 2;
     constexpr int NRW = R == 68 ? 2 : 1;
     const int pr = gemm_pr(wave);
     const bool dup = (NCW & 1) && pr == 1;
-    gemm_wave<NRW, NCW, TM_MFMA4, 0, NC, KB, MODE, XS2, NPRE>(A, lda, Bp, NRW * pr, gemm_ch(wave) * NCW,
-                                                             col_rot<NCW>(wave), R - R % 16, dup, lane, e, pre, AX, ldx);
+    if constexpr (NSUB == 1) {
+        gemm_wave<NRW, NCW, TM_MFMA4, 0, NC, KB, MODE, XS2, NPRE>(A, lda, Bp, NRW * pr, gemm_ch(wave) * NCW,
+                                                                 col_rot<NCW>(wave), R - R % 16, dup, lane, e, pre, AX, ldx);
+    } else {
+        constexpr int N0 = NCW / 2, N1 = NCW - N0;
+        if (wave < 4)
+            gemm_wave<NRW, NCW, TM_MFMA4, 0, NC, KB, MODE, XS2, NPRE, 0, N0, N1>(
+                A, lda, Bp, NRW * pr, gemm_ch(wave) * NCW, col_rot<NCW>(wave), R - R % 16, dup, lane, e, pre, AX, ldx);
+        else
+            gemm_wave<NRW, NCW, TM_MFMA4, 0, NC, KB, MODE, XS2, NPRE, N0, N1, N1>(
+                A, lda, Bp, NRW * pr, gemm_ch(wave) * NCW, col_rot<NCW>(wave), R - R % 16, dup, lane, e, pre, AX, ldx);
+    }
 }
 
 template <int PW>
@@ -520,6 +581,12 @@
 #ifndef DPK_PWF16
 #define DPK_PWF16 3
 #endif
+#ifndef DPK_PWF16_W8
+#define DPK_PWF16_W8 6
+#endif
+#ifndef DPK_PWQ16_W8
+#define DPK_PWQ16_W8 9
+#endif
 constexpr int BLKB = 1024;
 template <int G>
 constexpr int blkh() { return G == 1 ? BLK16 : BLKB; }
@@ -573,40 +640,66 @@
 template <int PW>
 __device__ __forceinline__ int passh_rot(int wave) { return gemm_pr(wave) ? (PW + 1) / 2 : 0; }
 template <int G, int NC, int KB32, int PW>
-__device__ __forceinline__ BPreH<G, PW> gemmh_prefetch(const char* Bp, int wave, int lane, int ps = 0) {
-    constexpr int BK = blkh<G>();
+__device__ __forceinline__ BPreH<G, sub_max(PW)> gemmh_prefetch(const char* Bp, int wave, int lane, int ps = 0) {
+    constexpr int BK = blkh<G>(), NP = sub_max(PW);
     const BSrcH s = bsrch<G, NC, KB32>(Bp);
     const int ctp = gemm_ch(wave) * (NC / 2) + ps * PW, rot = passh_rot<PW>(wave);
-    BPreH<G, PW> pre;
-#pragma unroll
-    for (int c = 0; c < PW; ++c) {
-        const int voff = lane * 16 + pass_col<PW>(ctp, c, rot) * KB32 * BK;
-#pragma unroll
-        for (int k = 0; k < 2; ++k) {
-            pre.h[k][c] = s.load(voff, k * BK);
-            if constexpr (G == 1) pre.l[k][c] = s.load(voff, k * BK + 1024);
+    BPreH<G, NP> pre;
+    if constexpr (NSUB == 1) {
+#pragma unroll
+        for (int c = 0; c < PW; ++c) {
+            const int voff = lane * 16 + pass_col<PW>(ctp, c, rot) * KB32 * BK;
+#pragma unroll
+            for (int k = 0; k < 2; ++k) {
+                pre.h[k][c] = s.load(voff, k * BK);
+                if constexpr (G == 1) pre.l[k][c] = s.load(voff, k * BK + 1024);
+            }
+        }
+        return pre;
+    }
+    const int c0 = (wave >> 2) * (PW / 2), nown = wave >> 2 ? PW - PW / 2 : PW / 2;
+#pragma unroll
+    for (int c = 0; c < NP; ++c) {
+        const int voff = lane * 16 + pass_col<PW>(ctp, c0 + c, rot) * KB32 * BK;
+        if (NSUB == 1 || c < nown) {
+#pragma unroll
+            for (int k = 0; k < 2; ++k) {
+                pre.h[k][c] = s.load(voff, k * BK);
+                if constexpr (G == 1) pre.l[k][c] = s.load(voff, k * BK + 1024);
+            }
+        } else {
+#pragma unroll
+            for (int k = 0; k < 2; ++k) {
+                pre.h[k][c] = f16x8{};
+                if constexpr (G == 1) pre.l[k][c] = f16x8{};
+            }
         }
     }
     return pre;
 }
 
-template <int G, int NR, int PW, int NC, int KB32, int MODE, bool XS2, int S, int AR>
+template <int G, int NR, int PW0, int NC, int KB32, int MODE, bool XS2, int S, int AR, int C0 = 0, int NCS = PW0,
+          int NPW = PW0>
 __device__ __forceinline__ void gemmh_pass(const float* A, int lda, const float* AX, int ldx, const BSrcH& src,
                                            int rt0, int ctp, int rot, int trow0, bool tail_dup, int lane,
-                                           const EpiArgs& e, const BPreH<G, PW>& pre, AFr<G> (*ar)[NR + 1]) {
+                                           const EpiArgs& e, const BPreH<G, NPW>& pre, AFr<G> (*ar)[NR + 1]) {
     constexpr int BK = blkh<G>();
-    constexpr int NQ = (PW + 1) / 2;
-    constexpr int NA = NR + 1;
+    constexpr int PW = NCS;
+    constexpr int NQF = (PW0 + 1) / 2;
+    constexpr int TQ = NQF - C0 < 0 ? 0 : (NQF - C0 > NCS ? NCS : NQF - C0);
+    constexpr int NQ = TQ > 0 ? TQ : 1;
+    static_assert(C0 >= 0 && NCS >= 1 && C0 + NCS <= PW0 && NPW >= NCS, "sub-wave tile range");
+    constexpr int NA = NR + (TQ > 0 ? 1 : 0);
     static_assert(S >= 2 && S <= KB32, "ring slots");
     lane = opaque(lane);
     const int rl = lane & 15, g = lane >> 4, kq = g * 4;
     int gcol[PW], voff[PW];
 #pragma unroll
     for (int c = 0; c < PW; ++c) {
-        gcol[c] = pass_col<PW>(ctp, c, rot);
+        gcol[c] = pass_col<PW0>(ctp, C0 + c, rot);
         voff[c] = lane * 16 + gcol[c] * KB32 * BK;
     }
-    int aoff[NA], xoff[NA];
+    int aoff[NR + 1], xoff[NR + 1];
 #pragma unroll
     for (int i = 0; i < NR; ++i) {
         aoff[i] = (int)__umul24((unsigned)((rt0 + i) * 16 + rl), (unsigned)lda) + kq;
@@ -615,7 +708,7 @@
     const int trow_a = min(trow0 + rl, R - 1);
     aoff[NR] = (int)__umul24((unsigned)trow_a, (unsigned)lda) + kq;
     xoff[NR] = (int)__umul24((unsigned)trow_a, (unsigned)ldx) + kq;
-    f32x4 raw[NA][2];
+    f32x4 raw[NR + 1][2];
     auto loadA = [&](int kb) {
         if constexpr (AR != 2) {
 #pragma unroll
@@ -661,7 +754,7 @@
     DPK_GEMM_HOOK(0);
     f32x4 acc[NR][PW], tacc[NQ];
     const f32x4 z = {0.f, 0.f, 0.f, 0.f};
-    AFr<G> af[NA];
+    AFr<G> af[NR + 1];
     auto cvt = [&](int kb) {
 #pragma unroll
         for (int i = 0; i < NA; ++i) {
@@ -680,7 +773,7 @@
             for (int c = 0; c < PW; ++c) oldv[i][c] = *reinterpret_cast<const f32x4*>(rp + gcol[c] * 16);
         }
 #pragma unroll
-        for (int q = 0; q < NQ; ++q)
+        for (int q = 0; q < TQ; ++q)
             oldt[q] = *reinterpret_cast<const f32x4*>(e.dst + __umul24((unsigned)trow_a, (unsigned)e.ldd) + gcol[q] * 16 + kq);
     };
     constexpr int LAG = 2;
@@ -704,7 +797,7 @@
     };
     auto tail_mfmas = [&](int st, int kb) {
 #pragma unroll
-        for (int q = 0; q < NQ; ++q) {
+        for (int q = 0; q < TQ; ++q) {
             f32x4 t = kb == 0 ? z : tacc[q];
             const f16x8 th = af[NR].h;
             if constexpr (G == 2) {
@@ -729,7 +822,7 @@
         const f32x2 hi = __builtin_elementwise_fma(f32x2{a[2], a[3]}, inv2, f32x2{bias4[q][2], bias4[q][3]});
         f32x4 o = epi_value4<MODE, true>(f32x4{lo[0], lo[1], hi[0], hi[1]}, z, tp, RES ? oldt[q] : z);
         asm volatile("" : "+v"(o));
-        const bool skip = (q == NQ - 1 && tail_dup) || row >= R;
+        const bool skip = (C0 + q == NQF - 1 && tail_dup) || row >= R;
         if (!skip) *reinterpret_cast<f32x4*>(e.dst + __umul24((unsigned)row, (unsigned)e.ldd) + gcol[q] * 16 + kq) = o;
     };
 #pragma unroll
@@ -767,13 +860,13 @@
 #pragma unroll
     for (int tt = NR * PW > LAG ? NR * PW - LAG : 0; tt < NR * PW; ++tt) epi_tile(tt / PW, tt % PW);
 #pragma unroll
-    for (int q = 0; q < NQ; ++q) epi_tail(q);
+    for (int q = 0; q < TQ; ++q) epi_tail(q);
     DPK_GEMM_HOOK(2);
 }
 
 template <int G, int NC, int KB32, int PW, int MODE, bool XS2 = false>
 __device__ __forceinline__ void gemmh_wg(const float* A, int lda, const char* Bp, int wave, int lane, const EpiArgs& e,
-                                         const BPreH<G, PW>& pre, const float* AX = nullptr, int ldx = 0) {
+                                         const BPreH<G, sub_max(PW)>& pre, const float* AX = nullptr, int ldx = 0) {
     static_assert(NC % 2 == 0 && (NC / 2) % PW == 0 && (R == 68 || R == 34), "passes of PW column tiles");
     constexpr int NCW = NC / 2, NRW = R == 68 ? 2 : 1, NPASS = NCW / PW;
     constexpr int S = PW >= 6 ? ((G == 2 && KB32 == 3) ? 3 : 2)
@@ -783,10 +876,28 @@
     const bool dup = (PW & 1) && pr == 1;
     const BSrcH src = bsrch<G, NC, KB32>(Bp);
     const int ct0 = gemm_ch(wave) * NCW;
-    if constexpr (NPASS == 1) {
+    auto passes = [&](auto c0_, auto ncs_) {
+        constexpr int C0 = decltype(c0_)::value, NCS = decltype(ncs_)::value, NPW = sub_max(PW);
+        if constexpr (NPASS == 1) {
+            gemmh_pass<G, NRW, PW, NC, KB32, MODE, XS2, S, 0, C0, NCS, NPW>(A, lda, AX, ldx, src, NRW * pr, ct0, rot,
+                                                                            R - R % 16, dup, lane, e, pre, nullptr);
+        } else {
+            AFr<G> ar[KB32][NRW + 1];
+            gemmh_pass<G, NRW, PW, NC, KB32, MODE, XS2, S, 1, C0, NCS, NPW>(A, lda, AX, ldx, src, NRW * pr, ct0, rot,
+                                                                            R - R % 16, dup, lane, e, pre, ar);
+#pragma unroll
+            for (int ps = 1; ps < NPASS; ++ps) {
+                const BPreH<G, NPW> p2 = gemmh_prefetch<G, NC, KB32, PW>(Bp, wave, lane, ps);
+                gemmh_pass<G, NRW, PW, NC, KB32, MODE, XS2, S, 2, C0, NCS, NPW>(A, lda, AX, ldx, src, NRW * pr,
+                                                                                ct0 + ps * PW, rot, R - R % 16, dup, lane,
+                                                                                e, p2, ar);
+            }
+        }
+    };
+    if constexpr (NSUB == 1 && NPASS == 1) {
         gemmh_pass<G, NRW, PW, NC, KB32, MODE, XS2, S, 0>(A, lda, AX, ldx, src, NRW * pr, ct0, rot, R - R % 16, dup,
                                                           lane, e, pre, nullptr);
-    } else {
+    } else if constexpr (NSUB == 1) {
         AFr<G> ar[KB32][NRW + 1];
         gemmh_pass<G, NRW, PW, NC, KB32, MODE, XS2, S, 1>(A, lda, AX, ldx, src, NRW * pr, ct0, rot, R - R % 16, dup,
                                                           lane, e, pre, ar);
@@ -796,12 +907,16 @@
             gemmh_pass<G, NRW, PW, NC, KB32, MODE, XS2, S, 2>(A, lda, AX, ldx, src, NRW * pr, ct0 + ps * PW, rot,
                                                               R - R % 16, dup, lane, e, p2, ar);
         }
+    } else {
+        constexpr int N0 = PW / 2;
+        if (wave < 4) passes(std::integral_constant<int, 0>{}, std::integral_constant<int, N0>{});
+        else passes(std::integral_constant<int, N0>{}, std::integral_constant<int, PW - N0>{});
     }
 }
 
 template <int G, int NC, int KB32, int PW>
 struct HGemm {
-    using Pre = BPreH<G, PW>;
+    using Pre = BPreH<G, sub_max(PW)>;
     __device__ __forceinline__ static Pre prefetch(const char* Bp, int wave, int lane) {
         return gemmh_prefetch<G, NC, KB32, PW>(Bp, wave, lane);
     }
@@ -879,7 +994,7 @@
     constexpr float RD = 1.0f / (float)D, RD1 = 1.0f / (float)(D - 1);
     constexpr int RM = R - R % 16, RT = R % 16;
     static_assert((RM == 64 && RT == 4) || (RM == 32 && RT == 2), "row tiles + one tail row per wave");
-    if constexpr (RM != 64)
+    if constexpr (RM != 64 || NW > 4)
         if (w >= RT) return;
     const int row = (POSEMAP ? w * J : w * 16) + (lane >> 2), part = lane & 3;
     const int trow = POSEMAP ? w * J + 16 : RM + w;
@@ -1695,10 +1810,12 @@
 #else
 #define BAR() __syncthreads()
 #endif
+    if constexpr (NSUB == 2)
+        if (wave >= 4) __builtin_amdgcn_s_setprio(1);
 #pragma unroll 1
     for (int s = s_beg; s < s_end; ++s) {
         {
-            const BPre<NCD / 2> pre = gemm_prefetch<NCD, 1>(W + OFF_WIN, wave, lane);
+            const BPre<sub_max(NCD / 2)> pre = gemm_prefetch<NCD, 1>(W + OFF_WIN, wave, lane);
             input_prep<SPARSE>(CW, XST, B1, tid);
             BAR();
             const EpiArgs e{XS, LDX, W + OFF_BIN, nullptr, 0, pose0, a.N - 1};
@@ -1711,13 +1828,13 @@
             const float* LW = W + l * LAYER_FLOATS;
             constexpr int GH = G16 ? G16 : 1;
             const char* LH = arena16 + offh<GH>(l, 0);
-            constexpr int PWQ = G16 == 2 ? 9 : DPK_PWQ16;
-            constexpr int PWF = G16 == 2 ? 6 : DPK_PWF16;
+            constexpr int PWQ = G16 == 2 ? 9 : (NSUB == 2 ? DPK_PWQ16_W8 : DPK_PWQ16);
+            constexpr int PWF = G16 == 2 ? 6 : (NSUB == 2 ? DPK_PWF16_W8 : DPK_PWF16);
             constexpr int GG = G16 == 2 ? 2 : 0;
             {
                 const EpiArgs e{B2, LD2, LW + OFF_CQKV, nullptr, 0, pose0, a.N - 1};
                 using HQ = HGemm<GH, 3 * NCD, KB32_D, PWQ>;
-                BPre<3 * NCD / 2> pre;
+                BPre<sub_max(3 * NCD / 2)> pre;
                 typename HQ::Pre preh;
                 if constexpr (G16 == 0 && !DPK_LATE(1)) pre = gemm_prefetch<3 * NCD, KB_D, DPK_QKV_NPRE>(LW + OFF_QKV, wave, lane);
                 if (DPK_RUN(8)) layer_norm<false, false>(XS, B1, LNP + l * 4 * D, LNP + l * 4 * D + D, tid);
@@ -1738,7 +1855,7 @@
             {
                 const EpiArgs e{XS, LDX, LW + OFF_BO, nullptr, 0, pose0, a.N - 1};
                 using HO = HGemm<GH, NCD, KB32_D, 3>;
-                BPre<NCD / 2> pre;
+                BPre<sub_max(NCD / 2)> pre;
                 typename HO::Pre preh;
                 auto o_pre = [&]() {
                     if constexpr (G16) preh = HO::prefetch(LH + O16_O / GH, wave, lane);
@@ -1764,23 +1881,24 @@
             gbias_load(gb, LW + OFF_BFC2, lane, wave);
             {
                 using HF = HGemm<GH, 2 * NCD, KB32_D, PWF>;
-                BPre<NCD> pre;
+                BPre<sub_max(NCD)> pre;
                 typename HF::Pre preh;
                 auto f_pre = [&]() {
                     if constexpr (G16) preh = HF::prefetch(LH + O16_FC1 / GH, wave, lane);
                     else pre = gemm_prefetch<2 * NCD, KB_D, DPK_FC1_NPRE>(LW + OFF_FC1, wave, lane);
                 };
-                constexpr bool FC1_MID = DPK_MID(4) && R == 68;
+                constexpr bool LN1_OWN = R == 68 && NW == P;
+                constexpr bool FC1_MID = DPK_MID(4) && LN1_OWN;
                 if constexpr (!DPK_LATE(4) && !FC1_MID) f_pre();
                 const GFrag gf = GG != 0 ? gfrag_load_h(LW + OFF_LG, lane) : gfrag_load(LW + OFF_LGF, lane);
-                if constexpr (R == 68) {
+                if constexpr (LN1_OWN) {
                     if (DPK_RUN(8)) layer_norm<true>(XS, B1, LNP + l * 4 * D + 2 * D, LNP + l * 4 * D + 3 * D, tid);
                     asm volatile("" ::: "memory");
                     if constexpr (FC1_MID) {
                         if (DPK_RUN(2)) graph_mma<false, GG>(gf, B1, B1, nullptr, wave, lane, f_pre);
                     } else if (DPK_RUN(2)) graph_mma<false, GG>(gf, B1, B1, nullptr, wave, lane);
                 } else {
-                    if (DPK_RUN(8)) layer_norm(XS, B1, LNP + l * 4 * D + 2 * D, LNP + l * 4 * D + 3 * D, tid);
+                    if (DPK_RUN(8)) layer_norm<R == 68>(XS, B1, LNP + l * 4 * D + 2 * D, LNP + l * 4 * D + 3 * D, tid);
                     BAR();
                     if (DPK_RUN(2)) graph_mma<false, GG>(gf, B1, B1, nullptr, wave, lane);
                 }
@@ -1808,7 +1926,7 @@
                     BAR();
                     if (DPK_RUN(16 | 256)) H2::template run<E_STORE_NB>(B2, LD2, LH + O16_FC2 / GH, wave, lane, e, pre);
                 } else {
-                    const BPre<NCD / 2> pre = gemm_prefetch<NCD, KB_D2>(LW + OFF_FC2, wave, lane);
+                    const BPre<sub_max(NCD / 2)> pre = gemm_prefetch<NCD, KB_D2>(LW + OFF_FC2, wave, lane);
                     BAR();
                     if (DPK_RUN(16 | 256)) gemm_wg<NCD, KB_D2, E_STORE_NB>(B2, LD2, LW + OFF_FC2, wave, lane, e, pre);
                 }
@@ -1817,7 +1935,7 @@
                 const float* tp = a.tproj + (MODE == M_SAMPLE ? (size_t)s * NL * D : 0) + l * D;
                 const EpiArgs e{B1, LDX, LW + OFF_BC1, tp, EPS_MODE ? NL * D : 0, pose0, a.N - 1};
                 using HC = HGemm<GH, NCD, KB32_D3, 3>;
-                BPre<NCD / 2> pre;
+                BPre<sub_max(NCD / 2)> pre;
                 typename HC::Pre preh;
                 auto c1_pre = [&]() {
                     if constexpr (G16) preh = HC::prefetch(LH + O16_C1 / GH, wave, lane);
@@ -1842,7 +1960,7 @@
             {
                 const EpiArgs e{XS, LDX, LW + OFF_BC2, nullptr, 0, pose0, a.N - 1};
                 using HC = HGemm<GH, NCD, KB32_D3, 3>;
-                BPre<NCD / 2> pre;
+                BPre<sub_max(NCD / 2)> pre;
                 typename HC::Pre preh;
                 auto c2_pre = [&]() {
                     if constexpr (G16) preh = HC::prefetch(LH + O16_C2 / GH, wave, lane);
diff --git a/diffpose-nw_amd/diffpose_amd/_lib.py b/diffpose-nw_amd/diffpose_amd/_lib.py
--- a/diffpose-nw_amd/diffpose_amd/_lib.py
+++ b/diffpose-nw_amd/diffpose_amd/_lib.py
@@ -12,7 +12,7 @@
 EXPORTS = ("dpk_version", "dpk_create", "dpk_set_graph", "dpk_load_weights", "dpk_set_mask", "dpk_set_pose_masks",
            "dpk_set_schedule", "dpk_eps", "dpk_sample", "dpk_sample_noise", "dpk_ddim_update", "dpk_ddim_update_noise",
            "dpk_pose", "dpk_pose_metrics", "dpk_gmm_sample", "dpk_gmm_sample_f64", "dpk_set_gemm_mode",
-           "dpk_set_tail_plan", "dpk_debug_split", "dpk_debug_resources", "dpk_profile", "dpk_profile_read",
+           "dpk_set_tail_plan", "dpk_set_tile_waves", "dpk_debug_split", "dpk_debug_resources", "dpk_profile", "dpk_profile_read",
            "dpk_kernel_geometry", "dpk_last_error", "dpk_destroy")
 
 
@@ -73,6 +73,7 @@
     L.dpk_gmm_sample_f64.argtypes = [vp, vp, i32, i32, vp, i32, vp, u64, ctypes.c_double, vp, vp, vp, vp]
     L.dpk_set_gemm_mode.argtypes = [vp, i32]
     L.dpk_set_tail_plan.argtypes = [vp, i32]
+    L.dpk_set_tile_waves.argtypes = [vp, i32]
     L.dpk_profile.argtypes = [vp, i32]
     L.dpk_profile_read.argtypes = [vp, fp, i32, ctypes.POINTER(i32)]
     L.dpk_kernel_geometry.argtypes = [ctypes.POINTER(i32)] * 3
diff --git a/diffpose-nw_amd/diffpose_amd/gcndiff.py b/diffpose-nw_amd/diffpose_amd/gcndiff.py
--- a/diffpose-nw_amd/diffpose_amd/gcndiff.py
+++ b/diffpose-nw_amd/diffpose_amd/gcndiff.py
@@ -180,6 +180,11 @@
             raise ValueError(f"tail plan must be one of {sorted(self.TAIL_PLANS)}, got {plan!r}")
         _lib.check(self._h, "dpk_set_tail_plan", _lib.lib().dpk_set_tail_plan(self._h, self.TAIL_PLANS[plan]))
 
+    def set_tile_waves(self, waves: int = 0) -> None:
+        if waves not in (0, 4, 8):
+            raise ValueError(f"tile waves must be 0, 4 or 8, got {waves!r}")
+        _lib.check(self._h, "dpk_set_tile_waves", _lib.lib().dpk_set_tile_waves(self._h, int(waves)))
+
     def debug_split(self, mode: int = 0, read: bool = False):
         n = ctypes.c_int(0)
         _lib.check(self._h, "dpk_debug_split",
diff --git a/include/diffpose_kernels.h b/include/diffpose_kernels.h
--- a/include/diffpose_kernels.h
+++ b/include/diffpose_kernels.h
@@ -74,6 +74,8 @@
 
 int dpk_set_tail_plan(dpk_handle* h, int plan);
 
+int dpk_set_tile_waves(dpk_handle* h, int waves);
+
 int dpk_profile(dpk_handle* h, int enable);
 int dpk_profile_read(dpk_handle* h, float* ms_out, int cap, int* count);
 
```
